# ilovepose/fast-human-pose-estimation.pytorch

Measured on AMD Instinct MI355X. Metric: images/sec FPD train step (4-stack HG student, 8-stack teacher) 256x256, higher is better.
Workload: dtype bf16; 1 GPU; configs[1]: hourglass student S=4 F=128 + teacher S=8 F=256, 256x256, batch 32/GPU, fused FPD step incl. Adam, teacher forward one batch ahead on a 2nd stream; global_batch=32, parallelism=dp1, backend=mfma, launch=one native plan call per phase, kernels launched eagerly on 3 streams, ranks=1, finite=True

## Files before the change

fast-human-pose-estimation.pytorch_amd/csrc/api.hip:

```cpp
#include <cstdarg>
#include <cstdio>
#include <cstdlib>
#include <cstring>
#include <string>
#include <vector>

#include "common.h"

int fpd_conv_mfma_launch(const fpd_conv_t& a, hipStream_t st);
int fpd_conv_tile_launch(const fpd_conv_t& a, hipStream_t st);
int fpd_conv_pp_launch(const fpd_conv_t& a, hipStream_t st);
int fpd_conv_c1_launch(const fpd_conv_t& a, hipStream_t st);
int fpd_conv_c3_launch(const fpd_conv_t& a, hipStream_t st);
int fpd_conv_c3_pair_launch(const fpd_conv_t& a, const fpd_conv_t& b, hipStream_t st);
int fpd_conv_c3_fold_ok(const fpd_conv_t& a, const fpd_conv_t* b);
int fpd_conv_c3_option(int which, int value);
int fpd_conv_c1_pair_launch(const fpd_conv_t& a, const fpd_conv_t& b, hipStream_t st);
int fpd_conv_c1_fold_ok(const fpd_conv_t& a, const fpd_conv_t* b);
int fpd_conv_c1_option(int which, int value);
int fpd_conv_c1_wgrad_partials(const fpd_conv_t& a);
int fpd_conv_c1_pair_wgrad_partials(const fpd_conv_t& a, const fpd_conv_t& b, int* na, int* nb);
int fpd_conv_pp_pair_launch(const fpd_conv_t& a, const fpd_conv_t& b, hipStream_t st);
int fpd_conv_pp_fold_ok(const fpd_conv_t& a, const fpd_conv_t* b);
int fpd_conv_tile_fold_ok(const fpd_conv_t& a);
int fpd_conv_tile_pair_fold_ok(const fpd_conv_t& a, const fpd_conv_t& b);
int fpd_conv_pp_option(int which, int value);
int fpd_conv_pp_wgrad_partials(const fpd_conv_t& a);
int fpd_conv_pp_pair_wgrad_partials(const fpd_conv_t& a, const fpd_conv_t& b, int* na, int* nb);
int fpd_conv_tile_pair_launch(const fpd_conv_t& a, const fpd_conv_t& b, hipStream_t st);
int fpd_bneck_fused_launch(const fpd_bneck_t& a, hipStream_t st);
int fpd_bneck_fold_launch(const fpd_bneck_t& a, float* out, hipStream_t st);
int fpd_pck_launch(const fpd_pck_t& a, hipStream_t st);
int fpd_conv_smallc_launch(const fpd_conv_t& a, hipStream_t st);
bool fpd_conv_f8_domain(const fpd_conv_t& a);
int fpd_conv_tile_f8_launch(const fpd_conv_t& a, const void* w8, const float* wscale, hipStream_t st);
int fpd_weight_quant_f8_launch(const fpd_wquant_entry_t* table, int n, hipStream_t st);
int fpd_flip_w_launch(const float* x, float* y, int64_t rows, int W, hipStream_t st);
int fpd_flip_merge_launch(const fpd_flipmerge_t& p, hipStream_t st);
int fpd_final_preds_launch(const fpd_finalpreds_t& p, hipStream_t st);
int fpd_render_targets_launch(const fpd_targets_t& a, hipStream_t st);
int fpd_warp_affine_launch(const fpd_warp_t& a, hipStream_t st);
int fpd_head_fused_launch(const fpd_head_t& a, hipStream_t st);
int fpd_head_fold_launch(const fpd_head_t& a, float* out, hipStream_t st);
int fpd_bneck_fused_pair_launch(const fpd_bneck_t& a, const fpd_bneck_t& b, hipStream_t st);
int fpd_wgrad_mfma_launch(const fpd_wgrad_t& a, hipStream_t st);
int fpd_wgrad_tile_launch(const fpd_wgrad_t& a, hipStream_t st);
int fpd_wgrad_tile_partials(const fpd_wgrad_t& a);
int fpd_wgrad_smallc_launch(const fpd_wgrad_t& a, hipStream_t st);
int fpd_wgrad_smallc_partials(const fpd_wgrad_t& a);
int fpd_wgrad_mfma_partials(const fpd_wgrad_t& a);
int fpd_wgrad_naive_partials(const fpd_wgrad_t& a);
int fpd_stem_wgrad_mfma_partials(const fpd_stem_t& a);
int fpd_stem_wgrad_partials(const fpd_stem_t& a);
int fpd_wreduce_launch(const fpd_wreduce_entry_t* table, int n, int64_t max_elems, hipStream_t st);
int fpd_conv_naive_launch(const fpd_conv_t& a, hipStream_t st);
int fpd_wgrad_naive_launch(const fpd_wgrad_t& a, hipStream_t st);
int fpd_stem_forward_launch(const fpd_stem_t& a, hipStream_t st);
int fpd_stem_forward_mfma_launch(const fpd_stem_t& a, hipStream_t st);
int fpd_stem_forward_s2d_launch(const fpd_stem_t& a, hipStream_t st);
int fpd_stem_wgrad_s2d_launch(const fpd_stem_t& a, hipStream_t st);
int fpd_stem_wgrad_s2d_partials(const fpd_stem_t& a);
int fpd_stem_wgrad_mfma_launch(const fpd_stem_t& a, hipStream_t st);
int fpd_stem_wgrad_launch(const fpd_stem_t& a, hipStream_t st);
int fpd_elementwise_launch(const fpd_ew_t& a, hipStream_t st);
int fpd_elementwise_pair_launch(const fpd_ew_t& a, const fpd_ew_t& b, hipStream_t st);
int fpd_affsum_launch(const fpd_affsum_t& a, hipStream_t st);
int fpd_loss_launch(const fpd_loss_t& a, hipStream_t st);
int fpd_adam_launch(const fpd_adam_t& a, hipStream_t st);
int fpd_weight_prep_launch(const fpd_wprep_entry_t* table, int n, int64_t max_elems, int dtype, hipStream_t st);
int fpd_bn_update_running_launch(const fpd_bnupd_entry_t* table, int n, hipStream_t st);
int fpd_cast_launch(const void* src, void* dst, int64_t n, int sd, int dd, hipStream_t st);
int fpd_nchw_to_nhwc_launch(const float* src, void* dst, int N, int C, int H, int W, int dtype, hipStream_t st);
int fpd_nhwc_to_nchw_launch(const void* src, float* dst, int N, int C, int H, int W, int dtype, hipStream_t st);

int g_fpd_backend = FPD_BACKEND_MFMA;
static thread_local char g_err[512] = "";

static FILE* g_launch_log_file = nullptr;
static bool launch_log_open() {
    const char* path = getenv("FPD_LAUNCH_LOG");
    if (path == nullptr || path[0] == 0) return false;
    g_launch_log_file = fopen(path, "w");
    if (g_launch_log_file == nullptr) fprintf(stderr, "[fpd_amd] FPD_LAUNCH_LOG: cannot open %s\n", path);
    return g_launch_log_file != nullptr;
}
bool g_fpd_launch_log = launch_log_open();
static thread_local char g_op_tag[256] = "-";
void fpd_log_launch(const char* kernel, const dim3& grid, const dim3& block) {
    if (g_launch_log_file == nullptr) return;
    fprintf(g_launch_log_file, "%s\t%u\t%u\t%s\n", kernel, grid.x * grid.y * grid.z, block.x * block.y * block.z, g_op_tag);
    fflush(g_launch_log_file);
}

int fpd_fail(int code, const char* fmt, ...) {
    va_list ap;
    va_start(ap, fmt);
    vsnprintf(g_err, sizeof(g_err), fmt, ap);
    va_end(ap);
    return code;
}

static int check_launch() {
    hipError_t e = hipGetLastError();
    if (e != hipSuccess) return fpd_fail(-100 - (int)e, "kernel launch failed: %s", hipGetErrorString(e));
    return 0;
}

static int validate_conv_dims(int N, int H, int W, int C, int K, int R, int S, int stride, int pad, int P, int Q) {
    FPD_REQUIRE(N > 0 && H > 0 && W > 0 && C > 0 && K > 0 && R > 0 && S > 0 && stride > 0 && pad >= 0,
                "conv: non-positive dimension");
    FPD_REQUIRE(P == (H + 2 * pad - R) / stride + 1 && Q == (W + 2 * pad - S) / stride + 1,
                "conv: output %dx%d inconsistent with input %dx%d k=%dx%d stride=%d pad=%d", P, Q, H, W, R, S, stride, pad);
    FPD_REQUIRE((int64_t)N * H * W * C < (1ll << 31) && (int64_t)N * P * Q * K < (1ll << 31), "conv: tensor too large for 32-bit indexing");
    return 0;
}

extern "C" {

const char* fpd_last_error(void) { return g_err; }
int fpd_abi_version(void) { return FPD_ABI_VERSION; }
int64_t fpd_stats_words(int32_t channels) { return FPD_STATS_WORDS(channels); }
int fpd_set_backend(int32_t backend) {
    const int prev = g_fpd_backend;
    if (backend == FPD_BACKEND_MFMA || backend == FPD_BACKEND_NAIVE || backend == FPD_BACKEND_MFMA_GENERIC) g_fpd_backend = backend;
    return prev;
}

static int g_wgrad_tile_only = 0;

int fpd_set_option(const char* name, int32_t value) {
    FPD_REQUIRE(name, "set_option: null name");
    if (!strcmp(name, "conv_pp")) return fpd_conv_pp_option(0, value);
    if (!strcmp(name, "conv_pp_blocks")) return fpd_conv_pp_option(1, value);
    if (!strcmp(name, "conv_c1")) return fpd_conv_c1_option(0, value);
    if (!strcmp(name, "conv_c1_blocks")) return fpd_conv_c1_option(1, value);
    if (!strcmp(name, "conv_c1_launches")) return fpd_conv_c1_option(2, value);
    if (!strcmp(name, "conv_c3")) return fpd_conv_c3_option(0, value);
    if (!strcmp(name, "conv_c3_blocks")) return fpd_conv_c3_option(1, value);
    if (!strcmp(name, "conv_c3_launches")) return fpd_conv_c3_option(2, value);
    if (!strcmp(name, "wgrad_tile_only")) { g_wgrad_tile_only = value; return 0; }
    return fpd_fail(-2, "set_option: unknown option '%s'", name);
}

int fpd_abi_sizeof(const char* n) {
#define SZ(T) if (!strcmp(n, #T)) return (int)sizeof(T)
    SZ(fpd_bn_t); SZ(fpd_conv_t); SZ(fpd_wgrad_t); SZ(fpd_stem_t); SZ(fpd_ew_t); SZ(fpd_loss_t); SZ(fpd_adam_t);
    SZ(fpd_wprep_entry_t); SZ(fpd_bnupd_entry_t); SZ(fpd_memset_t); SZ(fpd_table_t); SZ(fpd_wreduce_entry_t); SZ(fpd_bneck_t); SZ(fpd_conv_pair_t); SZ(fpd_bneck_pair_t); SZ(fpd_ew_pair_t); SZ(fpd_pck_t); SZ(fpd_head_t); SZ(fpd_affsum_t); SZ(fpd_layout_t);
    SZ(fpd_conv_f8_t); SZ(fpd_wquant_entry_t); SZ(fpd_flipmerge_t); SZ(fpd_finalpreds_t); SZ(fpd_targets_t); SZ(fpd_warp_src_t); SZ(fpd_warp_t);
#undef SZ
    return -1;
}

static int validate_conv(const fpd_conv_t* a) {
    FPD_REQUIRE(a && a->x && a->w && a->y, "conv: null pointer");
    int rc = validate_conv_dims(a->N, a->H, a->W, a->C, a->K, a->R, a->S, a->stride, a->pad, a->P, a->Q);
    if (rc) return rc;
    FPD_REQUIRE(a->dtype == FPD_F32 || a->dtype == FPD_BF16, "conv: bad dtype %d", a->dtype);
    FPD_REQUIRE(a->bn.mode == FPD_BN_NONE || (a->bn.gamma && a->bn.beta), "conv: BN prologue without gamma/beta");
    FPD_REQUIRE(a->bn.mode != FPD_BN_TRAIN || a->bn.stats, "conv: train-mode BN without statistics");
    FPD_REQUIRE(a->bn.mode != FPD_BN_EVAL || (a->bn.running_mean && a->bn.running_var), "conv: eval-mode BN without running stats");
    FPD_REQUIRE(a->epi == FPD_EPI_PLAIN || (a->epi_x && a->epi_stats && a->epi_bn.mode == FPD_BN_TRAIN && a->epi_bn.stats),
                "conv: BNRELU_BWD epilogue needs epi_x, epi_stats and a train-mode epi_bn");
    return 0;
}

static int dispatch_conv(const fpd_conv_t* a, hipStream_t st) {
    int rc = 1;
    if (g_fpd_backend == FPD_BACKEND_MFMA) rc = fpd_conv_c1_launch(*a, st);
    if (rc == 1 && g_fpd_backend == FPD_BACKEND_MFMA) rc = fpd_conv_c3_launch(*a, st);
    if (rc == 1 && g_fpd_backend == FPD_BACKEND_MFMA) rc = fpd_conv_pp_launch(*a, st);
    FPD_REQUIRE(rc != 1 || a->wg_partial == nullptr, "conv: a fused weight gradient (wg_partial) needs the persistent kernel; "
                "fpd_conv_fused_wgrad_partials() reports 0 for this launch");
    if (rc == 1 && g_fpd_backend == FPD_BACKEND_MFMA) rc = fpd_conv_tile_launch(*a, st);
    FPD_REQUIRE(rc != 1 || a->fold_x == nullptr, "conv: a folded BN-backward apply (fold_x) needs the persistent or the halo-tile "
                "kernel; fpd_conv_fold_supported() reports 0 for this launch");
    if (rc == 1 && g_fpd_backend != FPD_BACKEND_NAIVE) rc = fpd_conv_mfma_launch(*a, st);
    if (rc == 1 && g_fpd_backend != FPD_BACKEND_NAIVE) rc = fpd_conv_smallc_launch(*a, st);
    if (rc == 1) rc = fpd_conv_naive_launch(*a, st);
    return rc;
}

int fpd_conv_forward(const fpd_conv_t* a, fpd_stream_t stream) {
    int rc = validate_conv(a);
    if (rc) return rc;
    rc = dispatch_conv(a, (hipStream_t)stream);
    return rc ? rc : check_launch();
}

int fpd_conv_fold_supported(const fpd_conv_t* a) {
    if (!a || g_fpd_backend != FPD_BACKEND_MFMA || validate_conv(a) != 0) return 0;
    return (fpd_conv_c1_fold_ok(*a, nullptr) || fpd_conv_c3_fold_ok(*a, nullptr) || fpd_conv_pp_fold_ok(*a, nullptr) || fpd_conv_tile_fold_ok(*a)) ? 1 : 0;
}
int fpd_conv_pair_fold_supported(const fpd_conv_pair_t* p) {
    if (!p || g_fpd_backend != FPD_BACKEND_MFMA || validate_conv(&p->a) != 0 || validate_conv(&p->b) != 0) return 0;
    if (fpd_conv_c1_fold_ok(p->a, &p->b)) return 1;
    if (fpd_conv_c3_fold_ok(p->a, &p->b)) return 1;
    if (fpd_conv_pp_fold_ok(p->a, &p->b)) return 1;
    const int r = fpd_conv_tile_pair_fold_ok(p->a, p->b);
    if (r >= 0) return r;
    return (fpd_conv_fold_supported(&p->a) && fpd_conv_fold_supported(&p->b)) ? 1 : 0;
}

int fpd_conv_fused_wgrad_partials(const fpd_conv_t* a) {
    if (!a || g_fpd_backend != FPD_BACKEND_MFMA || validate_conv(a) != 0) return 0;
    const int n = fpd_conv_c1_wgrad_partials(*a);
    return n >= 0 ? n : fpd_conv_pp_wgrad_partials(*a);
}
int fpd_conv_pair_fused_wgrad_partials(const fpd_conv_pair_t* p, int32_t* n_a, int32_t* n_b) {
    FPD_REQUIRE(p && n_a && n_b, "conv_pair_fused_wgrad_partials: null pointer");
    *n_a = *n_b = 0;
    if (g_fpd_backend != FPD_BACKEND_MFMA || validate_conv(&p->a) != 0 || validate_conv(&p->b) != 0) return 0;
    int na = 0, nb = 0;
    if (fpd_conv_c1_pair_wgrad_partials(p->a, p->b, &na, &nb) < 0) fpd_conv_pp_pair_wgrad_partials(p->a, p->b, &na, &nb);
    *n_a = na; *n_b = nb;
    return 0;
}

int fpd_conv_f8_in_domain(const fpd_conv_t* c) { return (c && fpd_conv_f8_domain(*c)) ? 1 : 0; }

int fpd_conv_forward_f8(const fpd_conv_f8_t* a, fpd_stream_t stream) {
    FPD_REQUIRE(a, "conv_f8: null pointer");
    int rc = validate_conv(&a->c);
    if (rc) return rc;
    FPD_REQUIRE(a->w8 && a->w8_scale, "conv_f8: null fp8 weights / scales");
    FPD_REQUIRE(((uintptr_t)a->w8 & 15) == 0, "conv_f8: w8 must be 16-byte aligned");
    rc = 1;
    if (g_fpd_backend == FPD_BACKEND_MFMA) rc = fpd_conv_tile_f8_launch(a->c, a->w8, a->w8_scale, (hipStream_t)stream);
    if (rc == 1) rc = dispatch_conv(&a->c, (hipStream_t)stream);
    return rc ? rc : check_launch();
}

int fpd_weight_quant_f8(const fpd_wquant_entry_t* t, int32_t n, fpd_stream_t stream) {
    FPD_REQUIRE(n == 0 || t != nullptr, "weight_quant_f8: null table");
    int rc = fpd_weight_quant_f8_launch(t, n, (hipStream_t)stream);
    return rc ? rc : check_launch();
}

int fpd_conv_forward_pair(const fpd_conv_pair_t* p, fpd_stream_t stream) {
    FPD_REQUIRE(p, "conv_pair: null pointer");
    int rc = validate_conv(&p->a);
    if (rc) return rc;
    rc = validate_conv(&p->b);
    if (rc) return rc;
    hipStream_t st = (hipStream_t)stream;
    rc = 1;
    if (g_fpd_backend == FPD_BACKEND_MFMA) rc = fpd_conv_c1_pair_launch(p->a, p->b, st);
    if (rc == 1 && g_fpd_backend == FPD_BACKEND_MFMA) rc = fpd_conv_c3_pair_launch(p->a, p->b, st);
    if (rc == 1 && g_fpd_backend == FPD_BACKEND_MFMA) rc = fpd_conv_pp_pair_launch(p->a, p->b, st);
    FPD_REQUIRE(rc != 1 || (p->a.wg_partial == nullptr && p->b.wg_partial == nullptr),
                "conv_pair: fused weight gradients need the persistent kernel; fpd_conv_pair_fused_wgrad_partials() reports 0 for this launch");
    if (rc == 1 && g_fpd_backend == FPD_BACKEND_MFMA) rc = fpd_conv_tile_pair_launch(p->a, p->b, st);
    if (rc == 1) {
        rc = dispatch_conv(&p->a, st);
        if (rc == 0) rc = dispatch_conv(&p->b, st);
    }
    return rc ? rc : check_launch();
}

static int validate_bneck_bns(const fpd_bneck_t* a) {
    const fpd_bn_t* bns[3] = {&a->bn1, &a->bn2, &a->bn3};
    for (int i = 0; i < 3; ++i)
        FPD_REQUIRE(bns[i]->mode == FPD_BN_EVAL && bns[i]->relu && bns[i]->gamma && bns[i]->beta && bns[i]->running_mean &&
                    bns[i]->running_var, "bottleneck: bn%d must be an eval-mode BN+ReLU with running statistics", i + 1);
    return 0;
}

int fpd_bottleneck_fold(const fpd_bneck_t* a, fpd_stream_t stream) {
    FPD_REQUIRE(a && a->folded, "bottleneck_fold: null pointer");
    int rc = validate_bneck_bns(a);
    if (rc) return rc;
    rc = fpd_bneck_fold_launch(*a, const_cast<float*>(a->folded), (hipStream_t)stream);
    if (rc == 1) return fpd_fail(-3, "bottleneck_fold: C=%d P=%d is outside the fused kernel's domain", a->C, a->P);
    return rc ? rc : check_launch();
}

int fpd_bottleneck_forward_pair(const fpd_bneck_pair_t* p, fpd_stream_t stream) {
    FPD_REQUIRE(p, "bottleneck_pair: null pointer");
    const fpd_bneck_t* ab[2] = {&p->a, &p->b};
    for (const fpd_bneck_t* a : ab) {
        FPD_REQUIRE(a->x && a->y && a->w1 && a->w2 && a->w3 && a->x != a->y, "bottleneck_pair: null pointer or y aliases x");
        FPD_REQUIRE((int64_t)a->N * a->H * a->W * a->C < ((int64_t)1 << 31), "bottleneck_pair: tensor too large for 32-bit indexing");
        int rc = validate_bneck_bns(a);
        if (rc) return rc;
    }
    int rc = fpd_bneck_fused_pair_launch(p->a, p->b, (hipStream_t)stream);
    if (rc == 1) {
        rc = fpd_bottleneck_forward(&p->a, stream);
        return rc ? rc : fpd_bottleneck_forward(&p->b, stream);
    }
    return rc ? rc : check_launch();
}

int fpd_bottleneck_forward(const fpd_bneck_t* a, fpd_stream_t stream) {
    FPD_REQUIRE(a && a->x && a->y && a->w1 && a->w2 && a->w3, "bottleneck: null pointer");
    FPD_REQUIRE(a->x != a->y, "bottleneck: y must not alias x");
    FPD_REQUIRE(a->N > 0 && a->H > 0 && a->W > 0 && a->C > 0 && a->P > 0, "bottleneck: bad dims");
    FPD_REQUIRE((int64_t)a->N * a->H * a->W * a->C < ((int64_t)1 << 31), "bottleneck: tensor too large for 32-bit indexing");
    int rc = validate_bneck_bns(a);
    if (rc) return rc;
    rc = fpd_bneck_fused_launch(*a, (hipStream_t)stream);
    if (rc == 1)
        return fpd_fail(-3, "bottleneck: shape N=%d H=%d W=%d C=%d P=%d dtype=%d is outside the fused kernel's domain",
                        a->N, a->H, a->W, a->C, a->P, a->dtype);
    return rc ? rc : check_launch();
}

int fpd_conv_wgrad(const fpd_wgrad_t* a, fpd_stream_t stream) {
    FPD_REQUIRE(a && a->x && a->dy && a->dw, "wgrad: null pointer");
    int rc = validate_conv_dims(a->N, a->H, a->W, a->C, a->K, a->R, a->S, a->stride, a->pad, a->P, a->Q);
    if (rc) return rc;
    FPD_REQUIRE(a->dtype == FPD_F32 || a->dtype == FPD_BF16, "wgrad: bad dtype %d", a->dtype);
    hipStream_t st = (hipStream_t)stream;
    rc = 1;
    FPD_REQUIRE(a->partial == nullptr || a->partial_stride >= (int64_t)a->K * a->R * a->S * a->C + a->K,
                "wgrad: partial_stride %lld smaller than weight + bias", (long long)a->partial_stride);
    if (g_fpd_backend == FPD_BACKEND_MFMA) rc = fpd_wgrad_tile_launch(*a, st);
    FPD_REQUIRE(!(g_wgrad_tile_only && rc == 1), "wgrad: option wgrad_tile_only is set and the halo-tile kernel declines N=%d H=%d W=%d C=%d K=%d R=%d", a->N, a->H, a->W, a->C, a->K, a->R);
    if (rc == 1 && g_fpd_backend != FPD_BACKEND_NAIVE) rc = fpd_wgrad_mfma_launch(*a, st);
    if (rc == 1 && g_fpd_backend != FPD_BACKEND_NAIVE) rc = fpd_wgrad_smallc_launch(*a, st);
    if (rc == 1) rc = fpd_wgrad_naive_launch(*a, st);
    return rc ? rc : check_launch();
}

int fpd_wgrad_num_partials(const fpd_wgrad_t* a) {
    if (!a) return 0;
    int n = 0;
    if (g_fpd_backend == FPD_BACKEND_MFMA) n = fpd_wgrad_tile_partials(*a);
    if (n == 0 && g_fpd_backend != FPD_BACKEND_NAIVE) n = fpd_wgrad_mfma_partials(*a);
    if (n == 0 && g_fpd_backend != FPD_BACKEND_NAIVE) n = fpd_wgrad_smallc_partials(*a);
    if (n == 0) n = fpd_wgrad_naive_partials(*a);
    return n;
}

int fpd_stem_wgrad_num_partials(const fpd_stem_t* a) {
    if (!a) return 0;
    int n = 0;
    if (g_fpd_backend == FPD_BACKEND_MFMA) n = fpd_stem_wgrad_s2d_partials(*a);
    if (n == 0 && g_fpd_backend == FPD_BACKEND_MFMA) n = fpd_stem_wgrad_mfma_partials(*a);
    if (n == 0) n = fpd_stem_wgrad_partials(*a);
    return n;
}

int fpd_wgrad_reduce(const fpd_wreduce_entry_t* t, int32_t n, int64_t max_elems, fpd_stream_t stream) {
    int rc = fpd_wreduce_launch(t, n, max_elems, (hipStream_t)stream);
    return rc ? rc : check_launch();
}

int fpd_stem_forward(const fpd_stem_t* a, fpd_stream_t stream) {
    FPD_REQUIRE(a && a->x && a->w && a->bias && a->y, "stem: null pointer");
    FPD_REQUIRE(a->P == (a->H + 6 - 7) / 2 + 1 && a->Q == (a->W + 6 - 7) / 2 + 1, "stem: bad output size");
    int rc = 1;
    if (g_fpd_backend == FPD_BACKEND_MFMA) rc = fpd_stem_forward_s2d_launch(*a, (hipStream_t)stream);
    if (rc == 1 && g_fpd_backend == FPD_BACKEND_MFMA) rc = fpd_stem_forward_mfma_launch(*a, (hipStream_t)stream);
    if (rc == 1) rc = fpd_stem_forward_launch(*a, (hipStream_t)stream);
    return rc ? rc : check_launch();
}

int fpd_stem_wgrad(const fpd_stem_t* a, fpd_stream_t stream) {
    FPD_REQUIRE(a && a->x && a->dy && a->dw, "stem wgrad: null pointer");
    FPD_REQUIRE(a->partial == nullptr || a->partial_stride >= (int64_t)a->K * 148, "stem wgrad: partial_stride %lld smaller than weight + bias",
                (long long)a->partial_stride);
    int rc = 1;
    if (g_fpd_backend == FPD_BACKEND_MFMA) rc = fpd_stem_wgrad_s2d_launch(*a, (hipStream_t)stream);
    if (rc == 1 && g_fpd_backend == FPD_BACKEND_MFMA) rc = fpd_stem_wgrad_mfma_launch(*a, (hipStream_t)stream);
    if (rc == 1) rc = fpd_stem_wgrad_launch(*a, (hipStream_t)stream);
    return rc ? rc : check_launch();
}

int fpd_affsum(const fpd_affsum_t* a, fpd_stream_t stream) {
    FPD_REQUIRE(a && a->y, "affsum: null pointer");
    FPD_REQUIRE(a->nterms >= 1 && a->nterms <= FPD_AFFSUM_MAX, "affsum: %d terms (1..%d supported)", a->nterms, FPD_AFFSUM_MAX);
    FPD_REQUIRE(a->dtype == FPD_F32 || a->dtype == FPD_BF16, "affsum: bad dtype %d", a->dtype);
    for (int j = 0; j < a->nterms; ++j) {
        const int up = a->t[j].up;
        FPD_REQUIRE(a->t[j].x, "affsum: term %d has no input", j);
        FPD_REQUIRE((up == 1 || up == 2 || up == 4 || up == 8) && a->H % up == 0 && a->W % up == 0,
                    "affsum: term %d: up-sampling factor %d does not divide %dx%d", j, up, a->H, a->W);
        const fpd_bn_t& bn = a->t[j].bn;
        FPD_REQUIRE(bn.mode == FPD_BN_NONE || (bn.gamma && bn.beta), "affsum: term %d: BN without gamma/beta", j);
        FPD_REQUIRE(bn.mode != FPD_BN_TRAIN || bn.stats, "affsum: term %d: train-mode BN without statistics", j);
        FPD_REQUIRE(bn.mode != FPD_BN_EVAL || (bn.running_mean && bn.running_var), "affsum: term %d: eval-mode BN without running stats", j);
    }
    int rc = fpd_affsum_launch(*a, (hipStream_t)stream);
    return rc ? rc : check_launch();
}

int fpd_elementwise(const fpd_ew_t* a, fpd_stream_t stream) {
    FPD_REQUIRE(a && (a->y || a->op == FPD_EW_BNRELU_BWD_R), "elementwise: null pointer");
    int rc = fpd_elementwise_launch(*a, (hipStream_t)stream);
    return rc ? rc : check_launch();
}

static int validate_head(const fpd_head_t* a) {
    FPD_REQUIRE(a && a->y0 && a->score && a->w_fc && a->w_score, "head: null pointer");
    FPD_REQUIRE(a->next == nullptr || (a->x && a->w_fc2 && a->w_score2 && a->next != a->x && a->next != a->y0),
                "head: next needs x, w_fc2, w_score2 and must not alias an input");
    FPD_REQUIRE(a->N > 0 && a->H > 0 && a->W > 0 && (int64_t)a->N * a->H * a->W * a->C < ((int64_t)1 << 31), "head: bad dims");
    FPD_REQUIRE(a->bn.mode == FPD_BN_EVAL && a->bn.relu && a->bn.gamma && a->bn.beta && a->bn.running_mean && a->bn.running_var,
                "head: bn must be an eval-mode BN+ReLU with running statistics");
    return 0;
}
int fpd_head_forward(const fpd_head_t* a, fpd_stream_t stream) {
    int rc = validate_head(a);
    if (rc) return rc;
    rc = fpd_head_fused_launch(*a, (hipStream_t)stream);
    if (rc == 1) return fpd_fail(-3, "head: C=%d J=%d dtype=%d is outside the fused kernel's domain", a->C, a->J, a->dtype);
    return rc ? rc : check_launch();
}
int fpd_head_fold(const fpd_head_t* a, fpd_stream_t stream) {
    FPD_REQUIRE(a && a->folded, "head_fold: null pointer");
    FPD_REQUIRE(a->bn.mode == FPD_BN_EVAL && a->bn.gamma && a->bn.beta && a->bn.running_mean && a->bn.running_var, "head_fold: bn");
    int rc = fpd_head_fold_launch(*a, const_cast<float*>(a->folded), (hipStream_t)stream);
    if (rc == 1) return fpd_fail(-3, "head_fold: C=%d is outside the fused kernel's domain", a->C);
    return rc ? rc : check_launch();
}

int fpd_pck(const fpd_pck_t* a, fpd_stream_t stream) {
    FPD_REQUIRE(a && a->out && a->target && a->counts && a->log && a->cursor, "pck: null pointer");
    FPD_REQUIRE(a->B > 0 && a->J > 0 && a->H > 0 && a->W > 0 && a->log_slots > 0, "pck: bad dims");
    FPD_REQUIRE(a->dtype == FPD_F32 || a->dtype == FPD_BF16, "pck: bad dtype %d", a->dtype);
    int rc = fpd_pck_launch(*a, (hipStream_t)stream);
    return rc ? rc : check_launch();
}

int fpd_flip_w(const float* x, float* y, int64_t rows, int32_t W, fpd_stream_t stream) {
    FPD_REQUIRE(x && y && x != y, "flip_w: null or aliased pointer");
    FPD_REQUIRE(rows > 0 && W > 0, "flip_w: bad dims");
    int rc = fpd_flip_w_launch(x, y, rows, W, (hipStream_t)stream);
    return rc ? rc : check_launch();
}
int fpd_flip_merge(const fpd_flipmerge_t* a, fpd_stream_t stream) {
    FPD_REQUIRE(a && a->b && a->y && a->b != a->y, "flip_merge: null or aliased pointer");
    FPD_REQUIRE(a->N > 0 && a->H > 0 && a->W > 0 && a->J > 0 && a->J <= FPD_MAX_JOINTS, "flip_merge: bad dims (J <= %d)", FPD_MAX_JOINTS);
    for (int j = 0; j < a->J; ++j) FPD_REQUIRE(a->src[j] >= 0 && a->src[j] < a->J, "flip_merge: src[%d] = %d out of range", j, a->src[j]);
    int rc = fpd_flip_merge_launch(*a, (hipStream_t)stream);
    return rc ? rc : check_launch();
}
int fpd_final_preds(const fpd_finalpreds_t* a, fpd_stream_t stream) {
    FPD_REQUIRE(a && a->hm && a->coords && a->maxvals, "final_preds: null pointer");
    FPD_REQUIRE((a->trans == nullptr) == (a->preds == nullptr), "final_preds: trans and preds go together");
    FPD_REQUIRE(a->N > 0 && a->H > 0 && a->W > 0 && a->J > 0, "final_preds: bad dims");
    int rc = fpd_final_preds_launch(*a, (hipStream_t)stream);
    return rc ? rc : check_launch();
}
int fpd_render_targets(const fpd_targets_t* a, fpd_stream_t stream) {
    FPD_REQUIRE(a && a->joints && a->vis && a->g && a->target && a->weight, "render_targets: null pointer");
    FPD_REQUIRE(a->B > 0 && a->J > 0 && a->H > 0 && a->W > 0 && a->patch > 0 && (a->patch & 1), "render_targets: bad dims");
    FPD_REQUIRE(a->stride_x > 0 && a->stride_y > 0, "render_targets: bad stride");
    int rc = fpd_render_targets_launch(*a, (hipStream_t)stream);
    return rc ? rc : check_launch();
}
int fpd_warp_affine(const fpd_warp_t* a, fpd_stream_t stream) {
    FPD_REQUIRE(a && a->src && a->out, "warp_affine: null pointer");
    FPD_REQUIRE(a->B > 0 && a->B <= 65535 && a->H > 0 && a->W > 0, "warp_affine: bad dims");
    for (int c = 0; c < 3; ++c) FPD_REQUIRE(a->std[c] != 0.f, "warp_affine: std[%d] == 0", c);
    int rc = fpd_warp_affine_launch(*a, (hipStream_t)stream);
    return rc ? rc : check_launch();
}

int fpd_elementwise_pair(const fpd_ew_pair_t* p, fpd_stream_t stream) {
    FPD_REQUIRE(p && p->a.y && p->b.y, "elementwise_pair: null pointer");
    int rc = fpd_elementwise_pair_launch(p->a, p->b, (hipStream_t)stream);
    if (rc == 1) {
        rc = fpd_elementwise_launch(p->a, (hipStream_t)stream);
        if (rc == 0) rc = fpd_elementwise_launch(p->b, (hipStream_t)stream);
    }
    return rc ? rc : check_launch();
}

int fpd_loss(const fpd_loss_t* a, fpd_stream_t stream) {
    FPD_REQUIRE(a && a->teacher && a->target && a->weight && a->losses, "loss: null pointer");
    int rc = fpd_loss_launch(*a, (hipStream_t)stream);
    return rc ? rc : check_launch();
}

int fpd_adam(const fpd_adam_t* a, fpd_stream_t stream) {
    FPD_REQUIRE(a && a->param && a->grad && a->m && a->v && a->n >= 0, "adam: null pointer");
    int rc = fpd_adam_launch(*a, (hipStream_t)stream);
    return rc ? rc : check_launch();
}

int fpd_weight_prep(const fpd_wprep_entry_t* t, int32_t n, int64_t max_elems, int32_t dtype, fpd_stream_t stream) {
    int rc = fpd_weight_prep_launch(t, n, max_elems, dtype, (hipStream_t)stream);
    return rc ? rc : check_launch();
}
int fpd_bn_update_running(const fpd_bnupd_entry_t* t, int32_t n, fpd_stream_t stream) {
    int rc = fpd_bn_update_running_launch(t, n, (hipStream_t)stream);
    return rc ? rc : check_launch();
}
int fpd_cast(const void* src, void* dst, int64_t n, int32_t sd, int32_t dd, fpd_stream_t stream) {
    int rc = fpd_cast_launch(src, dst, n, sd, dd, (hipStream_t)stream);
    return rc ? rc : check_launch();
}
int fpd_nchw_to_nhwc(const float* src, void* dst, int32_t N, int32_t C, int32_t H, int32_t W, int32_t dtype, fpd_stream_t stream) {
    int rc = fpd_nchw_to_nhwc_launch(src, dst, N, C, H, W, dtype, (hipStream_t)stream);
    return rc ? rc : check_launch();
}
int fpd_nhwc_to_nchw(const void* src, float* dst, int32_t N, int32_t C, int32_t H, int32_t W, int32_t dtype, fpd_stream_t stream) {
    int rc = fpd_nhwc_to_nchw_launch(src, dst, N, C, H, W, dtype, (hipStream_t)stream);
    return rc ? rc : check_launch();
}

struct fpd_op {
    int32_t type;
    union {
        fpd_affsum_t affsum; fpd_layout_t layout; fpd_conv_f8_t conv8; fpd_conv_t conv; fpd_conv_pair_t pair; fpd_bneck_t bneck; fpd_bneck_pair_t bpair; fpd_ew_pair_t epair; fpd_pck_t pck; fpd_head_t head; fpd_wgrad_t wgrad; fpd_stem_t stem; fpd_ew_t ew; fpd_loss_t loss; fpd_adam_t adam;
        fpd_memset_t mset; fpd_table_t table;
    } u;
};
struct fpd_sched {
    int32_t lane = 0;
    bool record = false;
    hipEvent_t done = nullptr;
    std::vector<int32_t> waits;
};
struct fpd_plan {
    std::vector<fpd_op> ops;
    std::vector<fpd_sched> sched;
    std::vector<hipGraphExec_t> graphs;
    std::vector<hipGraph_t> graph_defs;
    hipStream_t lanes[FPD_MAX_LANES] = {};
    hipEvent_t lane_done[FPD_MAX_LANES] = {};
    hipEvent_t fork = nullptr;
};

fpd_plan* fpd_plan_create(void) { return new fpd_plan(); }
void fpd_plan_destroy(fpd_plan* p) {
    if (!p) return;
    for (auto g : p->graphs) (void)hipGraphExecDestroy(g);
    for (auto g : p->graph_defs) (void)hipGraphDestroy(g);
    for (auto& s : p->sched) if (s.done) (void)hipEventDestroy(s.done);
    for (int l = 0; l < FPD_MAX_LANES; ++l) {
        if (p->lanes[l]) (void)hipStreamDestroy(p->lanes[l]);
        if (p->lane_done[l]) (void)hipEventDestroy(p->lane_done[l]);
    }
    if (p->fork) (void)hipEventDestroy(p->fork);
    delete p;
}
int fpd_plan_size(const fpd_plan* p) { return p ? (int)p->ops.size() : -1; }

int fpd_plan_add(fpd_plan* p, int32_t op, const void* args, int64_t bytes) {
    FPD_REQUIRE(p && args, "plan_add: null");
    fpd_op o;
    memset(&o, 0, sizeof(o));
    o.type = op;
    size_t want = 0;
    switch (op) {
        case FPD_OP_CONV: want = sizeof(fpd_conv_t); break;
        case FPD_OP_CONV_F8: want = sizeof(fpd_conv_f8_t); break;
        case FPD_OP_WGRAD: want = sizeof(fpd_wgrad_t); break;
        case FPD_OP_CONV_PAIR: want = sizeof(fpd_conv_pair_t); break;
        case FPD_OP_BNECK_PAIR: want = sizeof(fpd_bneck_pair_t); break;
        case FPD_OP_EW_PAIR: want = sizeof(fpd_ew_pair_t); break;
        case FPD_OP_PCK: want = sizeof(fpd_pck_t); break;
        case FPD_OP_HEAD: case FPD_OP_HEAD_FOLD: want = sizeof(fpd_head_t); break;
        case FPD_OP_BNECK: case FPD_OP_BNECK_FOLD: want = sizeof(fpd_bneck_t); break;
        case FPD_OP_STEM_FWD: case FPD_OP_STEM_WGRAD: want = sizeof(fpd_stem_t); break;
        case FPD_OP_EW: want = sizeof(fpd_ew_t); break;
        case FPD_OP_LOSS: want = sizeof(fpd_loss_t); break;
        case FPD_OP_ADAM: want = sizeof(fpd_adam_t); break;
        case FPD_OP_MEMSET: case FPD_OP_NOP: want = sizeof(fpd_memset_t); break;
        case FPD_OP_AFFSUM: want = sizeof(fpd_affsum_t); break;
        case FPD_OP_NCHW2NHWC: want = sizeof(fpd_layout_t); break;
        case FPD_OP_WPREP: case FPD_OP_BNUPD: case FPD_OP_WREDUCE: case FPD_OP_WQUANT: want = sizeof(fpd_table_t); break;
        default: return fpd_fail(-2, "plan_add: unknown op %d", op);
    }
    FPD_REQUIRE((size_t)bytes == want, "plan_add: op %d expects %zu bytes of args, got %lld", op, want, (long long)bytes);
    memcpy(&o.u, args, want);
    p->ops.push_back(o);
    p->sched.emplace_back();
    return (int)p->ops.size() - 1;
}

int fpd_plan_set_schedule(fpd_plan* p, int32_t op, int32_t lane, const int32_t* wait_ops, int32_t n_waits) {
    FPD_REQUIRE(p && op >= 0 && op < (int)p->ops.size(), "plan_set_schedule: bad op index %d", op);
    FPD_REQUIRE(lane >= 0 && lane < FPD_MAX_LANES, "plan_set_schedule: lane %d outside [0,%d)", lane, FPD_MAX_LANES);
    FPD_REQUIRE(n_waits >= 0 && (n_waits == 0 || wait_ops != nullptr), "plan_set_schedule: bad wait list");
    for (int i = 0; i < n_waits; ++i)
        FPD_REQUIRE(wait_ops[i] >= 0 && wait_ops[i] < op, "plan_set_schedule: op %d may only wait for earlier ops (got %d)", op, wait_ops[i]);
    fpd_sched& s = p->sched[op];
    s.lane = lane;
    s.waits.assign(wait_ops, wait_ops + n_waits);
    for (int i = 0; i < n_waits; ++i) p->sched[wait_ops[i]].record = true;
    return 0;
}

int fpd_plan_mark_event(fpd_plan* p, int32_t op) {
    FPD_REQUIRE(p && op >= 0 && op < (int)p->ops.size(), "plan_mark_event: bad op index %d", op);
    p->sched[op].record = true;
    return 0;
}

int fpd_plan_wait_op(fpd_plan* p, int32_t op, fpd_stream_t stream) {
    FPD_REQUIRE(p && op >= 0 && op < (int)p->ops.size(), "plan_wait_op: bad op index %d", op);
    FPD_REQUIRE(p->sched[op].record && p->sched[op].done, "plan_wait_op: op %d has no recorded event (mark it, then run its range)", op);
    FPD_CHECK_HIP(hipStreamWaitEvent((hipStream_t)stream, p->sched[op].done, 0));
    return 0;
}

static void conv_tag(char* p, size_t n, const char* what, const fpd_conv_t& c) {
    snprintf(p, n, "%s N=%d H=%d W=%d C=%d K=%d R=%d s=%d %s%s%s%s", what, c.N, c.H, c.W, c.C, c.K, c.R, c.stride,
             c.epi == FPD_EPI_BNRELU_BWD ? "dgrad" : "fwd", c.bn.mode == FPD_BN_EVAL ? " evalbn" : "", c.wg_partial ? " +wgrad" : "", c.fold_x ? " +fold" : "");
}
static void set_op_tag(int idx, const fpd_op& o) {
    char t[200] = "";
    static const char* ew_names[] = {"bnrelu_fwd", "bnrelu_bwd_r", "bn_bwd_apply", "maxpool_fwd", "maxpool_bwd", "upadd_fwd", "sumpool", "add", "relu_mask", "dilate2"};
    auto ewn = [&](int op) { return (op >= 0 && op < 10) ? ew_names[op] : "ew"; };
    switch (o.type) {
        case FPD_OP_CONV: conv_tag(t, sizeof(t), "conv", o.u.conv); break;
        case FPD_OP_CONV_F8: conv_tag(t, sizeof(t), "conv_f8", o.u.conv8.c); break;
        case FPD_OP_CONV_PAIR: {
            char a[90], b[90];
            conv_tag(a, sizeof(a), "conv2", o.u.pair.a);
            snprintf(b, sizeof(b), " | H=%d W=%d", o.u.pair.b.H, o.u.pair.b.W);
            snprintf(t, sizeof(t), "%s%s", a, b);
            break;
        }
        case FPD_OP_WGRAD: snprintf(t, sizeof(t), "wgrad N=%d H=%d W=%d C=%d K=%d R=%d s=%d", o.u.wgrad.N, o.u.wgrad.H, o.u.wgrad.W, o.u.wgrad.C, o.u.wgrad.K, o.u.wgrad.R, o.u.wgrad.stride); break;
        case FPD_OP_BNECK: snprintf(t, sizeof(t), "bneck N=%d H=%d W=%d C=%d P=%d", o.u.bneck.N, o.u.bneck.H, o.u.bneck.W, o.u.bneck.C, o.u.bneck.P); break;
        case FPD_OP_BNECK_PAIR: snprintf(t, sizeof(t), "bneck2 N=%d H=%d W=%d C=%d P=%d | H=%d W=%d", o.u.bpair.a.N, o.u.bpair.a.H, o.u.bpair.a.W, o.u.bpair.a.C, o.u.bpair.a.P, o.u.bpair.b.H, o.u.bpair.b.W); break;
        case FPD_OP_HEAD: snprintf(t, sizeof(t), "head N=%d H=%d W=%d C=%d J=%d", o.u.head.N, o.u.head.H, o.u.head.W, o.u.head.C, o.u.head.J); break;
        case FPD_OP_EW: snprintf(t, sizeof(t), "ew %s N=%d H=%d W=%d C=%d", ewn(o.u.ew.op), o.u.ew.N, o.u.ew.H, o.u.ew.W, o.u.ew.C); break;
        case FPD_OP_EW_PAIR: snprintf(t, sizeof(t), "ew2 %s N=%d H=%d W=%d C=%d | H=%d W=%d", ewn(o.u.epair.a.op), o.u.epair.a.N, o.u.epair.a.H, o.u.epair.a.W, o.u.epair.a.C, o.u.epair.b.H, o.u.epair.b.W); break;
        case FPD_OP_STEM_FWD: case FPD_OP_STEM_WGRAD: snprintf(t, sizeof(t), "%s N=%d H=%d W=%d K=%d", o.type == FPD_OP_STEM_FWD ? "stem_fwd" : "stem_wgrad", o.u.stem.N, o.u.stem.H, o.u.stem.W, o.u.stem.K); break;
        case FPD_OP_AFFSUM: snprintf(t, sizeof(t), "affsum N=%d H=%d W=%d C=%d terms=%d", o.u.affsum.N, o.u.affsum.H, o.u.affsum.W, o.u.affsum.C, o.u.affsum.nterms); break;
        case FPD_OP_LOSS: snprintf(t, sizeof(t), "loss B=%d J=%d H=%d W=%d S=%d", o.u.loss.B, o.u.loss.J, o.u.loss.H, o.u.loss.W, o.u.loss.S); break;
        case FPD_OP_ADAM: snprintf(t, sizeof(t), "adam n=%lld", (long long)o.u.adam.n); break;
        case FPD_OP_WREDUCE: snprintf(t, sizeof(t), "wreduce entries=%d", o.u.table.n); break;
        case FPD_OP_WPREP: snprintf(t, sizeof(t), "wprep entries=%d", o.u.table.n); break;
        case FPD_OP_BNUPD: snprintf(t, sizeof(t), "bnupd entries=%d", o.u.table.n); break;
        default: snprintf(t, sizeof(t), "op%d", o.type); break;
    }
    snprintf(g_op_tag, sizeof(g_op_tag), "%d\t%s", idx, t);
}

static int run_op(const fpd_op& o, fpd_stream_t s) {
    switch (o.type) {
        case FPD_OP_CONV: return fpd_conv_forward(&o.u.conv, s);
        case FPD_OP_CONV_F8: return fpd_conv_forward_f8(&o.u.conv8, s);
        case FPD_OP_WQUANT: return fpd_weight_quant_f8((const fpd_wquant_entry_t*)o.u.table.table, o.u.table.n, s);
        case FPD_OP_WGRAD: return fpd_conv_wgrad(&o.u.wgrad, s);
        case FPD_OP_CONV_PAIR: return fpd_conv_forward_pair(&o.u.pair, s);
        case FPD_OP_BNECK_PAIR: return fpd_bottleneck_forward_pair(&o.u.bpair, s);
        case FPD_OP_EW_PAIR: return fpd_elementwise_pair(&o.u.epair, s);
        case FPD_OP_PCK: return fpd_pck(&o.u.pck, s);
        case FPD_OP_HEAD: return fpd_head_forward(&o.u.head, s);
        case FPD_OP_HEAD_FOLD: return fpd_head_fold(&o.u.head, s);
        case FPD_OP_BNECK: return fpd_bottleneck_forward(&o.u.bneck, s);
        case FPD_OP_BNECK_FOLD: return fpd_bottleneck_fold(&o.u.bneck, s);
        case FPD_OP_STEM_FWD: return fpd_stem_forward(&o.u.stem, s);
        case FPD_OP_STEM_WGRAD: return fpd_stem_wgrad(&o.u.stem, s);
        case FPD_OP_EW: return fpd_elementwise(&o.u.ew, s);
        case FPD_OP_LOSS: return fpd_loss(&o.u.loss, s);
        case FPD_OP_ADAM: return fpd_adam(&o.u.adam, s);
        case FPD_OP_MEMSET: {
            FPD_CHECK_HIP(hipMemsetAsync(o.u.mset.ptr, 0, (size_t)o.u.mset.bytes, (hipStream_t)s));
            return 0;
        }
        case FPD_OP_NOP: return 0;
        case FPD_OP_AFFSUM: return fpd_affsum(&o.u.affsum, s);
        case FPD_OP_NCHW2NHWC:
            return fpd_nchw_to_nhwc(o.u.layout.src, o.u.layout.dst, o.u.layout.N, o.u.layout.C, o.u.layout.H, o.u.layout.W, o.u.layout.dtype, s);
        case FPD_OP_WPREP:
            return fpd_weight_prep((const fpd_wprep_entry_t*)o.u.table.table, o.u.table.n, o.u.table.max_elems, o.u.table.dtype, s);
        case FPD_OP_BNUPD: return fpd_bn_update_running((const fpd_bnupd_entry_t*)o.u.table.table, o.u.table.n, s);
        case FPD_OP_WREDUCE: return fpd_wgrad_reduce((const fpd_wreduce_entry_t*)o.u.table.table, o.u.table.n, o.u.table.max_elems, s);
    }
    return fpd_fail(-2, "run_op: unknown op %d", o.type);
}

static int lane_priority() { return 0; }

static int side_streams() { return FPD_MAX_LANES; }

int fpd_plan_run(fpd_plan* p, int32_t begin, int32_t end, fpd_stream_t stream) {
    FPD_REQUIRE(p && begin >= 0 && end <= (int)p->ops.size() && begin <= end, "plan_run: bad range [%d,%d)", begin, end);
    hipStream_t main_s = (hipStream_t)stream;
    bool multi = false;
    for (int i = begin; i < end; ++i) multi |= p->sched[i].lane != 0;
    bool used[FPD_MAX_LANES] = {};
    if (multi) {
        if (!p->fork) FPD_CHECK_HIP(hipEventCreateWithFlags(&p->fork, hipEventDisableTiming));
        FPD_CHECK_HIP(hipEventRecord(p->fork, main_s));
    }
    int rc = 0;
    for (int i = begin; i < end && rc == 0; ++i) {
        fpd_sched& sc = p->sched[i];
        hipStream_t st = main_s;
        if (sc.lane != 0) {
            const int l = 1 + (sc.lane - 1) % side_streams();
            if (!p->lanes[l]) {
                FPD_CHECK_HIP(hipStreamCreateWithPriority(&p->lanes[l], hipStreamNonBlocking, lane_priority()));
                FPD_CHECK_HIP(hipEventCreateWithFlags(&p->lane_done[l], hipEventDisableTiming));
            }
            st = p->lanes[l];
            if (!used[l]) {
                FPD_CHECK_HIP(hipStreamWaitEvent(st, p->fork, 0));
                used[l] = true;
            }
        }
        for (int32_t w : sc.waits)
            if (w >= begin && w < end) FPD_CHECK_HIP(hipStreamWaitEvent(st, p->sched[w].done, 0));
        if (g_fpd_launch_log) set_op_tag(i, p->ops[i]);
        rc = run_op(p->ops[i], (fpd_stream_t)st);
        if (rc) {
            char tmp[400];
            snprintf(tmp, sizeof(tmp), "%s", g_err);
            rc = fpd_fail(rc, "plan op %d (type %d): %s", i, p->ops[i].type, tmp);
            break;
        }
        if (sc.record) {
            if (!sc.done) FPD_CHECK_HIP(hipEventCreateWithFlags(&sc.done, hipEventDisableTiming));
            FPD_CHECK_HIP(hipEventRecord(sc.done, st));
        }
    }
    for (int l = 1; l < FPD_MAX_LANES; ++l)
        if (used[l]) {
            FPD_CHECK_HIP(hipEventRecord(p->lane_done[l], p->lanes[l]));
            FPD_CHECK_HIP(hipStreamWaitEvent(main_s, p->lane_done[l], 0));
        }
    return rc;
}

int fpd_plan_run_op(fpd_plan* p, int32_t op, fpd_stream_t stream) {
    FPD_REQUIRE(p && op >= 0 && op < (int)p->ops.size(), "plan_run_op: bad op index %d", op);
    if (g_fpd_launch_log) set_op_tag(op, p->ops[op]);
    return run_op(p->ops[op], stream);
}

int fpd_plan_capture(fpd_plan* p, int32_t begin, int32_t end, fpd_stream_t stream) {
    FPD_REQUIRE(p, "plan_capture: null");
    FPD_REQUIRE(!g_fpd_launch_log, "plan_capture: FPD_LAUNCH_LOG is set -- the launch log keys a kernel trace 1:1 and cannot follow hipGraph replays; unset one of them");
    hipStream_t st = (hipStream_t)stream;
    FPD_CHECK_HIP(hipStreamBeginCapture(st, hipStreamCaptureModeThreadLocal));
    int rc = fpd_plan_run(p, begin, end, stream);
    hipGraph_t g = nullptr;
    hipError_t e = hipStreamEndCapture(st, &g);
    if (rc) { if (g) (void)hipGraphDestroy(g); return rc; }
    if (e != hipSuccess) return fpd_fail(-100 - (int)e, "hipStreamEndCapture: %s", hipGetErrorString(e));
    hipGraphExec_t ge = nullptr;
    FPD_CHECK_HIP(hipGraphInstantiate(&ge, g, nullptr, nullptr, 0));
    p->graph_defs.push_back(g);
    p->graphs.push_back(ge);
    return (int)p->graphs.size() - 1;
}

int fpd_plan_replay(fpd_plan* p, int32_t gid, fpd_stream_t stream) {
    FPD_REQUIRE(p && gid >= 0 && gid < (int)p->graphs.size(), "plan_replay: bad graph id %d", gid);
    FPD_CHECK_HIP(hipGraphLaunch(p->graphs[gid], (hipStream_t)stream));
    return 0;
}

void* fpd_event_create(void) {
    hipEvent_t e = nullptr;
    if (hipEventCreate(&e) != hipSuccess) return nullptr;
    return (void*)e;
}
int fpd_event_record(void* ev, fpd_stream_t stream) {
    FPD_CHECK_HIP(hipEventRecord((hipEvent_t)ev, (hipStream_t)stream));
    return 0;
}
float fpd_event_elapsed_ms(void* start, void* stop) {
    float ms = -1.f;
    if (hipEventSynchronize((hipEvent_t)stop) != hipSuccess) return -1.f;
    if (hipEventElapsedTime(&ms, (hipEvent_t)start, (hipEvent_t)stop) != hipSuccess) return -1.f;
    return ms;
}
void fpd_event_destroy(void* ev) { if (ev) (void)hipEventDestroy((hipEvent_t)ev); }

}
```

fast-human-pose-estimation.pytorch_amd/csrc/bneck_fused.hip:

```cpp
#include <algorithm>
#include <cstdlib>
#include <type_traits>

#include "common.h"

namespace {

typedef unsigned int u32x4 __attribute__((ext_vector_type(4)));
template <int N, typename F>
__device__ __forceinline__ void static_for(F&& f) {
    if constexpr (N > 0) {
        static_for<N - 1>(f);
        f(std::integral_constant<int, N - 1>{});
    }
}

#ifdef FPD_BNECK_TIMING
#define STAMP(i) do { if (tid == 0 && bid_in == 0) stamps[i] = clock64(); } while (0)
#else
#define STAMP(i) do { } while (0)
#endif

template <int P>
__device__ __forceinline__ void bneck_fold_tables(const fpd_bneck_t& a, float* out, int tid, int nthreads) {
    constexpr int C = 2 * P;
    for (int c = tid; c < C; c += nthreads) {
        float sc, sh;
        bn_coef_eval(a.bn1, c, sc, sh);
        out[c] = sc;
        out[C + c] = sh;
        out[2 * C + 4 * P + c] = a.b3 ? a.b3[c] : 0.f;
    }
    for (int c = tid; c < 2 * P; c += nthreads) {
        const bool second = c >= P;
        const int cc = second ? c - P : c;
        float sc, sh;
        bn_coef_eval(second ? a.bn3 : a.bn2, cc, sc, sh);
        const float* bias = second ? a.b2 : a.b1;
        out[2 * C + (second ? 2 * P : 0) + cc] = sc;
        out[2 * C + (second ? 2 * P : 0) + P + cc] = fmaf(sc, bias ? bias[cc] : 0.f, sh);
    }
}

template <int P>
__global__ void bneck_fold_kernel(const fpd_bneck_t a, float* out) { bneck_fold_tables<P>(a, out, threadIdx.x, blockDim.x); }

template <int P, bool DMA>
__device__ __forceinline__ void bneck_eval_body(const fpd_bneck_t& a, const int logW, const int swz, const int bid_in,
                                                const int nblk, const int ntiles) {
    constexpr int C = 2 * P;
    constexpr int LDW = DMA ? P : P + 8;
    constexpr int LDX = 64 + 8;
    constexpr int LD2 = P + 8;
    constexpr int TNH = P / 64;
    constexpr int CW = 32 * TNH;
    constexpr int NSTEP = 9 + 2;
    constexpr int VPR2 = P / 8;
    constexpr int WV = P * VPR2 / 512;
    constexpr int W1V = P * 8 / 512;
    constexpr int NCH = C / 64;
    constexpr int ASTG = (128 + P) * LDX;
    extern __shared__ __attribute__((aligned(16))) unsigned char smem[];

    const int tid = threadIdx.x, lane = tid & 63, wave = tid >> 6;
#ifdef FPD_BNECK_TIMING
    long long stamps[8];
    long long astamp[10];
    int acnt = 0;
#define ASTAMP() do { if (tid == 0 && bid_in == 0 && acnt < 10) astamp[acnt++] = clock64(); } while (0)
#else
#define ASTAMP() do { } while (0)
#endif
    STAMP(0);
    const int q = wave & 3, hC = wave >> 2;
    const int koff = 8 * (lane >> 5);
    const int H = a.H, W = a.W;
    const int M = a.N * H * W, GR = a.N * H;
    const int nrows = 128 >> logW, hrows = nrows + 2, WP = W + 2;
    const int rrows = 2 * nrows;
    const bool whole = (128 % (H * W)) == 0;
    const int irows = whole ? hrows : rrows;
    const int zero_px = irows * WP;
    int m0 = 0, g0 = 0;
    int vrow0 = 0;

    float* s_sc1 = reinterpret_cast<float*>(smem);
    float* s_sh1 = s_sc1 + C;
    float* s_sc2 = s_sh1 + C;
    float* s_sh2 = s_sc2 + P;
    float* s_sc3 = s_sh2 + P;
    float* s_sh3 = s_sc3 + P;
    float* s_b3 = s_sh3 + P;
    bf16_t* sA2 = reinterpret_cast<bf16_t*>(s_b3 + C);
    bf16_t* sR2 = sA2 + (zero_px + 3) * LD2;
    const bf16_t* __restrict__ x = reinterpret_cast<const bf16_t*>(a.x);
    const bf16_t* __restrict__ w1 = reinterpret_cast<const bf16_t*>(a.w1);
    const bf16_t* __restrict__ w2 = reinterpret_cast<const bf16_t*>(a.w2);
    const bf16_t* __restrict__ w3 = reinterpret_cast<const bf16_t*>(a.w3);

    int hp0 = whole ? W : 0;
    int npass = whole ? 1 : ((hrows * W + 127) >> 7);
    const int xpx = tid >> 3, xcv = (tid & 7) * 8;
    int xo[2];
    bool xok[2];
    auto pass_addr = [&](int p) __attribute__((always_inline)) {
#pragma unroll
        for (int i = 0; i < 2; ++i) {
            const int hp = hp0 + 128 * p + xpx + 64 * i;
            const int hr = hp >> logW, j = hp & (W - 1);
            const int g = g0 - 1 + hr;
            xok[i] = hr < hrows && (unsigned)g < (unsigned)GR;
            xo[i] = xok[i] ? (g * W + j) * C + xcv : 0;
        }
    };
    int w1o[W1V], w1l[W1V];
#pragma unroll
    for (int i = 0; i < W1V; ++i) {
        const int v = tid + i * 512;
        w1o[i] = (v >> 3) * C + (v & 7) * 8;
        w1l[i] = 128 * LDX + (v >> 3) * LDX + (v & 7) * 8;
    }
    const int xl = xpx * LDX + xcv;

    u32x4 rx[NCH][2], rw[NCH][W1V];
    auto a_load = [&](auto kcc) __attribute__((always_inline)) {
        constexpr int kc = decltype(kcc)::value;
        static_for<2>([&](auto ic) {
            constexpr int i = decltype(ic)::value;
            const u32x4 z = {0u, 0u, 0u, 0u};
            rx[kc][i] = z;
            if (xok[i]) rx[kc][i] = *reinterpret_cast<const u32x4*>(x + (xo[i] + kc * 64));
        });
        static_for<W1V>([&](auto ic) {
            constexpr int i = decltype(ic)::value;
            rw[kc][i] = *reinterpret_cast<const u32x4*>(w1 + (w1o[i] + kc * 64));
        });
    };
    constexpr int NSL = 2 + W1V;
    auto a_store_slice = [&](auto kcc, auto slc) __attribute__((always_inline)) {
        constexpr int kc = decltype(kcc)::value, sl = decltype(slc)::value;
        bf16_t* dst = sR2 + (kc & 1) * ASTG;
        if constexpr (sl < 2) {
            f32x4 sc[2], sh[2];
            sc[0] = *reinterpret_cast<const f32x4*>(s_sc1 + kc * 64 + xcv);
            sc[1] = *reinterpret_cast<const f32x4*>(s_sc1 + kc * 64 + xcv + 4);
            sh[0] = *reinterpret_cast<const f32x4*>(s_sh1 + kc * 64 + xcv);
            sh[1] = *reinterpret_cast<const f32x4*>(s_sh1 + kc * 64 + xcv + 4);
            float f[8];
            const u32x4 r = rx[kc][sl];
            DT<bf16_t>::unpack(make_uint4(r[0], r[1], r[2], r[3]), f);
#pragma unroll
            for (int e = 0; e < 8; ++e) f[e] = fmaxf(fmaf(f[e], sc[e >> 2][e & 3], sh[e >> 2][e & 3]), 0.f);
            *reinterpret_cast<uint4*>(dst + xl + 64 * sl * LDX) = DT<bf16_t>::pack(f);
        } else if constexpr (sl < NSL) {
            *reinterpret_cast<u32x4*>(dst + w1l[sl - 2]) = rw[kc][sl - 2];
        }
    };
    auto a_store = [&](auto kcc) __attribute__((always_inline)) {
        static_for<NSL>([&](auto slc) { a_store_slice(kcc, slc); });
    };
    int t2o[WV], t3o[WV], tlo[WV];
#pragma unroll
    for (int i = 0; i < WV; ++i) {
        const int v = tid + i * 512;
        const int row = v / VPR2, col = (v - row * VPR2) * 8;
        t2o[i] = row * 9 * P + col;
        t3o[i] = row * P + col;
        tlo[i] = row * LD2 + col;
    }
    u32x4 rb[DMA ? 1 : 2][DMA ? 1 : WV];
    auto t_load = [&](auto sc_) __attribute__((always_inline)) {
        constexpr int s = decltype(sc_)::value;
        if constexpr (!DMA) {
            static_for<WV>([&](auto ic) {
                constexpr int i = decltype(ic)::value;
                const bf16_t* src = s < 9 ? w2 + (t2o[i] + s * P) : w3 + (t3o[i] + (s - 9) * P * P);
                rb[s & 1][i] = *reinterpret_cast<const u32x4*>(src);
            });
        }
    };
    auto t_store = [&](auto sc_) __attribute__((always_inline)) {
        constexpr int s = decltype(sc_)::value;
        if constexpr (!DMA) {
            bf16_t* dst = sR2 + (s & 1) * P * LDW;
            static_for<WV>([&](auto ic) {
                constexpr int i = decltype(ic)::value;
                *reinterpret_cast<u32x4*>(dst + tlo[i]) = rb[s & 1][i];
            });
        }
    };
    constexpr int CPR = P / 8;
    constexpr int RPI = 64 / CPR;
    constexpr int DPW = P / RPI / 8;
    unsigned dma2[DMA ? DPW : 1], dma3[DMA ? DPW : 1];
    if constexpr (DMA) {
#pragma unroll
        for (int j = 0; j < DPW; ++j) {
            const int row = wave * DPW * RPI + j * RPI + lane / CPR;
            const int sw = (P == 128) ? (row & 15) : ((row >> 1) & 7);
            const int c8 = ((lane % CPR) ^ sw) * 8;
            dma2[j] = (unsigned)(row * 9 * P + c8) * 2u;
            dma3[j] = (unsigned)(row * P + c8) * 2u;
        }
    }
    auto t_dma = [&](auto sc_) __attribute__((always_inline)) {
        constexpr int s = decltype(sc_)::value;
        if constexpr (DMA) {
            unsigned char* ring = reinterpret_cast<unsigned char*>(sR2) + (s & 1) * P * P * 2 + wave * DPW * 1024;
            const char* gbase = s < 9 ? reinterpret_cast<const char*>(w2) + s * P * 2
                                      : reinterpret_cast<const char*>(w3) + (s - 9) * P * P * 2;
            static_for<DPW>([&](auto jc) {
                constexpr int j = decltype(jc)::value;
                unsigned off = s < 9 ? dma2[j] : dma3[j];
                asm volatile("" : "+v"(off));
                __builtin_amdgcn_global_load_lds((const __attribute__((address_space(1))) void*)(gbase + off),
                                                 (__attribute__((address_space(3))) void*)(ring + j * 1024), 16, 0, 0);
            });
        }
    };

    if (a.folded != nullptr) {
        for (int v = tid; v < (3 * C + 4 * P) / 4; v += 512)
            reinterpret_cast<f32x4*>(s_sc1)[v] = reinterpret_cast<const f32x4*>(a.folded)[v];
    } else {
        bneck_fold_tables<P>(a, s_sc1, tid, 512);
    }

    const int t_beg = fpd_cut(bid_in, ntiles, nblk), t_end = fpd_cut(bid_in + 1, ntiles, nblk);
    (void)swz;
    for (int tile = t_beg; tile < t_end; ++tile) {
    {
        m0 = tile * 128;
        g0 = m0 >> logW;
        vrow0 = (tile * nrows) % rrows;
        if (!whole) {
            const bool incr = tile > t_beg && (g0 % H) != 0;
            hp0 = incr ? 2 * W : 0;
            npass = incr ? 1 : ((hrows * W + 127) >> 7);
        }
    }
    pass_addr(0);
    static_for<NCH>([&](auto kcc) { a_load(kcc); });
    if (npass > 1) pass_addr(1);
    __syncthreads();
    {
        constexpr int VR = LD2 / 8;
        const uint4 z = make_uint4(0, 0, 0, 0);
        for (int v = tid; v < (2 * irows + 3) * VR; v += 512) {
            const int pz = v / VR, cv = (v - pz * VR) * 8;
            const int px = pz < 2 * irows ? ((pz >> 1) * WP + ((pz & 1) ? WP - 1 : 0)) : zero_px + (pz - 2 * irows);
            *reinterpret_cast<uint4*>(sA2 + px * LD2 + cv) = z;
        }
    }
    STAMP(1);

    auto refill = [&](auto kcc, int pp) __attribute__((always_inline)) {
        constexpr int kc = decltype(kcc)::value;
        if (pp + 1 < npass) a_load(kcc);
        else if constexpr (kc < 2) t_load(kcc);
    };
#ifdef FPD_BNECK_TIMING
    acnt = 0;
#endif
    ASTAMP();
    a_store(std::integral_constant<int, 0>{});
    refill(std::integral_constant<int, 0>{}, 0);
    __syncthreads();
    ASTAMP();
    for (int p = 0; p < npass; ++p) {
        f32x16 acc[TNH];
#pragma unroll
        for (int tn = 0; tn < TNH; ++tn)
#pragma unroll
            for (int i = 0; i < 16; ++i) acc[tn][i] = 0.f;
        static_for<NCH>([&](auto kcc) {
            constexpr int kc = decltype(kcc)::value;
            auto stage_slice = [&](auto slc) __attribute__((always_inline)) {
                constexpr int sl = decltype(slc)::value;
                if constexpr (kc + 1 < NCH) {
                    a_store_slice(std::integral_constant<int, (kc + 1) % NCH>{}, slc);
                    if constexpr (sl == NSL - 1) refill(std::integral_constant<int, (kc + 1) % NCH>{}, p);
                } else {
                    if (p + 1 < npass) {
                        a_store_slice(std::integral_constant<int, 0>{}, slc);
                        if constexpr (sl == NSL - 1) {
                            if (p + 2 < npass) pass_addr(p + 2);
                            refill(std::integral_constant<int, 0>{}, p + 1);
                        }
                    }
                }
            };
            const bf16_t* xrow = sR2 + (kc & 1) * ASTG + (q * 32 + (lane & 31)) * LDX + koff;
            const bf16_t* wrow = sR2 + (kc & 1) * ASTG + 128 * LDX + (hC * CW + (lane & 31)) * LDX + koff;
            static_for<4>([&](auto kkc) {
                constexpr int kk = decltype(kkc)::value;
                const bf16x8 px = *reinterpret_cast<const bf16x8*>(xrow + kk * 16);
#pragma unroll
                for (int tn = 0; tn < TNH; ++tn) {
                    const bf16x8 wf = *reinterpret_cast<const bf16x8*>(wrow + tn * 32 * LDX + kk * 16);
                    acc[tn] = __builtin_amdgcn_mfma_f32_32x32x16_bf16(wf, px, acc[tn], 0, 0, 0);
                }
                stage_slice(kkc);
            });
            __syncthreads();
            ASTAMP();
        });
        if (p + 1 == npass) {
            t_dma(std::integral_constant<int, 0>{});
            t_dma(std::integral_constant<int, 1>{});
        }
        const int hp = hp0 + 128 * p + q * 32 + (lane & 31);
        const int hr = hp >> logW, j = hp & (W - 1);
        if (hr < hrows) {
            const int rr = whole ? hr : ((vrow0 + hr) & (rrows - 1));
            bf16_t* dst = sA2 + (rr * WP + j + 1) * LD2;
#pragma unroll
            for (int tn = 0; tn < TNH; ++tn)
#pragma unroll
                for (int gi = 0; gi < 4; ++gi) {
                    const int c = hC * CW + tn * 32 + 8 * gi + 4 * (lane >> 5);
                    const f32x4 sc = *reinterpret_cast<const f32x4*>(s_sc2 + c);
                    const f32x4 sh = *reinterpret_cast<const f32x4*>(s_sh2 + c);
                    float v[4];
#pragma unroll
                    for (int e = 0; e < 4; ++e) v[e] = fmaxf(fmaf(acc[tn][4 * gi + e], sc[e], sh[e]), 0.f);
                    *reinterpret_cast<uint2*>(dst + c) = make_uint2(f2bf_pk(v[0], v[1]), f2bf_pk(v[2], v[3]));
                }
        }
    }

    const int ml = q * 32 + (lane & 31);
    const int a3px = whole ? 0 : vrow0 * WP;
    int ab[3];
    {
        const int ti = ml >> logW, tj = ml & (W - 1);
        const int g = g0 + ti;
        const int pr = g % H;
        const bool live = g < GR;
        const int r0 = whole ? ti : ((vrow0 + ti) & (rrows - 1)), r1 = whole ? ti + 1 : ((vrow0 + ti + 1) & (rrows - 1)),
                  r2 = whole ? ti + 2 : ((vrow0 + ti + 2) & (rrows - 1));
        ab[0] = (live && pr - 1 >= 0) ? (r0 * WP + tj) * LD2 : zero_px * LD2;
        ab[1] = live ? (r1 * WP + tj) * LD2 : zero_px * LD2;
        ab[2] = (live && pr + 1 < H) ? (r2 * WP + tj) * LD2 : zero_px * LD2;
    }
    STAMP(2);
    t_store(std::integral_constant<int, 0>{});
    t_load(std::integral_constant<int, 2>{});
    __syncthreads();
    STAMP(3);

    f32x16 accB[TNH], accC[2][TNH];
#pragma unroll
    for (int tn = 0; tn < TNH; ++tn)
#pragma unroll
        for (int i = 0; i < 16; ++i) accB[tn][i] = 0.f;

    const int wsw = (P == 128) ? (lane & 15) : ((lane >> 1) & 7);
    auto mma = [&](const bf16_t* arow, int buf, f32x16* acc) __attribute__((always_inline)) {
        const bf16_t* wbase = sR2 + buf * P * LDW + (hC * CW + (lane & 31)) * LDW;
#pragma unroll
        for (int kk = 0; kk < P / 16; ++kk) {
            const bf16x8 px = *reinterpret_cast<const bf16x8*>(arow + kk * 16);
            const int wo = DMA ? (((2 * kk + (lane >> 5)) ^ wsw) * 8) : (kk * 16 + koff);
#pragma unroll
            for (int tn = 0; tn < TNH; ++tn) {
                const bf16x8 wf = *reinterpret_cast<const bf16x8*>(wbase + tn * 32 * LDW + wo);
                acc[tn] = __builtin_amdgcn_mfma_f32_32x32x16_bf16(wf, px, acc[tn], 0, 0, 0);
            }
        }
    };

    constexpr int VW = CW / 8;
    constexpr int NIT = 32 * VW / 64;
    u32x4 rres[2][NIT];
    auto res_load = [&](auto stc) __attribute__((always_inline)) {
        constexpr int st = decltype(stc)::value;
        static_for<NIT>([&](auto itc) {
            constexpr int it = decltype(itc)::value;
            const int idx = lane + 64 * it;
            const int px = idx / VW, cv = (idx - px * VW) * 8;
            const int m = m0 + q * 32 + px;
            const u32x4 z = {0u, 0u, 0u, 0u};
            rres[st][it] = z;
            if (m < M) rres[st][it] = *reinterpret_cast<const u32x4*>(x + ((size_t)m * C + st * P + hC * CW + cv));
        });
    };

    static_for<NSTEP>([&](auto sc_) {
        constexpr int s = decltype(sc_)::value;
        if constexpr (DMA && s >= 1 && s + 1 < NSTEP) t_dma(std::integral_constant<int, (s + 1 < NSTEP ? s + 1 : 0)>{});
        if constexpr (s < 9) {
            mma(sA2 + ab[s / 3] + (s % 3) * LD2 + koff, s & 1, accB);
        } else {
#pragma unroll
            for (int tn = 0; tn < TNH; ++tn)
#pragma unroll
                for (int i = 0; i < 16; ++i) accC[s - 9][tn][i] = 0.f;
            mma(sA2 + (a3px + ml) * LD2 + koff, s & 1, accC[s - 9]);
        }
        if constexpr (s + 1 < NSTEP) {
            t_store(std::integral_constant<int, s + 1>{});
            if constexpr (s + 3 < NSTEP) t_load(std::integral_constant<int, (s + 3 < NSTEP ? s + 3 : 0)>{});
            if constexpr (s == 8) res_load(std::integral_constant<int, 0>{});
            if constexpr (s == 9) res_load(std::integral_constant<int, 1>{});
            __syncthreads();
        }
        if constexpr (s == 8) {
            STAMP(4);
            bf16_t* dst = sA2 + (a3px + ml) * LD2;
#pragma unroll
            for (int tn = 0; tn < TNH; ++tn)
#pragma unroll
                for (int gi = 0; gi < 4; ++gi) {
                    const int c = hC * CW + tn * 32 + 8 * gi + 4 * (lane >> 5);
                    const f32x4 sc = *reinterpret_cast<const f32x4*>(s_sc3 + c);
                    const f32x4 sh = *reinterpret_cast<const f32x4*>(s_sh3 + c);
                    float v[4];
#pragma unroll
                    for (int e = 0; e < 4; ++e) v[e] = fmaxf(fmaf(accB[tn][4 * gi + e], sc[e], sh[e]), 0.f);
                    *reinterpret_cast<uint2*>(dst + c) = make_uint2(f2bf_pk(v[0], v[1]), f2bf_pk(v[2], v[3]));
                }
            __syncthreads();
        }
    });

    STAMP(5);
    constexpr int LDS_ = CW + 4;
    float* stage = reinterpret_cast<float*>(sR2) + wave * 32 * LDS_;
    bf16_t* __restrict__ y = reinterpret_cast<bf16_t*>(a.y);
    static_for<2>([&](auto stc) {
        constexpr int st = decltype(stc)::value;
        __syncthreads();
#pragma unroll
        for (int tn = 0; tn < TNH; ++tn)
#pragma unroll
            for (int gi = 0; gi < 4; ++gi) {
                f32x4 v;
#pragma unroll
                for (int e = 0; e < 4; ++e) v[e] = accC[st][tn][4 * gi + e];
                *reinterpret_cast<f32x4*>(stage + (lane & 31) * LDS_ + tn * 32 + 8 * gi + 4 * (lane >> 5)) = v;
            }
        __syncthreads();
        static_for<NIT>([&](auto itc) {
            constexpr int it = decltype(itc)::value;
            const int idx = lane + 64 * it;
            const int px = idx / VW, cv = (idx - px * VW) * 8;
            const int m = m0 + q * 32 + px;
            if (m < M) {
                const int c = st * P + hC * CW + cv;
                const f32x4 v0 = *reinterpret_cast<const f32x4*>(stage + px * LDS_ + cv);
                const f32x4 v1 = *reinterpret_cast<const f32x4*>(stage + px * LDS_ + cv + 4);
                const f32x4 b0 = *reinterpret_cast<const f32x4*>(s_b3 + c);
                const f32x4 b1 = *reinterpret_cast<const f32x4*>(s_b3 + c + 4);
                float res[8], o[8];
                const u32x4 r = rres[st][it];
                DT<bf16_t>::unpack(make_uint4(r[0], r[1], r[2], r[3]), res);
#pragma unroll
                for (int e = 0; e < 4; ++e) {
                    o[e] = v0[e] + b0[e] + res[e];
                    o[4 + e] = v1[e] + b1[e] + res[4 + e];
                }
                *reinterpret_cast<uint4*>(y + ((size_t)m * C + c)) = DT<bf16_t>::pack(o);
            }
        });
    });
    }
#ifdef FPD_BNECK_TIMING
    STAMP(6);
    if (tid == 0 && bid_in == 0)
        printf("bneck W=%d: setup %lld | phaseA %lld | tile0 %lld | B(9 taps) %lld | a3+C %lld | epilogue %lld | total %lld cycles\n",
               W, stamps[1] - stamps[0], stamps[2] - stamps[1], stamps[3] - stamps[2], stamps[4] - stamps[3],
               stamps[5] - stamps[4], stamps[6] - stamps[5], stamps[6] - stamps[0]);
    if (tid == 0 && bid_in == 0 && acnt == 10)
        printf("  phase A steps: first-stage %lld | pass0 %lld %lld %lld %lld | pass1 %lld %lld %lld %lld | a2 write %lld\n",
               astamp[1] - astamp[0], astamp[2] - astamp[1], astamp[3] - astamp[2], astamp[4] - astamp[3], astamp[5] - astamp[4],
               astamp[6] - astamp[5], astamp[7] - astamp[6], astamp[8] - astamp[7], astamp[9] - astamp[8], stamps[2] - astamp[9]);
#endif
}

template <int P, bool DMA>
__global__ __launch_bounds__(512, 1) void bneck_eval_kernel(const fpd_bneck_t a, const int logW, const int ntiles) {
    bneck_eval_body<P, DMA>(a, logW, (ntiles & 7) == 0, blockIdx.x, gridDim.x, ntiles);
}

template <int P, bool DMA>
__global__ __launch_bounds__(512, 1) void bneck_eval_pair_kernel(const fpd_bneck_t a, const fpd_bneck_t b, const int logWa,
                                                                 const int logWb, const int nblk_a, const int ntiles_a,
                                                                 const int ntiles_b) {
    if ((int)blockIdx.x < nblk_a) bneck_eval_body<P, DMA>(a, logWa, (ntiles_a & 7) == 0, blockIdx.x, nblk_a, ntiles_a);
    else bneck_eval_body<P, DMA>(b, logWb, (ntiles_b & 7) == 0, (int)blockIdx.x - nblk_a, (int)gridDim.x - nblk_a, ntiles_b);
}


static int bneck_block_cap() {
    static int cap = 0;
    if (!cap) {
        const char* e = getenv("FPD_BNECK_BLOCKS");
        cap = e ? atoi(e) : 128;
        if (cap < 8) cap = 8;
    }
    return cap;
}
static int bneck_blocks(int tiles, int cap) {
    if (tiles <= cap) return tiles;
    const int rounds = cdiv(tiles, cap);
    return cdiv(tiles, rounds);
}

template <int P>
size_t bneck_lds_bytes(int H, int W) {
    constexpr int C = 2 * P, LD2 = P + 8, LDX = 72, CW = 32 * (P / 64);
    int logW = 0;
    while ((1 << logW) < W) ++logW;
    const int nrows = 128 >> logW, WP = W + 2;
    const bool whole = (128 % (H * W)) == 0;
    const int irows = whole ? nrows + 2 : 2 * nrows;
    const size_t r2 = std::max({(size_t)2 * P * LD2 * 2, (size_t)2 * (128 + P) * LDX * 2, (size_t)8 * 32 * (CW + 4) * 4});
    return (size_t)(3 * C + 4 * P) * sizeof(float) + (size_t)(irows * WP + 3) * LD2 * 2 + r2;
}

template <int P, bool DMA>
int launch_bneck_pair(const fpd_bneck_t& a, const fpd_bneck_t& b, hipStream_t st) {
    const size_t lds = std::max(bneck_lds_bytes<P>(a.H, a.W), bneck_lds_bytes<P>(b.H, b.W));
    static LdsAttr configured;
    if (int rc_ = configured.ensure(reinterpret_cast<const void*>(&bneck_eval_pair_kernel<P, DMA>), lds)) return rc_;
    int la = 0, lb = 0;
    while ((1 << la) < a.W) ++la;
    while ((1 << lb) < b.W) ++lb;
    const int ta = cdiv(a.N * a.H * a.W, 128), tb = cdiv(b.N * b.H * b.W, 128);
    int na = ta, nb = tb;
    const int cap = bneck_block_cap();
    if (ta + tb > cap) {
        const int capb = std::max(1, (int)((int64_t)cap * tb / (ta + tb)));
        nb = bneck_blocks(tb, capb);
        na = bneck_blocks(ta, std::max(1, cap - nb));
    }
    FPD_LAUNCH((bneck_eval_pair_kernel<P, DMA>), dim3(na + nb), dim3(512), lds, st, a, b, la, lb, na, ta, tb);
    return 0;
}

template <int P, bool DMA>
int launch_bneck(const fpd_bneck_t& a, int logW, hipStream_t st) {
    const size_t lds = bneck_lds_bytes<P>(a.H, a.W);
    static LdsAttr configured;
    if (int rc_ = configured.ensure(reinterpret_cast<const void*>(&bneck_eval_kernel<P, DMA>), lds)) return rc_;
    const int ntiles = cdiv(a.N * a.H * a.W, 128);
    FPD_LAUNCH((bneck_eval_kernel<P, DMA>), dim3(bneck_blocks(ntiles, bneck_block_cap())), dim3(512), lds, st, a, logW, ntiles);
    return 0;
}

}

static bool bneck_in_domain(const fpd_bneck_t& a) {
    if (a.dtype != FPD_BF16 || a.C != 2 * a.P || (a.P != 64 && a.P != 128)) return false;
    if (a.W < 4 || a.W > 64 || (a.W & (a.W - 1)) != 0) return false;
    const int hw = a.H * a.W;
    return hw % 128 == 0 || 128 % hw == 0;
}

int fpd_bneck_fused_launch(const fpd_bneck_t& a, hipStream_t st) {
    if (!bneck_in_domain(a)) return 1;
    int logW = 0;
    while ((1 << logW) < a.W) ++logW;
    return a.P == 128 ? launch_bneck<128, true>(a, logW, st) : launch_bneck<64, true>(a, logW, st);
}

int fpd_bneck_fused_pair_launch(const fpd_bneck_t& a, const fpd_bneck_t& b, hipStream_t st) {
    if (!bneck_in_domain(a) || !bneck_in_domain(b) || a.P != b.P) return 1;
    return a.P == 128 ? launch_bneck_pair<128, true>(a, b, st) : launch_bneck_pair<64, true>(a, b, st);
}

int fpd_bneck_fold_launch(const fpd_bneck_t& a, float* out, hipStream_t st) {
    if (a.C != 2 * a.P || (a.P != 64 && a.P != 128)) return 1;
    if (a.P == 128) FPD_LAUNCH((bneck_fold_kernel<128>), dim3(1), dim3(256), 0, st, a, out);
    else FPD_LAUNCH((bneck_fold_kernel<64>), dim3(1), dim3(256), 0, st, a, out);
    return 0;
}
```

fast-human-pose-estimation.pytorch_amd/executor.py:

```python
import ctypes as C
import os

import torch

from . import graph as G
from . import runtime as R
from .schedule import PhaseSchedule

_EW = {'bnrelu_fwd': R.EW_BNRELU_FWD, 'bnrelu_bwd_r': R.EW_BNRELU_BWD_R, 'bn_bwd_apply': R.EW_BN_BWD_APPLY,
       'maxpool_fwd': R.EW_MAXPOOL_FWD, 'maxpool_bwd': R.EW_MAXPOOL_BWD, 'upadd_fwd': R.EW_UPADD_FWD,
       'sumpool': R.EW_SUMPOOL, 'add': R.EW_ADD, 'relu_mask': R.EW_RELU_MASK, 'dilate2': R.EW_DILATE2}
_ARENA_DTYPE = {'param': torch.float32, 'grad': torch.float32, 'rstat': torch.float32, 'nbt': torch.int64,
                'stats': torch.int64, 'losses': torch.float64, 'image': torch.float32, 'target': torch.float32,
                'weight': torch.float32, 'adam_m': torch.float32, 'adam_v': torch.float32, 'fold': torch.float32,
                'w8': torch.uint8, 'w8s': torch.float32}


def act_torch_dtype(dtype):
    return torch.bfloat16 if dtype == R.BF16 else torch.float32


_STAT_HI, _STAT_LO = float(2 ** 20), float(2 ** 60)


class Arenas:

    def __init__(self, device, dtype, parent=None):
        self.device, self.dtype, self.parent = device, dtype, parent
        self.t = {}

    def alloc(self, name, n):
        dt = _ARENA_DTYPE.get(name, act_torch_dtype(self.dtype))
        n = max(int(n), 4) * (2 if name == 'stats' else 1)
        self.t[name] = torch.zeros(n, dtype=dt, device=self.device)
        return self.t[name]

    def stats_read(self, buf):
        raw = self.view(buf)
        return raw[:, :, 0, :].double() / _STAT_HI + raw[:, :, 1, :].double() / _STAT_LO

    def stats_write(self, buf, values):
        v = values.to(self.device, torch.float64).reshape(buf.shape)
        hi = torch.round(v * _STAT_HI)
        lo = torch.round((v - hi / _STAT_HI) * _STAT_LO)
        self.view(buf).copy_(torch.stack([hi.to(torch.int64), lo.to(torch.int64)], 2))

    def tensor(self, name):
        if name in self.t:
            return self.t[name]
        if self.parent is not None:
            return self.parent.tensor(name)
        raise KeyError(name)

    def ptr(self, buf):
        if buf is None:
            return None
        t = self.tensor(buf.arena)
        return t.data_ptr() + buf.off * t.element_size() * (2 if buf.arena == 'stats' else 1)

    def view(self, buf):
        if buf.arena == 'stats':
            r, two, c = buf.shape
            return self.tensor('stats')[2 * buf.off:2 * (buf.off + buf.numel)].view(r, two, 2, c)
        return self.tensor(buf.arena)[buf.off:buf.off + buf.numel].view(buf.shape)


def _abuf(a):
    return None if a is None else (a.buf if isinstance(a, G.Act) else a)


_WHATIF = frozenset(t for t in os.environ.get('FPD_WHATIF', '').split(',') if t)
if _WHATIF:
    import sys
    sys.stderr.write('[fpd_amd] WARNING: FPD_WHATIF=%s is set: op classes are dropped from the plans -- TIMING ONLY, every result '
                     '(maps, losses, gradients, parameters) of this process is WRONG\n' % ','.join(sorted(_WHATIF)))


def _whatif_drop(op, train):
    k = op.kind
    if k in ('conv2', 'bneck2', 'ew2'):
        sub = op.a
        k = sub.kind
    else:
        sub = op
    dims = getattr(sub, 'dims', None)
    h = dims[1] if dims else 0
    if not train:
        if k not in ('conv', 'bneck', 'head', 'ew', 'stem_fwd'):
            return False
        if h >= 64 and (('t_bneck_big' in _WHATIF and k == 'bneck') or ('t_head' in _WHATIF and k == 'head') or
                        ('t_plain_big' in _WHATIF and k in ('conv', 'ew', 'stem_fwd'))):
            return True
        return ('t_all' in _WHATIF or ('t_big' in _WHATIF and h >= 64) or ('t_mid' in _WHATIF and h == 32) or
                ('t_small' in _WHATIF and h <= 16))
    if k in ('wgrad', 'stem_wgrad', 'wreduce'):
        return ('nowgrad' in _WHATIF or ('nowgrad_small' in _WHATIF and k == 'wgrad' and h <= 16) or
                ('nowgrad_big' in _WHATIF and k == 'wgrad' and h >= 64))
    if k not in ('conv', 'ew', 'stem_fwd'):
        return False
    if k == 'ew' and ('noew' in _WHATIF or ('noapply' in _WHATIF and sub.op == 'bn_bwd_apply')):
        return True
    if k == 'conv' and 'nobigconv' in _WHATIF and h >= 64:
        return True
    if k == 'conv' and h >= 32 and (('no3x3big' in _WHATIF and dims[5] == 3) or ('no1x1big' in _WHATIF and dims[5] == 1)):
        return True
    return ('nobig' in _WHATIF and h >= 64) or ('nomid' in _WHATIF and h == 32) or ('nosmall' in _WHATIF and h <= 16)


class Lowering:

    def __init__(self, arenas, dtype):
        self.A, self.dtype = arenas, dtype
        self.keep = []
        self.use_partials = False
        self.partials, self.partial_elems = {}, 0
        self.fused = set()
        self.reduces = []

    def bn(self, bn):
        s = R.BnT()
        if bn is None:
            s.mode = R.BN_NONE
            return s
        s.mode = R.BN_TRAIN if bn.mode == 'train' else R.BN_EVAL
        s.relu = 1 if bn.relu else 0
        s.eps = G.BN_EPS
        s.stats = self.A.ptr(bn.stats) if bn.mode == 'train' else None
        s.gamma, s.beta = self.A.ptr(bn.gamma), self.A.ptr(bn.beta)
        s.running_mean, s.running_var = self.A.ptr(bn.rmean), self.A.ptr(bn.rvar)
        return s

    def conv(self, op, plain=False):
        s = R.ConvT()
        (s.N, s.H, s.W, s.C, s.K, s.R, s.S, s.stride, s.pad, s.P, s.Q) = op.dims
        s.dtype = self.dtype
        s.epi = R.EPI_BNRELU_BWD if op.epi == 'bnrelu_bwd' else R.EPI_PLAIN
        p = self.A.ptr
        s.x, s.w, s.bias, s.residual, s.y = p(_abuf(op.x)), p(op.w), p(op.bias), p(_abuf(op.residual)), p(_abuf(op.y))
        s.out_stats = p(op.out_stats)
        s.bn = self.bn(op.bn)
        s.epi_x, s.epi_bn, s.epi_stats = p(_abuf(op.epi_x)), self.bn(op.epi_bn), p(op.epi_stats)
        s.wg_partial, s.wg_stride, s.wg_bias, s.wg_count = None, 0, 0, 0
        if not plain and getattr(op, 'fused_wgrad', None) is not None and self.use_partials:
            n = R.lib().fpd_conv_fused_wgrad_partials(C.byref(s))
            if n > 0:
                self._fuse_wgrad(op, s, n)
        if not plain:
            self._fill_fold(op, s)
        if getattr(op, 'w8', None) is not None and not plain:
            f = R.ConvF8T()
            f.c, f.w8, f.w8_scale = s, p(op.w8), p(op.w8s)
            return R.OP_CONV_F8, f
        return R.OP_CONV, s

    def plan_folds(self, ops):
        if os.environ.get('FPD_FOLD_APPLY', '1') == '0':
            return
        l = R.lib()
        members_of = lambda top: [m for m in ((top.a, top.b) if top.kind in ('conv2', 'ew2', 'bneck2') else (top,)) if m is not None]
        for i, op in enumerate(ops):
            if op is None or op.kind not in ('conv', 'conv2'):
                continue
            members = members_of(op)
            cands = [m for m in members if getattr(m, 'fold_apply', None) is not None and not getattr(m.fold_apply, 'folded', False)]
            if not cands or any(getattr(m, 'w8', None) is not None for m in members):
                continue
            early = False
            for m in cands:
                y = _abuf(m.fold_apply.y)
                own = (id(m), id(m.fold_apply), id(getattr(m, 'fold_wgrad', None)))
                m.fold_other_readers = False
                for j, top in enumerate(ops):
                    if top is None:
                        continue
                    for o in members_of(top):
                        if id(o) in own or not any(_abuf(t) is y for t in o.acts_in()):
                            continue
                        if j < i:
                            early = True
                        m.fold_other_readers = True
            if early:
                continue
            if op.kind == 'conv2':
                ps = R.ConvPairT()
                ps.a, ps.b = self.conv(op.a, plain=True)[1], self.conv(op.b, plain=True)[1]
                ok = l.fpd_conv_pair_fold_supported(C.byref(ps)) == 1
            else:
                ok = l.fpd_conv_fold_supported(C.byref(self.conv(op, plain=True)[1])) == 1
            if ok:
                for m in cands:
                    m.fold_active = True
                    m.fold_apply.folded = True

    def _fill_fold(self, op, s):
        if not getattr(op, 'fold_active', False):
            return
        ap, p = op.fold_apply, self.A.ptr
        assert ap.add is None and _abuf(ap.y) is _abuf(op.x), 'fold: the apply must produce exactly this operand'
        s.x = p(_abuf(ap.dy))
        s.fold_x, s.fold_bn, s.fold_stats = p(_abuf(ap.x)), self.bn(ap.bn), p(ap.bstats)
        s.fold_dgamma, s.fold_dbeta = p(ap.dgamma), p(ap.dbeta)
        skip = getattr(op, 'fused_active', False) and not getattr(op, 'fold_other_readers', False)
        s.fold_out = None if skip else p(_abuf(ap.y))

    def _fuse_wgrad(self, op, s, n):
        fw = op.fused_wgrad
        numel = fw.dw.numel
        assert numel == s.C * s.K, (numel, s.C, s.K)
        stride = (numel + s.C + 63) // 64 * 64
        self.partials[id(fw)] = [s, fw.dw, numel, stride, n, self.partial_elems, fw.dbias, s.C]
        self.partial_elems += n * stride
        s.wg_bias = 1 if fw.dbias is not None else 0
        s.wg_count = n
        self.fused.add(id(fw))
        op.fused_active = True

    def wquant(self, entries):
        ents = []
        for w, q, sc in entries:
            e = R.WquantEntryT()
            e.w, e.w8, e.scale = self.A.ptr(w), self.A.ptr(q), self.A.ptr(sc)
            e.K, e.RSC = w.shape[0], w.numel // w.shape[0]
            ents.append(e)
        s = R.TableT()
        s.table, s.n, s.dtype, s.max_elems = self._table(ents, R.WquantEntryT), len(ents), self.dtype, 0
        return R.OP_WQUANT, s

    def bneck(self, op):
        s = R.BneckT()
        (s.N, s.H, s.W, s.C, s.P) = op.dims
        s.dtype = self.dtype
        p = self.A.ptr
        s.x, s.y = p(_abuf(op.x)), p(_abuf(op.y))
        s.w1, s.b1, s.w2, s.b2, s.w3, s.b3 = p(op.w1), p(op.b1), p(op.w2), p(op.b2), p(op.w3), p(op.b3)
        s.bn1, s.bn2, s.bn3 = self.bn(op.bn1), self.bn(op.bn2), self.bn(op.bn3)
        s.folded = p(getattr(op, 'folded', None))
        return R.OP_BNECK, s

    def head(self, op):
        s = R.HeadT()
        (s.N, s.H, s.W, s.C, s.J) = op.dims
        s.dtype = self.dtype
        p = self.A.ptr
        s.y0, s.x, s.score, s.next = p(_abuf(op.y0)), p(_abuf(op.x)), p(_abuf(op.score)), p(_abuf(op.next))
        s.w_fc, s.b_fc, s.w_score, s.b_score = p(op.w_fc), p(op.b_fc), p(op.w_score), p(op.b_score)
        s.w_fc2, s.b_fc2, s.w_score2, s.b_score2 = p(op.w_fc2), p(op.b_fc2), p(op.w_score2), p(op.b_score2)
        s.bn = self.bn(op.bn)
        s.folded = p(getattr(op, 'folded', None))
        return R.OP_HEAD, s

    def wgrad(self, op):
        if id(op) in self.fused:
            return R.OP_NOP, R.MemsetT()
        s = R.WgradT()
        (s.N, s.H, s.W, s.C, s.K, s.R, s.S, s.stride, s.pad, s.P, s.Q) = op.dims
        s.dtype = self.dtype
        p = self.A.ptr
        s.x, s.dy, s.dw, s.dbias = p(_abuf(op.x)), p(_abuf(op.dy)), p(op.dw), p(op.dbias)
        s.bn = self.bn(op.bn)
        s.partial, s.partial_stride = None, 0
        if self.use_partials:
            n = R.lib().fpd_wgrad_num_partials(C.byref(s))
            if n > 0:
                numel = op.dw.numel
                stride = (numel + s.K + 63) // 64 * 64
                self.partials[id(op)] = [s, op.dw, numel, stride, n, self.partial_elems, op.dbias, s.K]
                self.partial_elems += n * stride
        return R.OP_WGRAD, s

    def wreduce(self, op):
        if not any(id(w) in self.partials for w in op.wgrads):
            return R.OP_NOP, R.MemsetT()
        t = R.TableT()
        self.reduces.append((op, t))
        return R.OP_WREDUCE, t

    def finish_partials(self):
        if not self.partials:
            return
        ws = torch.empty(self.partial_elems, dtype=torch.float32, device=self.A.device)
        self.keep.append(ws)
        for s, dw, numel, stride, n, off, dbias, nbias in self.partials.values():
            if isinstance(s, R.ConvT):
                s.wg_partial, s.wg_stride = ws.data_ptr() + 4 * off, stride
            else:
                s.partial, s.partial_stride = ws.data_ptr() + 4 * off, stride
        for op, t in self.reduces:
            ents, mx = [], 0
            for w in op.wgrads:
                rec = self.partials.get(id(w))
                if rec is None:
                    continue
                s, dw, numel, stride, n, off, dbias, nbias = rec
                base = ws.data_ptr() + 4 * off
                e = R.WreduceEntryT()
                e.partial, e.dw, e.n, e.stride, e.count = base, self.A.ptr(dw), numel, stride, n
                ents.append(e)
                if dbias is not None:
                    e = R.WreduceEntryT()
                    e.partial, e.dw, e.n, e.stride, e.count = base + 4 * numel, self.A.ptr(dbias), nbias, stride, n
                    ents.append(e)
                mx = max(mx, numel)
            t.table, t.n, t.dtype, t.max_elems = self._table(ents, R.WreduceEntryT), len(ents), self.dtype, mx

    def stem(self, op):
        s = R.StemT()
        (s.N, s.H, s.W, s.K, s.P, s.Q) = op.dims
        s.dtype = self.dtype
        p = self.A.ptr
        s.x = p(op.image)
        if op.kind == 'stem_fwd':
            s.w, s.bias, s.y, s.out_stats = p(op.w), p(op.bias), p(_abuf(op.y)), p(op.out_stats)
            return R.OP_STEM_FWD, s
        s.dy, s.dw, s.dbias = p(_abuf(op.dy)), p(op.dw), p(op.dbias)
        s.partial, s.partial_stride = None, 0
        if self.use_partials:
            n = R.lib().fpd_stem_wgrad_num_partials(C.byref(s))
            if n > 0:
                numel = op.dw.numel
                stride = (numel + s.K + 63) // 64 * 64
                self.partials[id(op)] = [s, op.dw, numel, stride, n, self.partial_elems, op.dbias, s.K]
                self.partial_elems += n * stride
        return R.OP_STEM_WGRAD, s

    def ew(self, op):
        if getattr(op, 'folded', False):
            return R.OP_NOP, R.MemsetT()
        s = R.EwT()
        s.op, s.dtype = _EW[op.op], self.dtype
        (s.N, s.H, s.W, s.C) = op.dims
        p = self.A.ptr
        s.x, s.x2, s.dy, s.add, s.y = p(_abuf(op.x)), p(_abuf(op.x2)), p(_abuf(op.dy)), p(_abuf(op.add)), p(_abuf(op.y))
        s.out_stats, s.bstats, s.dgamma, s.dbeta = p(op.out_stats), p(op.bstats), p(op.dgamma), p(op.dbeta)
        s.bn = self.bn(op.bn)
        return R.OP_EW, s

    def _table(self, entries, cls):
        arr = (cls * len(entries))(*entries)
        raw = torch.frombuffer(bytearray(bytes(arr)), dtype=torch.uint8).to(self.A.device)
        self.keep.append(raw)
        return raw.data_ptr()

    def bnupd(self, op):
        ents = []
        for bn in op.bns:
            e = R.BnupdEntryT()
            e.stats, e.running_mean, e.running_var = self.A.ptr(bn.stats), self.A.ptr(bn.rmean), self.A.ptr(bn.rvar)
            e.num_batches_tracked = self.A.ptr(bn.nbt)
            e.count, e.momentum, e.C = float(bn.count), G.BN_MOMENTUM, bn.C
            ents.append(e)
        s = R.TableT()
        s.table, s.n, s.dtype, s.max_elems = self._table(ents, R.BnupdEntryT), len(ents), self.dtype, 0
        return R.OP_BNUPD, s

    def wprep(self, entries):
        ents, mx = [], 0
        for w, wf, wb in entries:
            e = R.WprepEntryT()
            e.w, e.w_fwd, e.w_bwd = self.A.ptr(w), self.A.ptr(wf), self.A.ptr(wb)
            (e.K, e.R, e.S, e.C) = w.shape
            mx = max(mx, w.numel)
            ents.append(e)
        s = R.TableT()
        s.table, s.n, s.dtype, s.max_elems = self._table(ents, R.WprepEntryT), len(ents), self.dtype, mx
        return R.OP_WPREP, s

    def memset(self, arena_name, off=0, n=None):
        t = self.A.tensor(arena_name)
        n = t.numel() - off if n is None else n
        s = R.MemsetT()
        s.ptr, s.bytes = t.data_ptr() + off * t.element_size(), n * t.element_size()
        return R.OP_MEMSET, s

    def op(self, op):
        if _WHATIF and _whatif_drop(op, getattr(self, 'train', True)):
            return R.OP_NOP, R.MemsetT()
        if op.kind == 'conv2':
            s = R.ConvPairT()
            s.a, s.b = self.conv(op.a, plain=True)[1], self.conv(op.b, plain=True)[1]
            if (self.use_partials and getattr(op.a, 'fused_wgrad', None) is not None and
                    getattr(op.b, 'fused_wgrad', None) is not None):
                na, nb = C.c_int32(0), C.c_int32(0)
                R.check(R.lib().fpd_conv_pair_fused_wgrad_partials(C.byref(s), C.byref(na), C.byref(nb)), 'fpd_conv_pair_fused_wgrad_partials')
                if na.value > 0 and nb.value > 0:
                    self._fuse_wgrad(op.a, s.a, na.value)
                    self._fuse_wgrad(op.b, s.b, nb.value)
            self._fill_fold(op.a, s.a)
            self._fill_fold(op.b, s.b)
            return R.OP_CONV_PAIR, s
        if op.kind == 'ew2':
            fa, fb = getattr(op.a, 'folded', False), getattr(op.b, 'folded', False)
            if fa or fb:
                return (R.OP_NOP, R.MemsetT()) if (fa and fb) else self.ew(op.b if fa else op.a)
            s = R.EwPairT()
            s.a, s.b = self.ew(op.a)[1], self.ew(op.b)[1]
            return R.OP_EW_PAIR, s
        if op.kind == 'bneck2':
            s = R.BneckPairT()
            s.a, s.b = self.bneck(op.a)[1], self.bneck(op.b)[1]
            return R.OP_BNECK_PAIR, s
        if op.kind == 'head':
            return self.head(op)
        if op.kind == 'head_fold':
            return R.OP_HEAD_FOLD, self.head(op.target)[1]
        if op.kind == 'bneck_fold':
            return R.OP_BNECK_FOLD, self.bneck(op.target)[1]
        if op.kind == 'affsum':
            s = R.AffsumT()
            (s.N, s.H, s.W, s.C) = op.dims
            s.dtype, s.relu, s.nterms = self.dtype, 1 if op.relu else 0, len(op.terms)
            assert len(op.terms) <= R.AFFSUM_MAX and op.out_stats is None
            for j, (t, bn, up) in enumerate(op.terms):
                s.t[j].x, s.t[j].bn, s.t[j].up = self.A.ptr(_abuf(t)), self.bn(bn), up
            s.y = self.A.ptr(_abuf(op.y))
            return R.OP_AFFSUM, s
        if op.kind == 'nchw2nhwc':
            s = R.LayoutT()
            (s.N, s.C, s.H, s.W) = op.dims
            s.src, s.dst, s.dtype = self.A.ptr(op.image), self.A.ptr(_abuf(op.y)), self.dtype
            return R.OP_NCHW2NHWC, s
        if op.kind == 'wreduce':
            return self.wreduce(op)
        if op.kind == 'grad_ready':
            return R.OP_NOP, R.MemsetT()
        return {'conv': self.conv, 'bneck': self.bneck, 'wgrad': self.wgrad, 'stem_fwd': self.stem, 'stem_wgrad': self.stem, 'ew': self.ew,
                'bnupd': self.bnupd}[op.kind](op)


class ModelState:

    def __init__(self, table, device, dtype):
        self.table, self.device, self.dtype = table, device, dtype
        self.A = Arenas(device, dtype)
        for name in ('param', 'rstat', 'nbt'):
            self.A.alloc(name, table.sizes[name])
        self.A.alloc('grad', table.sizes['param'])


class GraphInstance:

    def __init__(self, state, cfg, batch, height, width, train, image=None, share_weights_with=None):
        self.state, self.train = state, train
        self._wlp_owner = share_weights_with
        self.dtype = state.dtype
        env = os.environ.get
        if cfg.get('arch') == 'hrnet':
            self.g = G.HRNetGraph(state.table, cfg['extra'], cfg['J'], batch, height, width, train,
                                  wlp_is_master=(self.dtype == R.F32),
                                  wgrad_batch=int(env('FPD_WGRAD_BATCH')) if env('FPD_WGRAD_BATCH') else None,
                                  fp8=bool(cfg.get('fp8', False)))
        else:
            self.g = G.HourglassGraph(state.table, cfg['F'], cfg['S'], cfg['J'], batch, height, width, train,
                                      num_blocks=cfg.get('num_blocks', 1), wlp_is_master=(self.dtype == R.F32),
                                      fuse_bneck=(self.dtype == R.BF16 and not train and env('FPD_FUSE_BNECK', '1') != '0'),
                                      pair_branches=env('FPD_PAIR', '1') != '0', fuse_head=env('FPD_FUSE_HEAD', '1') != '0',
                                      wgrad_batch=int(env('FPD_WGRAD_BATCH')) if env('FPD_WGRAD_BATCH') else None)
        self.A = Arenas(state.device, self.dtype, parent=state.A)
        self.low = Lowering(self.A, self.dtype)
        self.low.train = train
        self.plan = R.Plan()
        self.rng = {}
        self.graphs = {}
        self._image_ext = image
        self._finalized = False
        self.mid_ops = []
        self.mid_native = []

    def _schedule(self, name, ir_ops):
        b, e = self.rng[name]
        assert e - b == len(ir_ops), (name, b, e, len(ir_ops))
        if not self.lanes_enabled or not any(o is not None and o.lane for o in ir_ops):
            return
        sch = PhaseSchedule([((o.lane or 0), o.accesses()) if o is not None else (0, None) for o in ir_ops], self.g.n_lanes)
        for k in range(len(ir_ops)):
            if sch.lanes[k] or sch.waits[k]:
                self.plan.set_schedule(b + k, sch.lanes[k], [b + w for w in sch.waits[k]])
        self.schedules[name] = sch

    def finalize(self):
        g = self.g
        ops = g.fwd + self.mid_ops + g.bwd
        self.lanes_enabled = os.environ.get('FPD_LANES', '1') != '0'
        self.schedules = {}
        delay = int(os.environ.get('FPD_REUSE_DELAY', '400')) if self.lanes_enabled else 0
        if not self.train:
            delay = 0
        act = G.plan_memory(ops, reuse_delay=delay)
        self.act_elems = act
        self.A.alloc('act', act)
        self.A.alloc('stats', g.stats_size)
        if self._wlp_owner is not None:
            o = self._wlp_owner
            assert o.g.wlp_size == g.wlp_size and o.g.fold_size == g.fold_size and not self.train
            self.A.t['wlp'] = o.A.t['wlp']
            self.A.t['fold'] = o.A.t['fold']
        else:
            self.A.alloc('wlp', g.wlp_size)
            self.A.alloc('fold', g.fold_size)
        if self._image_ext is not None:
            self.A.t['image'] = self._image_ext
        else:
            self.A.alloc('image', g.N * 3 * g.H * g.W)
        p = self.plan
        b = len(p)
        p.add(*self.low.memset('stats'))
        entries = []
        for k in self.state.table.conv_keys():
            if k in g.MASTER_ONLY:
                continue
            wf, wb = g.wfwd.get(k), g.wbwd.get(k)
            if wf is not None or wb is not None:
                entries.append((self.state.table[k], wf, wb))
        if entries:
            p.add(*self.low.wprep(entries))
        w8 = getattr(g, 'w8', None)
        if w8:
            self.A.alloc('w8', g.w8_size)
            self.A.alloc('w8s', g.w8s_size)
            p.add(*self.low.wquant([(self.state.table[k], q, sc) for k, (q, sc) in w8.items()]))
        for op in g.fwd:
            for sub in ((op.a, op.b) if op.kind == 'bneck2' else (op,)):
                if sub.kind == 'bneck' and getattr(sub, 'folded', None) is not None:
                    p.add(*self.low.op(G.Op('bneck_fold', target=sub)))
                if sub.kind == 'head' and getattr(sub, 'folded', None) is not None:
                    p.add(*self.low.op(G.Op('head_fold', target=sub)))
        self.rng['prep'] = (b, len(p))
        b = len(p)
        self.op_index = {}
        for op in g.fwd:
            self.op_index[id(op)] = p.add(*self.low.op(op))
        self.rng['fwd'] = (b, len(p))
        self._schedule('fwd', list(g.fwd))
        b = len(p)
        for fn in self.mid_native:
            fn(p)
        self.rng['mid'] = (b, len(p))
        if self.train:
            b = len(p)
            p.add(*self.low.memset('grad'))
            self.low.use_partials = True
            bwd_ir = [op for op in g.bwd if op.kind != 'seed']
            self.low.plan_folds(bwd_ir)
            lowered = [self.low.op(op) for op in bwd_ir]
            self.low.finish_partials()
            self.bucket_ops = {}
            for ir, (code, st) in zip(bwd_ir, lowered):
                k = self.op_index[id(ir)] = p.add(code, st)
                if ir.kind == 'grad_ready':
                    self.bucket_ops[ir.bucket] = k
                    p.mark_event(k)
            self.rng['bwd'] = (b, len(p))
            self._schedule('bwd', [None] + bwd_ir)
        self._finalized = True
        return self

    def run(self, name, stream=None):
        gid = self.graphs.get(name)
        if gid is not None:
            self.plan.replay(gid, stream)
            return
        b, e = self.rng[name]
        self.plan.run(b, e, stream)

    def capture(self, names, cap_stream):
        torch.cuda.synchronize()
        with torch.cuda.stream(cap_stream):
            for n in names:
                b, e = self.rng[n]
                self.graphs[n] = self.plan.capture(b, e, C.c_void_p(cap_stream.cuda_stream))
        torch.cuda.synchronize()

    def image(self):
        return self.A.tensor('image').view(self.g.N, 3, self.g.H, self.g.W)

    def calibrate_running_stats(self):
        assert self.train
        torch.cuda.synchronize()
        for bn in self.g.bns:
            st = self.A.stats_read(bn.stats).sum(0)
            mean = st[0] / bn.count
            var = (st[1] / bn.count - mean * mean).clamp_min(0) * (bn.count / max(bn.count - 1, 1))
            self.A.view(bn.rmean).copy_(mean.float())
            self.A.view(bn.rvar).copy_(var.float())

    def output_view(self, i):
        return self.A.view(self.g.outputs[i].buf)

    def out_grad_view(self, i):
        return self.A.view(self.g.out_grads[i].buf)


class FusedFPDStep:

    def __init__(self, student_state, student_cfg, teacher_state, teacher_cfg, batch, height, width, alpha,
                 lr=2.5e-4, betas=(0.9, 0.999), eps=1e-8, world_size=1, adam=None, teacher_chunks=None,
                 use_target_weight=(True, True)):
        dev = student_state.device
        self.use_w = (bool(use_target_weight[0]), bool(use_target_weight[1]))
        self.dtype = student_state.dtype
        self.alpha, self.world_size = alpha, world_size
        self.B, self.J = batch, student_cfg['J']
        self.teacher = None
        self.teachers = []
        self.tmap = [None, None]
        if teacher_state is not None:
            assert teacher_state.dtype == self.dtype
            if teacher_chunks is None:
                teacher_chunks = 1
            while batch % teacher_chunks:
                teacher_chunks -= 1
            cb = batch // teacher_chunks
            self.teacher = GraphInstance(teacher_state, teacher_cfg, cb, height, width, train=False).finalize()
            self.teachers = [self.teacher] + [
                GraphInstance(teacher_state, teacher_cfg, cb, height, width, train=False,
                              share_weights_with=self.teacher).finalize() for _ in range(1, teacher_chunks)]
            self.teacher.run('prep')
            nt = self.teacher.g.outputs[-1].numel * teacher_chunks
            self.tmap = [torch.zeros(nt, dtype=act_torch_dtype(self.dtype), device=dev) for _ in range(2)]
            self.t_streams = [torch.cuda.Stream(device=dev) for _ in range(teacher_chunks)]
            self.t_stream = self.t_streams[0]
            self.ev_t = [torch.cuda.Event(), torch.cuda.Event()]
            self.ev_chunk = [torch.cuda.Event() for _ in range(teacher_chunks)]
        self._k_t = self._k_s = 0
        self._late_teacher_wait = True
        self.student = GraphInstance(student_state, student_cfg, batch, height, width, train=True)
        g = self.student.g
        self.hh, self.hw = g.outputs[0].shape[1:3]
        A = self.student.A
        A.alloc('target', self.B * self.J * self.hh * self.hw)
        A.alloc('weight', self.B * self.J)
        if self.use_w[0] != self.use_w[1]:
            A.t['weight_kd'] = torch.ones(self.B * self.J, dtype=torch.float32, device=dev)
        if not self.use_w[0]:
            A.tensor('weight').fill_(1.0)
        A.alloc('losses', 4)
        self.student.mid_ops = [G.Op('loss', extra_in=list(g.outputs), extra_out=list(g.out_grads))]
        self.student.mid_native = [lambda plan: self._add_loss(plan, 0)]
        self.student.finalize()
        b = len(self.student.plan)
        self._add_loss(self.student.plan, 1)
        self.student.rng['mid1'] = (b, len(self.student.plan))
        n = student_state.table.sizes['param']
        self.n_param = n
        if adam is not None:
            self.m, self.v, self.lr_dev, self.step_dev = adam.m, adam.v, adam.lr_dev, adam.step_dev
            betas, eps = adam.param_groups[0]['betas'], adam.param_groups[0]['eps']
        else:
            self.m = torch.zeros(n, dtype=torch.float32, device=dev)
            self.v = torch.zeros(n, dtype=torch.float32, device=dev)
            self.lr_dev = torch.full((1,), lr, dtype=torch.float32, device=dev)
            self.step_dev = torch.zeros(1, dtype=torch.int64, device=dev)
        self.betas, self.eps = betas, eps
        a = R.AdamT()
        a.n = n
        pa = student_state.A
        a.param, a.grad = pa.tensor('param').data_ptr(), pa.tensor('grad').data_ptr()
        a.m, a.v = self.m.data_ptr(), self.v.data_ptr()
        a.param_lp = None
        a.lr, a.beta1, a.beta2, a.eps = lr, betas[0], betas[1], eps
        a.bias_corr1 = a.bias_corr2 = 1.0
        a.grad_scale = 1.0
        a.lr_dev, a.step_dev = self.lr_dev.data_ptr(), self.step_dev.data_ptr()
        self._adam_args = a
        b = len(self.student.plan)
        self.student.plan.add(R.OP_ADAM, a)
        self.student.rng['adam'] = (b, len(self.student.plan))
        self._dist_work = None

    def enable_metric(self, min_slots=0):
        m = getattr(self, 'metric', None)
        if m is None or m.slots < min_slots:
            assert m is None or m.pending() == 0, 'drain() the metric ring before enlarging it'
            from .lib.core.evaluate import DeviceAccuracy
            g, A = self.student.g, self.student.A
            self.metric = DeviceAccuracy(self.B, self.J, self.hh, self.hw, self.dtype, self.student.state.device,
                                         slots=max(4096, int(min_slots))).bind(
                A.ptr(g.outputs[-1].buf), A.tensor('target').data_ptr(), A.tensor('losses').data_ptr())
        return self.metric

    def _add_loss(self, plan, slot):
        A, g = self.student.A, self.student.g
        plan.add(*self.student.low.memset('losses'))
        s = R.LossT()
        s.B, s.J, s.H, s.W, s.S, s.dtype = self.B, self.J, self.hh, self.hw, len(g.outputs), self.dtype
        s.target_nchw, s.alpha = 1, self.alpha
        for i, (o, d) in enumerate(zip(g.outputs, g.out_grads)):
            s.out[i] = A.ptr(o.buf)
            s.dout[i] = A.ptr(d.buf)
        if self.teacher is not None:
            s.teacher = self.tmap[slot].data_ptr()
        else:
            s.teacher = A.ptr(g.outputs[-1].buf)
        s.target, s.weight = A.tensor('target').data_ptr(), A.tensor('weight').data_ptr()
        s.weight_kd = A.tensor('weight_kd').data_ptr() if 'weight_kd' in A.t else None
        s.losses = A.tensor('losses').data_ptr()
        s.grad_scale = 1.0 / self.world_size
        plan.add(R.OP_LOSS, s)

    def set_batch(self, inp, target, target_weight):
        self.student.image().copy_(inp, non_blocking=True)
        self.student.A.tensor('target').view(target.shape).copy_(target, non_blocking=True)
        if self.use_w[0]:
            self.student.A.tensor('weight').view(target_weight.shape).copy_(target_weight, non_blocking=True)
        elif self.use_w[1]:
            self.student.A.tensor('weight_kd').view(target_weight.shape).copy_(target_weight, non_blocking=True)
        self._last_inp = inp

    def teacher_async(self, inp=None):
        if self.teacher is None:
            return
        slot = self._k_t % 2
        cur = torch.cuda.current_stream()
        n = len(self.teachers)
        for k in reversed(range(n)):
            t, T = self.teachers[k], self.t_streams[k]
            T.wait_stream(cur)
            with torch.cuda.stream(T):
                cb = t.g.N
                if inp is not None:
                    t.image().copy_(inp[k * cb:(k + 1) * cb], non_blocking=True)
                t.run('fwd')
                o = t.g.outputs[-1].buf
                self.tmap[slot][k * o.numel:(k + 1) * o.numel].copy_(t.A.tensor('act')[o.off:o.off + o.numel])
                if k:
                    self.ev_chunk[k].record(T)
                else:
                    for j in range(1, n):
                        T.wait_event(self.ev_chunk[j])
                    self.ev_t[slot].record(T)
        self._k_t += 1

    def student_step(self, allreduce=None):
        s = self.student
        slot = self._k_s % 2
        late = self._late_teacher_wait
        if self.teacher is not None:
            assert self._k_t > self._k_s, 'teacher_async() must be submitted before student_step()'
            if not late:
                torch.cuda.current_stream().wait_event(self.ev_t[slot])
        if self._dist_work is not None:
            self._dist_work()
            self._dist_work = None
            s.run('adam')
        s.run('prep')
        s.run('fwd')
        if self.teacher is not None and late:
            torch.cuda.current_stream().wait_event(self.ev_t[slot])
        s.run('mid' if slot == 0 else 'mid1')
        if getattr(self, 'metric', None) is not None:
            self.metric.enqueue()
        s.run('bwd')
        if allreduce is not None:
            self._dist_work = allreduce(self.student.state.A.tensor('grad'), self.grad_buckets())
        else:
            s.run('adam')
        self._k_s += 1

    def grad_buckets(self):
        s = self.student
        n = self.n_param
        if s.graphs.get('bwd') is not None or not getattr(s, 'bucket_ops', None):
            return [(0, n, None)]
        table = s.state.table
        out = []
        for b, (lo, hi) in enumerate(table.buckets):
            op = s.bucket_ops.get(b)
            if hi <= lo:
                continue
            assert op is not None, 'gradient bucket %d [%d, %d) has no completion op: it would never be all-reduced' % (b, lo, hi)
            out.append((lo, hi, (lambda stream, op=op: s.plan.wait_op(op, C.c_void_p(stream.cuda_stream)))))
        cover = sorted((lo, hi) for lo, hi, _ in out)
        assert cover and cover[0][0] == 0 and cover[-1][1] == n and all(a[1] == b[0] for a, b in zip(cover, cover[1:])), \
            'gradient buckets %r do not tile the arena [0, %d)' % (cover, n)
        return out

    def enable_graphs(self):
        cap = torch.cuda.Stream(device=self.student.state.device)
        for t in self.teachers:
            t.capture(['fwd'], cap)
        self.student.capture(['prep', 'fwd', 'mid', 'mid1', 'bwd', 'adam'], cap)

    def step(self, allreduce=None):
        self.teacher_async(getattr(self, '_last_inp', None))
        self.student_step(allreduce)

    def run_pipelined(self, n_steps, allreduce=None):
        inp = getattr(self, '_last_inp', None)
        self.teacher_async(inp)
        for i in range(n_steps):
            if i + 1 < n_steps:
                self.teacher_async(None)
            self.student_step(allreduce)
        self.flush()

    def flush(self):
        if self._dist_work is not None:
            self._dist_work()
            self._dist_work = None
            self.student.run('adam')

    def launches_per_step(self):
        def count(inst, name):
            b, e = inst.rng[name]
            return sum(1 for k in range(b, e) if inst.plan.op_type(k) != R.OP_NOP)
        out = {'teacher_fwd': count(self.teacher, 'fwd') * len(self.teachers)} if self.teacher is not None else {}
        for ph in ('prep', 'fwd', 'mid', 'bwd', 'adam'):
            out['student_' + ph] = count(self.student, ph)
        out['total'] = sum(out.values())
        return out

    def losses(self):
        l = self.student.A.tensor('losses')[:2].cpu()
        pose, kd = float(l[0]), float(l[1])
        return pose, kd, (1 - self.alpha) * pose + self.alpha * kd

    def set_lr(self, lr):
        self.lr_dev.fill_(lr)
```

fast-human-pose-estimation.pytorch_amd/graph.py:

```python
import os
from collections import OrderedDict

BN_EPS = 1e-5
BN_MOMENTUM = 0.1
STATS_REPLICAS = int(os.environ.get('FPD_STATS_REPLICAS', '4'))
WGRAD_LANES = 1
LANE_LEVELS = 0
FOLD_APPLY = os.environ.get('FPD_FOLD_APPLY', '1') != '0'
WREDUCE_MODE = os.environ.get('FPD_WREDUCE_MODE', 'lag')
WGRAD_BATCH = 8


class Buf:
    __slots__ = ('arena', 'off', 'shape', 'name')

    def __init__(self, arena, off, shape, name=''):
        self.arena, self.off, self.shape, self.name = arena, off, tuple(shape), name

    @property
    def numel(self):
        n = 1
        for s in self.shape:
            n *= s
        return n

    def __repr__(self):
        return 'Buf(%s+%s %s %s)' % (self.arena, self.off, self.shape, self.name)


class Act:
    __slots__ = ('shape', 'buf', 'stats', 'producer', 'grad', 'name', 'persistent', 'needs_grad', 'apply_op')

    def __init__(self, shape, name=''):
        self.shape = tuple(shape)
        self.buf = None
        self.stats = None
        self.producer = None
        self.grad = None
        self.name = name
        self.persistent = False
        self.needs_grad = True
        self.apply_op = None

    @property
    def numel(self):
        n, h, w, c = self.shape
        return n * h * w * c


class BN:
    __slots__ = ('name', 'mode', 'relu', 'C', 'gamma', 'beta', 'rmean', 'rvar', 'nbt', 'stats', 'count')

    def __init__(self, name, mode, C, gamma, beta, rmean, rvar, nbt, stats=None, relu=True):
        self.name, self.mode, self.C, self.relu = name, mode, C, relu
        self.gamma, self.beta, self.rmean, self.rvar, self.nbt, self.stats = gamma, beta, rmean, rvar, nbt, stats
        self.count = 0


def f8_conv_domain(dims):
    n, h, w, C, K, R, S, stride, pad, P, Q = dims
    if stride != 1 or R != S or R not in (1, 3) or pad != (R - 1) // 2 or w > 128 or w < 2:
        return False
    if C % 32 or K % 8 or C > 512:
        return False
    bk = 64 if C % 64 == 0 else 32
    return (max(1, 128 // w) + R - 1) * w * (bk // 8) <= 2048


class Op:

    def __init__(self, kind, **kw):
        self.kind = kind
        self.lane = None
        self.__dict__.update(kw)

    def accesses(self):
        def b(a):
            return a.buf if isinstance(a, Act) else a

        def bn_bufs(bn):
            if bn is None:
                return []
            return [bn.gamma, bn.beta] + ([bn.stats] if bn.mode == 'train' else [bn.rmean, bn.rvar])
        k = self.kind
        if k in ('conv2', 'bneck2', 'ew2'):
            (ra, wa), (rb, wb) = self.a.accesses(), self.b.accesses()
            return ra + rb, wa + wb
        if k == 'conv':
            rd = [b(self.x), self.w, self.bias, b(self.residual), b(self.epi_x)] + bn_bufs(self.bn) + bn_bufs(self.epi_bn)
            rd += [getattr(self, 'w8', None), getattr(self, 'w8s', None)]
            wr = [b(self.y), self.out_stats, self.epi_stats]
            fw = getattr(self, 'fused_wgrad', None)
            if fw is not None and getattr(self, 'fused_active', False):
                wr += [fw.dw, fw.dbias]
            fa = getattr(self, 'fold_apply', None)
            if fa is not None and getattr(self, 'fold_active', False):
                rd += [b(fa.x), b(fa.dy), fa.bstats] + bn_bufs(fa.bn)
                wr += [b(fa.y), fa.dgamma, fa.dbeta]
        elif k == 'head':
            rd = [b(self.y0), b(self.x), self.w_fc, self.b_fc, self.w_score, self.b_score, self.w_fc2, self.b_fc2,
                  self.w_score2, self.b_score2] + bn_bufs(self.bn)
            wr = [b(self.score), b(self.next)]
        elif k == 'bneck':
            rd = [b(self.x), self.w1, self.b1, self.w2, self.b2, self.w3, self.b3] + bn_bufs(self.bn1) + \
                bn_bufs(self.bn2) + bn_bufs(self.bn3)
            wr = [b(self.y)]
        elif k == 'wgrad':
            rd = [b(self.x), b(self.dy)] + bn_bufs(self.bn)
            wr = [self.dw, self.dbias]
        elif k == 'affsum':
            rd = [b(t) for t, _, _ in self.terms]
            for _, bn, _ in self.terms:
                rd += bn_bufs(bn)
            wr = [b(self.y), self.out_stats]
        elif k == 'nchw2nhwc':
            rd, wr = [self.image], [b(self.y)]
        elif k == 'wreduce':
            rd, wr = list(self.bufs), list(self.bufs)
        elif k == 'grad_ready':
            rd, wr = [self.region], []
        elif k == 'stem_fwd':
            rd, wr = [self.image, self.w, self.bias], [b(self.y), self.out_stats]
        elif k == 'stem_wgrad':
            rd, wr = [self.image, b(self.dy)], [self.dw, self.dbias]
        elif k == 'ew':
            rd = [b(self.x), b(self.x2), b(self.dy), b(self.add)] + bn_bufs(self.bn)
            wr = [b(self.y), self.out_stats, self.bstats, self.dgamma, self.dbeta]
        else:
            return None
        return [x for x in rd if x is not None], [x for x in wr if x is not None]

    def acts_in(self):
        if self.kind in ('conv2', 'bneck2', 'ew2'):
            return self.a.acts_in() + self.b.acts_in()
        if self.kind == 'head':
            return [t for t in (self.y0, self.x) if t is not None]
        fa = getattr(self, 'fold_apply', None)
        folded = [t for t in (fa.x, fa.dy) if isinstance(t, Act)] if fa is not None else []
        return [getattr(self, f) for f in ('x', 'x2', 'dy', 'add', 'residual', 'epi_x') if
                isinstance(getattr(self, f, None), Act)] + [a for a in getattr(self, 'extra_in', []) if a is not None] + folded

    def acts_out(self):
        if self.kind in ('conv2', 'bneck2', 'ew2'):
            return self.a.acts_out() + self.b.acts_out()
        if self.kind == 'head':
            return [t for t in (self.score, self.next) if t is not None]
        return [getattr(self, f) for f in ('y',) if isinstance(getattr(self, f, None), Act)] + \
               [a for a in getattr(self, 'extra_out', []) if a is not None]


class ParamTable:

    def __init__(self, keys, bucket_of=None):
        self.keys = list(keys)
        self.entries = OrderedDict()
        self.logical = dict(self.keys)
        self.sizes = {'param': 0, 'rstat': 0, 'nbt': 0}
        self.bucket = {k: (bucket_of(k) if bucket_of else 0) for k, _ in self.keys}
        placed = {}
        self.buckets = []
        for k, shp in sorted(self.keys, key=lambda ks: self.bucket[ks[0]]):
            if k.endswith('num_batches_tracked'):
                arena = 'nbt'
            elif k.endswith('running_mean') or k.endswith('running_var'):
                arena = 'rstat'
            else:
                arena = 'param'
            n = 1
            for s in shp:
                n *= s
            phys = (shp[0], shp[2], shp[3], shp[1]) if len(shp) == 4 else tuple(shp)
            off = self.sizes[arena]
            placed[k] = Buf(arena, off, phys, k)
            step = 4 if arena != 'nbt' else 2
            self.sizes[arena] = off + (n + step - 1) // step * step
            if arena == 'param':
                b = self.bucket[k]
                while len(self.buckets) <= b:
                    self.buckets.append([off, off])
                self.buckets[b][1] = self.sizes[arena]
        for k, _ in self.keys:
            self.entries[k] = placed[k]
        self.buckets = [tuple(b) for b in self.buckets]

    def __getitem__(self, k):
        return self.entries[k]

    def grad(self, k):
        b = self.entries[k]
        return Buf('grad', b.off, b.shape, 'grad:' + k)

    def conv_keys(self):
        return [k for k, shp in self.keys if len(shp) == 4]

    def trainable_keys(self):
        return [k for k, b in self.entries.items() if b.arena == 'param']

    def grad_bucket(self, b):
        lo, hi = self.buckets[b]
        return Buf('grad', lo, (hi - lo,), 'grad:bucket%d' % b)


def hourglass_bucket_of(num_stacks):
    def f(key):
        p = key.split('.')
        if p[0] in ('hg', 'res', 'fc', 'score', 'fc_', 'score_'):
            return num_stacks - 1 - int(p[1])
        return num_stacks - 1
    return f


def plan_memory(ops, align=64, reuse_delay=0):
    last = {}
    for i, op in enumerate(ops):
        for a in op.acts_in() + op.acts_out():
            last[id(a)] = i
    free = []
    limbo = []
    top = 0

    def alloc(n):
        nonlocal top
        n = (n + align - 1) // align * align
        best = None
        for j, (o, s) in enumerate(free):
            if s >= n and (best is None or s < free[best][1]):
                best = j
        if best is not None:
            o, s = free.pop(best)
            if s > n:
                free.append((o + n, s - n))
            return o, n
        o = top
        top += n
        return o, n

    def release(o, n):
        free.append((o, n))
        free.sort()
        merged = []
        for o2, s2 in free:
            if merged and merged[-1][0] + merged[-1][1] == o2:
                merged[-1] = (merged[-1][0], merged[-1][1] + s2)
            else:
                merged.append((o2, s2))
        free[:] = merged

    sizes = {}
    for i, op in enumerate(ops):
        while limbo and limbo[0][0] + reuse_delay <= i:
            _, o, n = limbo.pop(0)
            release(o, n)
        for a in op.acts_in() + op.acts_out():
            if a.buf is None:
                o, n = alloc(a.numel)
                a.buf = Buf('act', o, a.shape, a.name)
                sizes[id(a)] = n
        seen = set()
        for a in op.acts_in() + op.acts_out():
            if id(a) in seen:
                continue
            seen.add(id(a))
            if last[id(a)] == i and not a.persistent and id(a) in sizes:
                limbo.append((i, a.buf.off, sizes.pop(id(a))))
    return top


class _OpList(list):

    def __init__(self, owner):
        super().__init__()
        self.owner = owner

    def append(self, op):
        if op.lane is None:
            op.lane = self.owner._lane
        super().append(op)


class HourglassGraph:

    def __init__(self, params, num_feats, num_stacks, num_joints, batch, height, width, train, num_blocks=1,
                 depth=4, wlp_is_master=True, lane_levels=None, wgrad_batch=None, fuse_bneck=False, pair_branches=True, fuse_head=True):
        self.p = params
        self.F, self.S, self.J = num_feats, num_stacks, num_joints
        self.N, self.H, self.W = batch, height, width
        self.train, self.num_blocks, self.depth = train, num_blocks, depth
        self.wlp_is_master = wlp_is_master
        self.fuse_bneck = fuse_bneck and not train
        self.fuse_head = fuse_head and self.fuse_bneck
        self.pair_branches = pair_branches
        self._pair_op = None
        self._pair_ew = None
        self.stats_size = 0
        self.fold_size = 0
        self.wlp_size = 0
        self.wfwd, self.wbwd = {}, {}
        self._lane = 0
        self.lane_levels = LANE_LEVELS if lane_levels is None else lane_levels
        self.wgrad_batch = WGRAD_BATCH if wgrad_batch is None else wgrad_batch
        self._setup()

    MASTER_ONLY = ('conv1.weight',)

    def _setup(self):
        self._wg_pending = []
        self.n_lanes = 1 + self.depth + WGRAD_LANES
        self.fwd, self.bwd = _OpList(self), _OpList(self)
        self.bns = []
        self.image = Buf('image', 0, (self.N, 3, self.H, self.W), 'image')
        self.outputs = []
        self._bn_pending = {}
        self._bn_uses = {}
        for k in self.p.conv_keys():
            if k in self.MASTER_ONLY:
                continue
            b = self.p[k]
            if not self.wlp_is_master:
                self.wfwd[k] = self._wlp(b)
            if self.train:
                K, R, S, C = b.shape
                self.wbwd[k] = self._wlp(Buf('param', 0, (C, R, S, K)))
        self.build_forward()
        if self.train:
            self.build_backward()

    def _w8(self, wkey):
        tab = self.__dict__.setdefault('w8', {})
        if wkey not in tab:
            b = self.p[wkey]
            q = Buf('w8', getattr(self, 'w8_size', 0), b.shape, 'w8:' + wkey)
            self.w8_size = q.off + (b.numel + 15) // 16 * 16
            sc = Buf('w8s', getattr(self, 'w8s_size', 0), (b.shape[0],), 'w8s:' + wkey)
            self.w8s_size = sc.off + (b.shape[0] + 3) // 4 * 4
            tab[wkey] = (q, sc)
        return tab[wkey]

    def _wlp(self, like):
        off = self.wlp_size
        self.wlp_size += (like.numel + 7) // 8 * 8
        return Buf('wlp', off, like.shape, 'wlp')

    def _stats(self, C, name=''):
        off = self.stats_size
        self.stats_size += STATS_REPLICAS * 2 * C
        return Buf('stats', off, (STATS_REPLICAS, 2, C), name)

    def _bn(self, name, C):
        g = self.p
        mode = 'train' if self.train else 'eval'
        return BN(name, mode, C, g[name + '.weight'], g[name + '.bias'], g[name + '.running_mean'],
                  g[name + '.running_var'], g[name + '.num_batches_tracked'])

    def conv(self, x, name, bn=None, residual=None, pad=0, sink=None, stride=1):
        wkey = name + '.weight'
        K, R, S, C = self.p[wkey].shape
        n, h, w, c = x.shape
        assert c == C, (name, x.shape, self.p[wkey].shape)
        y = Act((n, (h + 2 * pad - R) // stride + 1, (w + 2 * pad - S) // stride + 1, K), name)
        wbuf = self.p[wkey] if self.wlp_is_master else self.wfwd[wkey]
        bkey = name + '.bias' if (name + '.bias') in self.p.entries else None
        op = Op('conv', x=x, w=wbuf, wkey=wkey, bias=self.p[bkey] if bkey else None, bkey=bkey, residual=residual,
                y=y, out_stats=None, bn=bn, epi='plain', epi_x=None, epi_bn=None, epi_stats=None,
                dims=(n, h, w, C, K, R, S, stride, pad, y.shape[1], y.shape[2]))
        y.producer = op
        op.w8 = op.w8s = None
        if getattr(self, 'fp8', False) and sink is None and f8_conv_domain(op.dims):
            op.w8, op.w8s = self._w8(wkey)
            op.w_master = self.p[wkey]
        if bn is not None:
            self._use_bn(x, bn)
        (self.fwd if sink is None else sink).append(op)
        return y

    def _use_bn(self, x, bn):
        if bn.mode == 'train':
            if x.stats is None:
                x.stats = self._stats(x.shape[3], 'stats:' + x.name)
                prod = x.producer
                assert prod is not None and hasattr(prod, 'out_stats'), 'no stats producer for ' + x.name
                prod.out_stats = x.stats
            bn.stats = x.stats
            key = (id(x), bn.name)
            self._bn_uses[key] = self._bn_uses.get(key, 0) + 1
            if not any(b.name == bn.name for b in self.bns):
                self.bns.append(bn)
        bn.count = x.shape[0] * x.shape[1] * x.shape[2]
        return bn

    def ew(self, opname, shape_large, y_shape, name, **kw):
        y = Act(y_shape, name)
        op = Op('ew', op=opname, dims=tuple(shape_large), y=y, out_stats=None, x=kw.get('x'), x2=kw.get('x2'),
                dy=None, add=None, bstats=None, dgamma=None, dbeta=None, bn=kw.get('bn'))
        y.producer = op
        self.fwd.append(op)
        return y

    def maxpool(self, x, name):
        n, h, w, c = x.shape
        return self.ew('maxpool_fwd', x.shape, (n, h // 2, w // 2, c), name, x=x)

    def upadd(self, a, b, name):
        assert a.shape[1] == 2 * b.shape[1] and a.shape[2] == 2 * b.shape[2] and a.shape[3] == b.shape[3]
        return self.ew('upadd_fwd', a.shape, a.shape, name, x=a, x2=b)

    def bottleneck(self, x, p, sink=None):
        c_in = x.shape[3]
        planes = self.p[p + 'conv1.weight'].shape[0]
        if self._fused(x, p):
            n, h, w, _ = x.shape
            y = Act(x.shape, p + 'out')
            wb = (lambda k: self.p[k]) if self.wlp_is_master else (lambda k: self.wfwd[k])
            fold = Buf('fold', self.fold_size, (3 * c_in + 4 * planes,), 'fold:' + p)
            self.fold_size += 3 * c_in + 4 * planes
            op = Op('bneck', x=x, y=y, dims=(n, h, w, c_in, planes), folded=fold,
                    w1=wb(p + 'conv1.weight'), b1=self.p[p + 'conv1.bias'], w2=wb(p + 'conv2.weight'),
                    b2=self.p[p + 'conv2.bias'], w3=wb(p + 'conv3.weight'), b3=self.p[p + 'conv3.bias'],
                    bn1=self._bn(p + 'bn1', c_in), bn2=self._bn(p + 'bn2', planes), bn3=self._bn(p + 'bn3', planes))
            y.producer = op
            (self.fwd if sink is None else sink).append(op)
            return y
        t = self.conv(x, p + 'conv1', bn=self._bn(p + 'bn1', c_in), sink=sink)
        t = self.conv(t, p + 'conv2', bn=self._bn(p + 'bn2', planes), pad=1, sink=sink)
        skip = x
        if (p + 'downsample.0.weight') in self.p.entries:
            assert sink is None
            skip = self.conv(x, p + 'downsample.0')
        return self.conv(t, p + 'conv3', bn=self._bn(p + 'bn3', planes), residual=skip, sink=sink)

    def _fused(self, x, p):
        planes = self.p[p + 'conv1.weight'].shape[0]
        return (self.fuse_bneck and self.bneck_fusable(x.shape, planes) and
                (p + 'downsample.0.weight') not in self.p.entries)

    def bottleneck_pair(self, xa, pa, xb, pb):
        la, lb = [], []
        ya = self.bottleneck(xa, pa, sink=la)
        yb = self.bottleneck(xb, pb, sink=lb)
        assert len(la) == len(lb) and len(la) in (1, 3)
        for oa, ob in zip(la, lb):
            self.fwd.append(Op('conv2' if oa.kind == 'conv' else 'bneck2', a=oa, b=ob))
        return ya, yb

    @staticmethod
    def bneck_fusable(shape, planes):
        n, h, w, c = shape
        return (c == 2 * planes and planes in (64, 128) and 4 <= w <= 64 and w & (w - 1) == 0 and
                ((h * w) % 128 == 0 or 128 % (h * w) == 0))

    def residual_seq(self, x, p, nb):
        for b in range(nb):
            x = self.bottleneck(x, '%s%d.' % (p, b))
        return x

    def hour_glass(self, x, p, n):
        q = '%s%d.' % (p, n - 1)
        nb = self.num_blocks
        laned = n > self.depth - self.lane_levels
        pa, pb = q + '0.0.', q + '1.0.'
        n_, h_, w_, c_ = x.shape
        if (self.pair_branches and nb == 1 and not laned and
                self._fused(x, pa) == self._fused(Act((n_, h_ // 2, w_ // 2, c_)), pb) and
                (pa + 'downsample.0.weight') not in self.p.entries and (pb + 'downsample.0.weight') not in self.p.entries):
            low = self.maxpool(x, q + 'pool')
            up1, low = self.bottleneck_pair(x, pa, low, pb)
        else:
            outer = self._lane
            if laned:
                self._lane = n
            up1 = self.residual_seq(x, q + '0.', nb)
            self._lane = outer
            low = self.maxpool(x, q + 'pool')
            low = self.residual_seq(low, q + '1.', nb)
        if n > 1:
            low = self.hour_glass(low, p, n - 1)
        else:
            low = self.residual_seq(low, q + '3.', nb)
        low = self.residual_seq(low, q + '2.', nb)
        return self.upadd(up1, low, q + 'upadd')

    def build_forward(self):
        K = self.p['conv1.weight'].shape[0]
        P, Q = (self.H + 6 - 7) // 2 + 1, (self.W + 6 - 7) // 2 + 1
        x = Act((self.N, P, Q, K), 'stem')
        op = Op('stem_fwd', image=self.image, w=self.p['conv1.weight'], bias=self.p['conv1.bias'], y=x, out_stats=None,
                dims=(self.N, self.H, self.W, K, P, Q))
        x.producer = op
        self.fwd.append(op)
        bn1 = self._bn('bn1', K)
        self._use_bn(x, bn1)
        x = self.ew('bnrelu_fwd', x.shape, x.shape, 'stem_act', x=x, bn=bn1)
        x = self.residual_seq(x, 'layer1.', 1)
        x = self.maxpool(x, 'pool1')
        x = self.residual_seq(x, 'layer2.', 1)
        x = self.residual_seq(x, 'layer3.', 1)
        ch = x.shape[3]
        for i in range(self.S):
            y = self.hour_glass(x, 'hg.%d.hg.' % i, self.depth)
            y = self.residual_seq(y, 'res.%d.' % i, self.num_blocks)
            if self.fuse_head and ch == 256 and self.J == 16:
                wb = (lambda k: self.p[k]) if self.wlp_is_master else (lambda k: self.wfwd[k])
                last = i == self.S - 1
                score = Act((y.shape[0], y.shape[1], y.shape[2], self.J), 'score.%d' % i)
                score.persistent = True
                nxt = None if last else Act(x.shape, 'stack%d.out' % i)
                fold = Buf('fold', self.fold_size, (3 * ch + 32,), 'fold:head%d' % i)
                self.fold_size += 3 * ch + 32
                op = Op('head', y0=y, x=None if last else x, score=score, next=nxt, dims=(y.shape[0], y.shape[1], y.shape[2], ch, self.J),
                        w_fc=wb('fc.%d.0.weight' % i), b_fc=self.p['fc.%d.0.bias' % i],
                        w_score=wb('score.%d.weight' % i), b_score=self.p['score.%d.bias' % i],
                        w_fc2=None if last else wb('fc_.%d.weight' % i), b_fc2=None if last else self.p['fc_.%d.bias' % i],
                        w_score2=None if last else wb('score_.%d.weight' % i),
                        b_score2=None if last else self.p['score_.%d.bias' % i],
                        bn=self._bn('fc.%d.1' % i, ch), folded=fold)
                score.producer = op
                if nxt is not None:
                    nxt.producer = op
                self.fwd.append(op)
                self.outputs.append(score)
                x = nxt
                continue
            y = self.conv(y, 'fc.%d.0' % i)
            fcbn = self._bn('fc.%d.1' % i, ch)
            score = self.conv(y, 'score.%d' % i, bn=fcbn)
            score.persistent = True
            self.outputs.append(score)
            if i < self.S - 1:
                fcbn2 = self._bn('fc.%d.1' % i, ch)
                t = self.conv(y, 'fc_.%d' % i, bn=fcbn2, residual=x)
                x = self.conv(score, 'score_.%d' % i, residual=t)
        if self.train:
            self.fwd.append(Op('bnupd', bns=list(self.bns)))

    def _contribute(self, t):
        prev = t.grad
        t.grad = Act(t.shape, 'd:' + t.name)
        return prev, t.grad

    def _contribute_identity(self, t, g):
        if t.grad is None:
            t.grad = g
        else:
            prev = t.grad
            t.grad = Act(t.shape, 'd:' + t.name)
            self.bwd.append(Op('ew', op='add', dims=t.shape, x=prev, x2=g, y=t.grad, dy=None, add=None,
                               out_stats=None, bstats=None, dgamma=None, dbeta=None, bn=None, lane=self._home(t)))

    def _home(self, t):
        return t.producer.lane if t.producer is not None and t.producer.lane is not None else 0

    def _bn_backward_contribution(self, x, bn, make_dgrad):
        key = (id(x), bn.name)
        pend = self._bn_pending.get(key)
        bstats = self._stats(bn.C, 'bstats:' + bn.name)
        if pend is None:
            dz = Act(x.shape, 'dz:' + bn.name)
            make_dgrad(dz, None, bstats)
            pend = {'dz': dz, 'left': self._bn_uses[key]}
            self._bn_pending[key] = pend
        else:
            make_dgrad(pend['dz'], pend['dz'], bstats)
        pend['left'] -= 1
        if pend['left'] == 0:
            add, out = self._contribute(x)
            apply = Op('ew', op='bn_bwd_apply', dims=x.shape, x=x, x2=None, dy=pend['dz'], add=add, y=out,
                       out_stats=None, bstats=bstats, dgamma=self.p.grad(bn.name + '.weight'),
                       dbeta=self.p.grad(bn.name + '.bias'), bn=bn, lane=self._home(x))
            if add is None:
                out.apply_op = apply
            c = self._pair_ew
            if c is None or (apply.lane or 0) != 0:
                self.bwd.append(apply)
            elif c.a is None:
                c.a = apply
                self.bwd.append(c)
            else:
                assert c.b is None
                c.b = apply
            del self._bn_pending[key]

    def build_backward(self):
        self.out_grads = []
        for o in self.outputs:
            o.grad = Act(o.shape, 'd:' + o.name)
            o.grad.persistent = True
            self.out_grads.append(o.grad)
        self.bwd.append(Op('seed', extra_in=list(self.outputs), extra_out=list(self.out_grads)))
        self._cur_bucket, self._wg_bucket = None, []
        for op in reversed(self.fwd):
            self._lane = op.lane
            bk = self._op_bucket(op)
            if bk is not None and bk != self._cur_bucket:
                if self._cur_bucket is not None:
                    assert bk > self._cur_bucket, 'gradient buckets must complete in increasing order'
                    self._lane = 0
                    self._close_bucket(self._cur_bucket)
                    self._lane = op.lane
                self._cur_bucket = bk
            if len(self._wg_pending) >= self.wgrad_batch and op.lane == 0:
                self._flush_wgrads()
            if op.kind == 'conv':
                self._conv_backward(op)
            elif op.kind == 'conv2':
                c = self._pair_op = Op('conv2', a=None, b=None)
                e = self._pair_ew = Op('ew2', a=None, b=None)
                self._conv_backward(op.a)
                self._conv_backward(op.b)
                self._pair_op = self._pair_ew = None
                for cont in (c, e):
                    if cont.a is not None and cont.b is None:
                        cont.a.lane = cont.lane
                        self.bwd[self.bwd.index(cont)] = cont.a
            elif op.kind == 'stem_fwd':
                dy = op.y.grad
                sw = Op('stem_wgrad', image=self.image, dy=dy, dw=self.p.grad('conv1.weight'),
                        dbias=self.p.grad('conv1.bias'), dims=op.dims, lane=1 + self.depth)
                self._wg_pending.append(sw)
            elif op.kind == 'ew':
                self._ew_backward(op)
            elif op.kind == 'affsum':
                self._affsum_backward(op)
        self._lane = 0
        self._close_bucket(self._cur_bucket if self._cur_bucket is not None else 0)
        assert not self._bn_pending, 'unfinished BN backward: %r' % list(self._bn_pending)

    def _op_bucket(self, op):
        if op.kind in ('conv2', 'bneck2', 'ew2'):
            return self._op_bucket(op.a)
        key = getattr(op, 'wkey', None)
        if key is None and op.kind == 'stem_fwd':
            key = 'conv1.weight'
        if key is None and getattr(op, 'bn', None) is not None:
            key = op.bn.name + '.weight'
        if key is None and op.kind == 'affsum':
            names = [bn.name for _, bn, _ in op.terms if bn is not None]
            key = names[0] + '.weight' if names else None
        return None if key is None else self.p.bucket[key]

    def _close_bucket(self, b):
        self._flush_wgrads(b, reduce=True)
        self.bwd.append(Op('grad_ready', bucket=b, region=self.p.grad_bucket(b), lane=1 + self.depth))

    def _flush_wgrads(self, b=None, reduce=None):
        def emit_reduce():
            if self._wg_bucket:
                bufs = [x for w in self._wg_bucket for x in (w.dw, w.dbias) if x is not None]
                self.bwd.append(Op('wreduce', bucket=self._cur_bucket if b is None else b, wgrads=list(self._wg_bucket), bufs=bufs,
                                   lane=1 + self.depth))
                self._wg_bucket = []
        if WREDUCE_MODE == 'lag' and self._wg_pending:
            emit_reduce()
        for w in reversed(self._wg_pending):
            self.bwd.append(w)
            if w.kind in ('wgrad', 'stem_wgrad'):
                self._wg_bucket.append(w)
        self._wg_pending = []
        if (WREDUCE_MODE == 'batch') if reduce is None else reduce:
            emit_reduce()

    def _emit_dgrad(self, op):
        c = self._pair_op
        if c is None:
            self.bwd.append(op)
        elif c.a is None:
            c.a = op
            self.bwd.append(c)
        else:
            assert c.b is None
            c.b = op

    def _conv_backward(self, op):
        dy = op.y.grad
        if dy is None:
            return
        x = op.x
        self._wg_pending.append(Op('wgrad', x=x, dy=dy, dw=self.p.grad(op.wkey), dbias=self.p.grad(op.bkey) if op.bkey else None,
                                   bn=op.bn, dims=op.dims, lane=1 + self.depth))
        if op.residual is not None:
            self._contribute_identity(op.residual, dy)
        if not x.needs_grad:
            return
        n, h, w, C, K, R, S, stride, pad, P, Q = op.dims
        ddims = (n, P, Q, K, C, R, S, 1, R - 1 - pad, h, w)
        if stride == 2:
            assert h == 2 * P and w == 2 * Q, 'stride-2 data gradient needs even input dims, got %dx%d' % (h, w)
            dil = Act((n, h, w, K), 'dil:' + op.wkey)
            self.bwd.append(Op('ew', op='dilate2', dims=(n, h, w, K), x=dy, x2=None, dy=None, add=None, y=dil,
                               out_stats=None, bstats=None, dgamma=None, dbeta=None, bn=None))
            dy, ddims = dil, (n, h, w, K, C, R, S, 1, R - 1 - pad, h, w)
        else:
            assert stride == 1
        wb = self.wbwd[op.wkey]
        if op.bn is not None:
            wg = self._wg_pending[-1]

            def make(dz, add, bstats, op=op, dy=dy, x=x):
                d = Op('conv', x=dy, w=wb, wkey=op.wkey, bias=None, bkey=None, residual=add, y=dz,
                       out_stats=None, bn=None, epi='bnrelu_bwd', epi_x=x, epi_bn=op.bn, epi_stats=bstats,
                       dims=ddims)
                if R == 1 and stride == 1 and dy is op.y.grad and any(w is wg for w in self._wg_pending):
                    d.fused_wgrad = wg
                ap = getattr(op.y.grad, 'apply_op', None)
                if FOLD_APPLY and ap is not None and stride == 1 and dy is op.y.grad and (ap.lane or 0) == (self._lane or 0):
                    d.fold_apply = ap
                    d.fold_wgrad = wg
                self._emit_dgrad(d)
            self._bn_backward_contribution(x, op.bn, make)
        else:
            add, out = self._contribute(x)
            self._emit_dgrad(Op('conv', x=dy, w=wb, wkey=op.wkey, bias=None, bkey=None, residual=add, y=out,
                                out_stats=None, bn=None, epi='plain', epi_x=None, epi_bn=None, epi_stats=None, dims=ddims,
                                lane=self._home(x) if add is not None else None))

    def _affsum_backward(self, op):
        dy = op.y.grad
        if dy is None:
            return

        def ew(name, dims, **kw):
            f = dict(x=None, x2=None, dy=None, add=None, y=None, out_stats=None, bstats=None, dgamma=None, dbeta=None, bn=None)
            f.update(kw)
            o = Op('ew', op=name, dims=tuple(dims), **f)
            self.bwd.append(o)
            return o
        g = dy
        fused = None
        if op.relu:
            g = Act(op.y.shape, 'g:' + op.y.name)
            if True:
                fused = next((t for t, bn, up in op.terms if up == 1 and bn is not None and bn.mode == 'train' and t.needs_grad), None)
            if fused is None:
                ew('relu_mask', op.y.shape, x=op.y, dy=dy, y=g)
        for t, bn, up in sorted(op.terms, key=lambda tm: tm[0] is not fused):
            if not t.needs_grad:
                continue
            gj = g
            f = up
            while f > 1:
                nxt = Act((gj.shape[0], gj.shape[1] // 2, gj.shape[2] // 2, gj.shape[3]), 'gs:' + t.name)
                ew('sumpool', gj.shape, x=gj, y=nxt)
                gj, f = nxt, f // 2
            if bn is None:
                self._contribute_identity(t, gj)
                continue
            if bn.mode != 'train':
                raise AssertionError('backward through an eval-mode BN term')
            bstats = self._stats(bn.C, 'bstats:' + bn.name)
            if t is fused:
                ew('bnrelu_bwd_r', t.shape, x=t, x2=op.y, dy=dy, y=g, bstats=bstats, bn=bn)
            else:
                ew('bnrelu_bwd_r', t.shape, x=t, dy=gj, y=None, bstats=bstats, bn=bn)
            add, out = self._contribute(t)
            ew('bn_bwd_apply', t.shape, x=t, dy=gj, add=add, y=out, bstats=bstats, dgamma=self.p.grad(bn.name + '.weight'),
               dbeta=self.p.grad(bn.name + '.bias'), bn=bn)

    def _ew_backward(self, op):
        dy = op.y.grad
        if dy is None:
            return
        if op.op == 'maxpool_fwd':
            add, out = self._contribute(op.x)
            self.bwd.append(Op('ew', op='maxpool_bwd', dims=op.dims, x=op.x, x2=None, dy=dy, add=add, y=out,
                               out_stats=None, bstats=None, dgamma=None, dbeta=None, bn=None))
        elif op.op == 'upadd_fwd':
            self._contribute_identity(op.x, dy)
            add, out = self._contribute(op.x2)
            self.bwd.append(Op('ew', op='sumpool', dims=op.dims, x=dy, x2=None, dy=None, add=add, y=out,
                               out_stats=None, bstats=None, dgamma=None, dbeta=None, bn=None))
        elif op.op == 'bnrelu_fwd':
            x, bn = op.x, op.bn

            def make(dz, add, bstats, dy=dy, x=x, bn=bn):
                assert add is None
                self.bwd.append(Op('ew', op='bnrelu_bwd_r', dims=x.shape, x=x, x2=None, dy=dy, add=None, y=dz,
                                   out_stats=None, bstats=bstats, dgamma=None, dbeta=None, bn=bn))
            self._bn_backward_contribution(x, bn, make)
        else:
            raise AssertionError(op.op)


HRNET_EXPANSION = {'BASIC': 1, 'BOTTLENECK': 4}


def hrnet_bucket_of(key):
    p = key.split('.')[0]
    return {'final_layer': 0, 'stage4': 0, 'transition3': 1, 'stage3': 1, 'transition2': 2, 'stage2': 2}.get(p, 3)


class HRNetGraph(HourglassGraph):

    MASTER_ONLY = ()

    def __init__(self, params, extra, num_joints, batch, height, width, train, wlp_is_master=True, wgrad_batch=None,
                 fp8=False):
        self.p = params
        self.fp8 = bool(fp8) and not wlp_is_master
        self.extra, self.J = extra, num_joints
        self.S = 1
        self.N, self.H, self.W = batch, height, width
        self.train, self.depth = train, 4
        self.wlp_is_master = wlp_is_master
        self.fuse_bneck = self.fuse_head = False
        self.pair_branches = False
        self._pair_op = self._pair_ew = None
        self.stats_size = self.fold_size = self.wlp_size = 0
        self.wfwd, self.wbwd = {}, {}
        self._lane = 0
        self.lane_levels = 0
        self.wgrad_batch = WGRAD_BATCH if wgrad_batch is None else wgrad_batch
        self._setup()

    def _bnx(self, name, C, relu):
        bn = self._bn(name, C)
        bn.relu = relu
        return bn

    def affsum(self, terms, name, relu=True):
        t0, _, f0 = terms[0]
        n, h, w, c = t0.shape
        shape = (n, h * f0, w * f0, c)
        for t, bn, f in terms:
            assert (t.shape[0], t.shape[1] * f, t.shape[2] * f, t.shape[3]) == shape, (name, t.shape, f, shape)
            if bn is not None:
                self._use_bn(t, bn)
        y = Act(shape, name)
        op = Op('affsum', terms=list(terms), y=y, relu=relu, out_stats=None, dims=shape, extra_in=[t for t, _, _ in terms])
        y.producer = op
        self.fwd.append(op)
        return y

    def block(self, x, p, kind, stride=1):
        planes = self.p[p + 'conv1.weight'].shape[0]
        if kind == 'BASIC':
            t = self.conv(x, p + 'conv1', pad=1, stride=stride)
            t = self.conv(t, p + 'conv2', bn=self._bnx(p + 'bn1', planes, True), pad=1)
            tail = (t, self._bnx(p + 'bn2', planes, False), 1)
        else:
            t = self.conv(x, p + 'conv1')
            t = self.conv(t, p + 'conv2', bn=self._bnx(p + 'bn1', planes, True), pad=1, stride=stride)
            t = self.conv(t, p + 'conv3', bn=self._bnx(p + 'bn2', planes, True))
            tail = (t, self._bnx(p + 'bn3', 4 * planes, False), 1)
        if (p + 'downsample.0.weight') in self.p.entries:
            d = self.conv(x, p + 'downsample.0', stride=stride)
            skip = (d, self._bnx(p + 'downsample.1', d.shape[3], False), 1)
        else:
            skip = (x, None, 1)
        return self.affsum([tail, skip], p + 'out')

    def hr_module(self, xs, p, sc, multi_scale_output):
        nb = len(xs)
        ys = []
        for i in range(nb):
            y = xs[i]
            for b in range(sc['NUM_BLOCKS'][i]):
                y = self.block(y, '%sbranches.%d.%d.' % (p, i, b), sc['BLOCK'])
            ys.append(y)
        if nb == 1:
            return ys
        outs = []
        for i in range(nb if multi_scale_output else 1):
            terms = []
            for j in range(nb):
                q = '%sfuse_layers.%d.%d.' % (p, i, j)
                if j == i:
                    terms.append((ys[j], None, 1))
                elif j > i:
                    t = self.conv(ys[j], q + '0')
                    terms.append((t, self._bnx(q + '1', t.shape[3], False), 2 ** (j - i)))
                else:
                    t, bn = ys[j], None
                    for k in range(i - j):
                        t = self.conv(t, '%s%d.0' % (q, k), bn=bn, pad=1, stride=2)
                        bn = self._bnx('%s%d.1' % (q, k), t.shape[3], k != i - j - 1)
                    terms.append((t, bn, 1))
            terms.sort(key=lambda tm: tm[2])
            outs.append(self.affsum(terms, '%sfuse%d' % (p, i)))
        return outs

    def transition(self, ys, p, pre, cur):
        xs = []
        for i, c in enumerate(cur):
            q = '%s%d.' % (p, i)
            if i < len(pre):
                if c != pre[i]:
                    t = self.conv(ys[-1], q + '0', pad=1)
                    xs.append(self.affsum([(t, self._bnx(q + '1', c, False), 1)], q + 'out'))
                else:
                    xs.append(ys[i])
            else:
                t, bn = ys[-1], None
                nlay = i + 1 - len(pre)
                for j in range(nlay):
                    t = self.conv(t, '%s%d.0' % (q, j), bn=bn, pad=1, stride=2)
                    bn = self._bnx('%s%d.1' % (q, j), t.shape[3], True)
                bn.relu = False
                xs.append(self.affsum([(t, bn, 1)], q + 'out'))
        return xs

    def build_forward(self):
        x0 = Act((self.N, self.H, self.W, 3), 'image_nhwc')
        x0.needs_grad = False
        op = Op('nchw2nhwc', image=self.image, y=x0, dims=(self.N, 3, self.H, self.W), extra_out=[])
        x0.producer = op
        self.fwd.append(op)
        t = self.conv(x0, 'conv1', pad=1, stride=2)
        t = self.conv(t, 'conv2', bn=self._bnx('bn1', 64, True), pad=1, stride=2)
        x = self.affsum([(t, self._bnx('bn2', 64, False), 1)], 'stem')
        for b in range(4):
            x = self.block(x, 'layer1.%d.' % b, 'BOTTLENECK')
        chans = [[c * HRNET_EXPANSION[self.extra[s]['BLOCK']] for c in self.extra[s]['NUM_CHANNELS']]
                 for s in ('STAGE2', 'STAGE3', 'STAGE4')]
        ys, pre = [x], [256]
        for si, sname in enumerate(('STAGE2', 'STAGE3', 'STAGE4')):
            sc = self.extra[sname]
            xs = self.transition(ys, 'transition%d.' % (si + 1), pre, chans[si])
            for m in range(sc['NUM_MODULES']):
                last = sname == 'STAGE4' and m == sc['NUM_MODULES'] - 1
                xs = self.hr_module(xs, 'stage%d.%d.' % (si + 2, m), sc, not last)
            ys, pre = xs, chans[si]
        k = self.extra.get('FINAL_CONV_KERNEL', 1)
        out = self.conv(ys[0], 'final_layer', pad=1 if k == 3 else 0)
        out.persistent = True
        self.outputs.append(out)
        if self.train:
            self.fwd.append(Op('bnupd', bns=list(self.bns)))
```

fast-human-pose-estimation.pytorch_amd/runtime.py:

```python
import ctypes as C
import os

_HERE = os.path.dirname(os.path.abspath(__file__))
LIB_PATH = os.environ.get('FPD_AMD_LIB') or os.path.join(_HERE, 'csrc', 'libfpd_amd.so')

F32, BF16 = 0, 1
BN_NONE, BN_TRAIN, BN_EVAL = 0, 1, 2
EPI_PLAIN, EPI_BNRELU_BWD = 0, 1
BACKEND_MFMA, BACKEND_NAIVE, BACKEND_MFMA_GENERIC = 0, 1, 2
(EW_BNRELU_FWD, EW_BNRELU_BWD_R, EW_BN_BWD_APPLY, EW_MAXPOOL_FWD, EW_MAXPOOL_BWD, EW_UPADD_FWD, EW_SUMPOOL,
 EW_ADD, EW_RELU_MASK, EW_DILATE2) = range(10)
(OP_CONV, OP_WGRAD, OP_STEM_FWD, OP_STEM_WGRAD, OP_EW, OP_LOSS, OP_ADAM, OP_MEMSET, OP_WPREP, OP_BNUPD,
 OP_WREDUCE, OP_BNECK, OP_BNECK_FOLD, OP_CONV_PAIR, OP_BNECK_PAIR, OP_EW_PAIR, OP_PCK, OP_HEAD, OP_HEAD_FOLD,
 OP_NOP, OP_AFFSUM, OP_NCHW2NHWC, OP_CONV_F8, OP_WQUANT) = range(24)
AFFSUM_MAX = 4
MAX_STACKS = 8
MAXC = 512

_i32, _i64, _f32, _f64, _vp = C.c_int32, C.c_int64, C.c_float, C.c_double, C.c_void_p


class BnT(C.Structure):
    _fields_ = [('mode', _i32), ('relu', _i32), ('eps', _f32), ('_pad', _i32), ('stats', _vp), ('gamma', _vp),
                ('beta', _vp), ('running_mean', _vp), ('running_var', _vp)]


class ConvT(C.Structure):
    _fields_ = [('N', _i32), ('H', _i32), ('W', _i32), ('C', _i32), ('K', _i32), ('R', _i32), ('S', _i32),
                ('stride', _i32), ('pad', _i32), ('P', _i32), ('Q', _i32), ('dtype', _i32), ('epi', _i32),
                ('_pad', _i32), ('x', _vp), ('w', _vp), ('bias', _vp), ('residual', _vp), ('y', _vp),
                ('out_stats', _vp), ('bn', BnT), ('epi_x', _vp), ('epi_bn', BnT), ('epi_stats', _vp),
                ('wg_partial', _vp), ('wg_stride', _i64), ('wg_bias', _i32), ('wg_count', _i32),
                ('fold_x', _vp), ('fold_bn', BnT), ('fold_stats', _vp), ('fold_out', _vp), ('fold_dgamma', _vp), ('fold_dbeta', _vp)]


class ConvF8T(C.Structure):
    _fields_ = [('c', ConvT), ('w8', _vp), ('w8_scale', _vp)]


class WquantEntryT(C.Structure):
    _fields_ = [('w', _vp), ('w8', _vp), ('scale', _vp), ('K', _i32), ('RSC', _i32)]


class ConvPairT(C.Structure):
    _fields_ = [('a', ConvT), ('b', ConvT)]


class BneckT(C.Structure):
    _fields_ = [('N', _i32), ('H', _i32), ('W', _i32), ('C', _i32), ('P', _i32), ('dtype', _i32), ('_pad', _i32 * 2),
                ('x', _vp), ('y', _vp), ('w1', _vp), ('b1', _vp), ('w2', _vp), ('b2', _vp), ('w3', _vp), ('b3', _vp),
                ('bn1', BnT), ('bn2', BnT), ('bn3', BnT), ('folded', _vp)]


class BneckPairT(C.Structure):
    _fields_ = [('a', BneckT), ('b', BneckT)]


class WgradT(C.Structure):
    _fields_ = [('N', _i32), ('H', _i32), ('W', _i32), ('C', _i32), ('K', _i32), ('R', _i32), ('S', _i32),
                ('stride', _i32), ('pad', _i32), ('P', _i32), ('Q', _i32), ('dtype', _i32), ('x', _vp), ('dy', _vp),
                ('dw', _vp), ('dbias', _vp), ('bn', BnT), ('partial', _vp), ('partial_stride', _i64)]


class StemT(C.Structure):
    _fields_ = [('N', _i32), ('H', _i32), ('W', _i32), ('K', _i32), ('P', _i32), ('Q', _i32), ('dtype', _i32),
                ('_pad', _i32), ('x', _vp), ('w', _vp), ('bias', _vp), ('y', _vp), ('out_stats', _vp), ('dy', _vp),
                ('dw', _vp), ('dbias', _vp), ('partial', _vp), ('partial_stride', _i64)]


class EwT(C.Structure):
    _fields_ = [('op', _i32), ('dtype', _i32), ('N', _i32), ('H', _i32), ('W', _i32), ('C', _i32), ('x', _vp),
                ('x2', _vp), ('dy', _vp), ('add', _vp), ('y', _vp), ('out_stats', _vp), ('bstats', _vp),
                ('dgamma', _vp), ('dbeta', _vp), ('bn', BnT)]


class EwPairT(C.Structure):
    _fields_ = [('a', EwT), ('b', EwT)]


class HeadT(C.Structure):
    _fields_ = [('N', _i32), ('H', _i32), ('W', _i32), ('C', _i32), ('J', _i32), ('dtype', _i32), ('_pad', _i32 * 2),
                ('y0', _vp), ('x', _vp), ('score', _vp), ('next', _vp), ('w_fc', _vp), ('b_fc', _vp), ('w_score', _vp),
                ('b_score', _vp), ('w_fc2', _vp), ('b_fc2', _vp), ('w_score2', _vp), ('b_score2', _vp), ('bn', BnT),
                ('folded', _vp)]


class AffTermT(C.Structure):
    _fields_ = [('x', _vp), ('bn', BnT), ('up', _i32), ('_pad', _i32)]


class AffsumT(C.Structure):
    _fields_ = [('N', _i32), ('H', _i32), ('W', _i32), ('C', _i32), ('dtype', _i32), ('relu', _i32), ('nterms', _i32),
                ('_pad', _i32), ('t', AffTermT * 4), ('y', _vp)]


class LayoutT(C.Structure):
    _fields_ = [('src', _vp), ('dst', _vp), ('N', _i32), ('C', _i32), ('H', _i32), ('W', _i32), ('dtype', _i32), ('_pad', _i32)]


class PckT(C.Structure):
    _fields_ = [('B', _i32), ('J', _i32), ('H', _i32), ('W', _i32), ('dtype', _i32), ('log_slots', _i32), ('thr', C.c_float),
                ('_pad', _i32), ('out', _vp), ('target', _vp), ('counts', _vp), ('log', _vp), ('cursor', _vp), ('losses', _vp)]


class FlipMergeT(C.Structure):
    _fields_ = [('N', _i32), ('J', _i32), ('H', _i32), ('W', _i32), ('shift', _i32), ('_pad', _i32), ('a', _vp), ('b', _vp),
                ('y', _vp), ('src', _i32 * 32)]


class FinalPredsT(C.Structure):
    _fields_ = [('N', _i32), ('J', _i32), ('H', _i32), ('W', _i32), ('post_process', _i32), ('_pad', _i32), ('hm', _vp),
                ('trans', _vp), ('coords', _vp), ('preds', _vp), ('maxvals', _vp)]


class TargetsT(C.Structure):
    _fields_ = [('B', _i32), ('J', _i32), ('H', _i32), ('W', _i32), ('patch', _i32), ('_pad', _i32), ('stride_x', _f64),
                ('stride_y', _f64), ('joints', _vp), ('vis', _vp), ('g', _vp), ('target', _vp), ('weight', _vp)]


class WarpSrcT(C.Structure):
    _fields_ = [('img', _vp), ('h', _i32), ('w', _i32), ('row_bytes', _i64), ('minv', _f64 * 6)]


class WarpT(C.Structure):
    _fields_ = [('B', _i32), ('H', _i32), ('W', _i32), ('_pad', _i32), ('src', _vp), ('mean', _f32 * 3), ('std', _f32 * 3),
                ('out', _vp)]


class LossT(C.Structure):
    _fields_ = [('B', _i32), ('J', _i32), ('H', _i32), ('W', _i32), ('S', _i32), ('dtype', _i32),
                ('target_nchw', _i32), ('alpha', _f32), ('out', _vp * MAX_STACKS), ('dout', _vp * MAX_STACKS),
                ('teacher', _vp), ('target', _vp), ('weight', _vp), ('losses', _vp), ('grad_scale', _f32),
                ('_pad', _i32), ('weight_kd', _vp)]


class AdamT(C.Structure):
    _fields_ = [('n', _i64), ('param', _vp), ('grad', _vp), ('m', _vp), ('v', _vp), ('param_lp', _vp),
                ('lr', _f32), ('beta1', _f32), ('beta2', _f32), ('eps', _f32), ('bias_corr1', _f32),
                ('bias_corr2', _f32), ('grad_scale', _f32), ('_pad', _i32), ('lr_dev', _vp), ('step_dev', _vp)]


class WprepEntryT(C.Structure):
    _fields_ = [('w', _vp), ('w_fwd', _vp), ('w_bwd', _vp), ('K', _i32), ('R', _i32), ('S', _i32), ('C', _i32)]


class BnupdEntryT(C.Structure):
    _fields_ = [('stats', _vp), ('running_mean', _vp), ('running_var', _vp), ('num_batches_tracked', _vp),
                ('count', _f64), ('momentum', _f32), ('C', _i32)]


class WreduceEntryT(C.Structure):
    _fields_ = [('partial', _vp), ('dw', _vp), ('n', _i64), ('stride', _i64), ('count', _i32), ('_pad', _i32)]


class MemsetT(C.Structure):
    _fields_ = [('ptr', _vp), ('bytes', _i64)]


class TableT(C.Structure):
    _fields_ = [('table', _vp), ('n', _i32), ('dtype', _i32), ('max_elems', _i64)]


_STRUCTS = {'fpd_bn_t': BnT, 'fpd_conv_t': ConvT, 'fpd_wgrad_t': WgradT, 'fpd_stem_t': StemT, 'fpd_ew_t': EwT,
            'fpd_loss_t': LossT, 'fpd_adam_t': AdamT, 'fpd_wprep_entry_t': WprepEntryT,
            'fpd_bnupd_entry_t': BnupdEntryT, 'fpd_memset_t': MemsetT, 'fpd_table_t': TableT,
            'fpd_wreduce_entry_t': WreduceEntryT, 'fpd_bneck_t': BneckT, 'fpd_conv_pair_t': ConvPairT, 'fpd_bneck_pair_t': BneckPairT, 'fpd_ew_pair_t': EwPairT, 'fpd_pck_t': PckT, 'fpd_head_t': HeadT, 'fpd_affsum_t': AffsumT, 'fpd_layout_t': LayoutT,
            'fpd_conv_f8_t': ConvF8T, 'fpd_wquant_entry_t': WquantEntryT, 'fpd_flipmerge_t': FlipMergeT, 'fpd_finalpreds_t': FinalPredsT, 'fpd_targets_t': TargetsT,
            'fpd_warp_src_t': WarpSrcT, 'fpd_warp_t': WarpT}

ABI_VERSION = 2

SYMBOLS = {
    'fpd_conv_forward': (C.c_int, [C.POINTER(ConvT), _vp]),
    'fpd_conv_forward_pair': (C.c_int, [C.POINTER(ConvPairT), _vp]),
    'fpd_conv_forward_f8': (C.c_int, [C.POINTER(ConvF8T), _vp]),
    'fpd_conv_f8_in_domain': (C.c_int, [C.POINTER(ConvT)]),
    'fpd_weight_quant_f8': (C.c_int, [_vp, _i32, _vp]),
    'fpd_bottleneck_forward': (C.c_int, [C.POINTER(BneckT), _vp]),
    'fpd_bottleneck_fold': (C.c_int, [C.POINTER(BneckT), _vp]),
    'fpd_bottleneck_forward_pair': (C.c_int, [C.POINTER(BneckPairT), _vp]),
    'fpd_conv_fused_wgrad_partials': (C.c_int, [C.POINTER(ConvT)]),
    'fpd_conv_fold_supported': (C.c_int, [_vp]),
    'fpd_conv_pair_fold_supported': (C.c_int, [_vp]),
    'fpd_conv_pair_fused_wgrad_partials': (C.c_int, [C.POINTER(ConvPairT), C.POINTER(C.c_int32), C.POINTER(C.c_int32)]),
    'fpd_conv_wgrad': (C.c_int, [C.POINTER(WgradT), _vp]),
    'fpd_wgrad_num_partials': (C.c_int, [C.POINTER(WgradT)]),
    'fpd_wgrad_reduce': (C.c_int, [_vp, _i32, _i64, _vp]),
    'fpd_stem_forward': (C.c_int, [C.POINTER(StemT), _vp]),
    'fpd_stem_wgrad': (C.c_int, [C.POINTER(StemT), _vp]),
    'fpd_stem_wgrad_num_partials': (C.c_int, [C.POINTER(StemT)]),
    'fpd_elementwise': (C.c_int, [C.POINTER(EwT), _vp]),
    'fpd_elementwise_pair': (C.c_int, [C.POINTER(EwPairT), _vp]),
    'fpd_pck': (C.c_int, [C.POINTER(PckT), _vp]),
    'fpd_affsum': (C.c_int, [C.POINTER(AffsumT), _vp]),
    'fpd_flip_w': (C.c_int, [_vp, _vp, _i64, _i32, _vp]),
    'fpd_flip_merge': (C.c_int, [C.POINTER(FlipMergeT), _vp]),
    'fpd_final_preds': (C.c_int, [C.POINTER(FinalPredsT), _vp]),
    'fpd_render_targets': (C.c_int, [C.POINTER(TargetsT), _vp]),
    'fpd_warp_affine': (C.c_int, [C.POINTER(WarpT), _vp]),
    'fpd_head_forward': (C.c_int, [C.POINTER(HeadT), _vp]),
    'fpd_head_fold': (C.c_int, [C.POINTER(HeadT), _vp]),
    'fpd_loss': (C.c_int, [C.POINTER(LossT), _vp]),
    'fpd_adam': (C.c_int, [C.POINTER(AdamT), _vp]),
    'fpd_weight_prep': (C.c_int, [_vp, _i32, _i64, _i32, _vp]),
    'fpd_bn_update_running': (C.c_int, [_vp, _i32, _vp]),
    'fpd_cast': (C.c_int, [_vp, _vp, _i64, _i32, _i32, _vp]),
    'fpd_nchw_to_nhwc': (C.c_int, [_vp, _vp, _i32, _i32, _i32, _i32, _i32, _vp]),
    'fpd_nhwc_to_nchw': (C.c_int, [_vp, _vp, _i32, _i32, _i32, _i32, _i32, _vp]),
    'fpd_plan_create': (_vp, []),
    'fpd_plan_destroy': (None, [_vp]),
    'fpd_plan_add': (C.c_int, [_vp, _i32, _vp, _i64]),
    'fpd_plan_size': (C.c_int, [_vp]),
    'fpd_plan_set_schedule': (C.c_int, [_vp, _i32, _i32, C.POINTER(C.c_int32), _i32]),
    'fpd_plan_mark_event': (C.c_int, [_vp, _i32]),
    'fpd_plan_wait_op': (C.c_int, [_vp, _i32, _vp]),
    'fpd_plan_run': (C.c_int, [_vp, _i32, _i32, _vp]),
    'fpd_plan_run_op': (C.c_int, [_vp, _i32, _vp]),
    'fpd_plan_capture': (C.c_int, [_vp, _i32, _i32, _vp]),
    'fpd_plan_replay': (C.c_int, [_vp, _i32, _vp]),
    'fpd_last_error': (C.c_char_p, []),
    'fpd_set_backend': (C.c_int, [_i32]),
    'fpd_set_option': (C.c_int, [C.c_char_p, _i32]),
    'fpd_abi_sizeof': (C.c_int, [C.c_char_p]),
    'fpd_abi_version': (C.c_int, []),
    'fpd_stats_words': (C.c_int64, [C.c_int32]),
    'fpd_event_create': (_vp, []),
    'fpd_event_record': (C.c_int, [_vp, _vp]),
    'fpd_event_elapsed_ms': (C.c_float, [_vp, _vp]),
    'fpd_event_destroy': (None, [_vp]),
}

_lib = None


class FpdError(RuntimeError):
    pass


def lib_sha16():
    import hashlib
    with open(LIB_PATH, 'rb') as f:
        return hashlib.sha256(f.read()).hexdigest()[:16]


def lib():
    global _lib
    if _lib is not None:
        return _lib
    if not os.path.exists(LIB_PATH):
        raise FpdError('HIP extension %s is missing: run `python __graft_entry__.py` (build()) first; '
                       'there is no CPU fallback for the FPD path' % LIB_PATH)
    import torch
    try:
        torch.cuda.is_available()
    except Exception:
        pass
    l = C.CDLL(LIB_PATH)
    for name, (res, args) in SYMBOLS.items():
        fn = getattr(l, name)
        fn.restype = res
        fn.argtypes = args
    if l.fpd_abi_version() != ABI_VERSION:
        raise FpdError('ABI version mismatch: library %d, python host %d' % (l.fpd_abi_version(), ABI_VERSION))
    for name, st in _STRUCTS.items():
        got = l.fpd_abi_sizeof(name.encode())
        if got != C.sizeof(st):
            raise FpdError('ABI mismatch for %s: library %d bytes, python %d bytes' % (name, got, C.sizeof(st)))
    _lib = l
    return l


def check(rc, what=''):
    if rc != 0:
        raise FpdError('%s failed (rc=%d): %s' % (what or 'fpd call', rc, lib().fpd_last_error().decode()))


def set_backend(backend):
    return lib().fpd_set_backend(backend)


def set_option(name, value):
    prev = lib().fpd_set_option(name.encode(), int(value))
    if prev < 0:
        check(prev, 'fpd_set_option(%s)' % name)
    return prev


def current_stream():
    import torch
    return C.c_void_p(torch.cuda.current_stream().cuda_stream)


class Plan:

    def __init__(self):
        self._l = lib()
        self._p = C.c_void_p(self._l.fpd_plan_create())
        self._graphs = {}
        self._types = []

    def add(self, op, args):
        rc = self._l.fpd_plan_add(self._p, op, C.byref(args), C.sizeof(args))
        if rc < 0:
            check(rc, 'fpd_plan_add')
        self._types.append(op)
        return rc

    def op_type(self, k):
        return self._types[k]

    def __len__(self):
        return self._l.fpd_plan_size(self._p)

    def set_schedule(self, op, lane, waits=()):
        arr = (C.c_int32 * max(len(waits), 1))(*waits)
        check(self._l.fpd_plan_set_schedule(self._p, op, lane, arr, len(waits)), 'fpd_plan_set_schedule')

    def mark_event(self, op):
        check(self._l.fpd_plan_mark_event(self._p, op), 'fpd_plan_mark_event')

    def wait_op(self, op, stream):
        check(self._l.fpd_plan_wait_op(self._p, op, stream), 'fpd_plan_wait_op')

    def run(self, begin, end, stream=None):
        check(self._l.fpd_plan_run(self._p, begin, end, stream if stream is not None else current_stream()),
              'fpd_plan_run')

    def run_op(self, op, stream=None):
        check(self._l.fpd_plan_run_op(self._p, op, stream if stream is not None else current_stream()), 'fpd_plan_run_op')

    def capture(self, begin, end, stream):
        gid = self._l.fpd_plan_capture(self._p, begin, end, stream)
        if gid < 0:
            check(gid, 'fpd_plan_capture')
        return gid

    def replay(self, gid, stream=None):
        check(self._l.fpd_plan_replay(self._p, gid, stream if stream is not None else current_stream()),
              'fpd_plan_replay')

    def __del__(self):
        try:
            if self._p:
                self._l.fpd_plan_destroy(self._p)
                self._p = None
        except Exception:
            pass
```

include/fpd_amd.h:

```cpp
#ifndef FPD_AMD_H
#define FPD_AMD_H

#include <stddef.h>
#include <stdint.h>

#ifdef __cplusplus
extern "C" {
#endif

typedef void* fpd_stream_t;

enum { FPD_F32 = 0, FPD_BF16 = 1 };
#ifndef FPD_STATS_REPLICAS
#define FPD_STATS_REPLICAS 4
#endif
typedef int64_t fpd_stat_t;
#define FPD_STATS_WORDS(C) ((int64_t)FPD_STATS_REPLICAS * 4 * (C))
enum { FPD_BN_NONE = 0, FPD_BN_TRAIN = 1, FPD_BN_EVAL = 2 };
enum { FPD_EPI_PLAIN = 0, FPD_EPI_BNRELU_BWD = 1 };
enum { FPD_BACKEND_MFMA = 0, FPD_BACKEND_NAIVE = 1, FPD_BACKEND_MFMA_GENERIC = 2 };

typedef struct {
    int32_t mode;
    int32_t relu;
    float eps;
    int32_t _pad;
    const fpd_stat_t* stats;
    const float* gamma;
    const float* beta;
    const float* running_mean;
    const float* running_var;
} fpd_bn_t;

typedef struct {
    int32_t N, H, W, C;
    int32_t K, R, S;
    int32_t stride, pad;
    int32_t P, Q;
    int32_t dtype;
    int32_t epi;
    int32_t _pad;
    const void* x;
    const void* w;
    const float* bias;
    const void* residual;
    void* y;
    fpd_stat_t* out_stats;
    fpd_bn_t bn;
    const void* epi_x;
    fpd_bn_t epi_bn;
    fpd_stat_t* epi_stats;
    float* wg_partial;
    int64_t wg_stride;
    int32_t wg_bias;
    int32_t wg_count;
    const void* fold_x;
    fpd_bn_t fold_bn;
    const fpd_stat_t* fold_stats;
    void* fold_out;
    float* fold_dgamma;
    float* fold_dbeta;
} fpd_conv_t;

typedef struct {
    int32_t N, H, W, C, P, dtype;
    int32_t _pad[2];
    const void* x;
    void* y;
    const void* w1;
    const float* b1;
    const void* w2;
    const float* b2;
    const void* w3;
    const float* b3;
    fpd_bn_t bn1, bn2, bn3;
    const float* folded;
} fpd_bneck_t;

typedef struct {
    int32_t N, H, W, C, J, dtype;
    int32_t _pad[2];
    const void* y0;
    const void* x;
    void* score;
    void* next;
    const void* w_fc;
    const float* b_fc;
    const void* w_score;
    const float* b_score;
    const void* w_fc2;
    const float* b_fc2;
    const void* w_score2;
    const float* b_score2;
    fpd_bn_t bn;
    const float* folded;
} fpd_head_t;
int fpd_head_forward(const fpd_head_t* a, fpd_stream_t stream);
int fpd_head_fold(const fpd_head_t* a, fpd_stream_t stream);

typedef struct { fpd_conv_t a, b; } fpd_conv_pair_t;

typedef struct { fpd_bneck_t a, b; } fpd_bneck_pair_t;

typedef struct {
    int32_t N, H, W, C, K, R, S, stride, pad, P, Q, dtype;
    const void* x;
    const void* dy;
    float* dw;
    float* dbias;
    fpd_bn_t bn;
    float* partial;
    int64_t partial_stride;
} fpd_wgrad_t;

typedef struct {
    int32_t N, H, W, K, P, Q, dtype, _pad;
    const float* x;
    const float* w;
    const float* bias;
    void* y;
    fpd_stat_t* out_stats;
    const void* dy;
    float* dw;
    float* dbias;
    float* partial;
    int64_t partial_stride;
} fpd_stem_t;

enum {
    FPD_EW_BNRELU_FWD = 0, FPD_EW_BNRELU_BWD_R = 1, FPD_EW_BN_BWD_APPLY = 2, FPD_EW_MAXPOOL_FWD = 3,
    FPD_EW_MAXPOOL_BWD = 4, FPD_EW_UPADD_FWD = 5, FPD_EW_SUMPOOL = 6, FPD_EW_ADD = 7, FPD_EW_RELU_MASK = 8,
    FPD_EW_DILATE2 = 9
};
typedef struct {
    int32_t op, dtype;
    int32_t N, H, W, C;
    const void* x;
    const void* x2;
    const void* dy;
    const void* add;
    void* y;
    fpd_stat_t* out_stats;
    fpd_stat_t* bstats;
    float* dgamma;
    float* dbeta;
    fpd_bn_t bn;
} fpd_ew_t;

#define FPD_AFFSUM_MAX 4
typedef struct { const void* x; fpd_bn_t bn; int32_t up; int32_t _pad; } fpd_affterm_t;
typedef struct {
    int32_t N, H, W, C;
    int32_t dtype, relu, nterms, _pad;
    fpd_affterm_t t[FPD_AFFSUM_MAX];
    void* y;
} fpd_affsum_t;
int fpd_affsum(const fpd_affsum_t* a, fpd_stream_t stream);

typedef struct { const float* src; void* dst; int32_t N, C, H, W, dtype, _pad; } fpd_layout_t;

#define FPD_MAX_STACKS 8
typedef struct {
    int32_t B, J, H, W, S, dtype;
    int32_t target_nchw;
    float alpha;
    const void* out[FPD_MAX_STACKS];
    void* dout[FPD_MAX_STACKS];
    const void* teacher;
    const float* target;
    const float* weight;
    double* losses;
    float grad_scale;
    int32_t _pad;
    const float* weight_kd;
} fpd_loss_t;

typedef struct {
    int64_t n;
    float* param; const float* grad; float* m; float* v;
    void* param_lp;
    float lr, beta1, beta2, eps;
    float bias_corr1, bias_corr2;
    float grad_scale;
    int32_t _pad;
    const float* lr_dev;
    int64_t* step_dev;
} fpd_adam_t;

typedef struct {
    const float* w;
    void* w_fwd;
    void* w_bwd;
    int32_t K, R, S, C;
} fpd_wprep_entry_t;

typedef struct {
    const fpd_stat_t* stats;
    float* running_mean; float* running_var; int64_t* num_batches_tracked;
    double count; float momentum; int32_t C;
} fpd_bnupd_entry_t;

typedef struct {
    const float* partial; float* dw; int64_t n; int64_t stride; int32_t count; int32_t _pad;
} fpd_wreduce_entry_t;

int fpd_conv_forward(const fpd_conv_t* a, fpd_stream_t stream);
int fpd_conv_forward_pair(const fpd_conv_pair_t* p, fpd_stream_t stream);
int fpd_bottleneck_forward(const fpd_bneck_t* a, fpd_stream_t stream);
int fpd_bottleneck_fold(const fpd_bneck_t* a, fpd_stream_t stream);
int fpd_bottleneck_forward_pair(const fpd_bneck_pair_t* p, fpd_stream_t stream);
int fpd_conv_fused_wgrad_partials(const fpd_conv_t* a);
int fpd_conv_fold_supported(const fpd_conv_t* a);
int fpd_conv_pair_fold_supported(const fpd_conv_pair_t* p);
int fpd_conv_pair_fused_wgrad_partials(const fpd_conv_pair_t* p, int32_t* n_a, int32_t* n_b);
int fpd_conv_wgrad(const fpd_wgrad_t* a, fpd_stream_t stream);
int fpd_wgrad_num_partials(const fpd_wgrad_t* a);
int fpd_wgrad_reduce(const fpd_wreduce_entry_t* table_dev, int32_t n_entries, int64_t max_elems, fpd_stream_t stream);
int fpd_stem_forward(const fpd_stem_t* a, fpd_stream_t stream);
int fpd_stem_wgrad(const fpd_stem_t* a, fpd_stream_t stream);
int fpd_stem_wgrad_num_partials(const fpd_stem_t* a);
int fpd_elementwise(const fpd_ew_t* a, fpd_stream_t stream);
typedef struct { fpd_ew_t a, b; } fpd_ew_pair_t;
int fpd_elementwise_pair(const fpd_ew_pair_t* p, fpd_stream_t stream);
int fpd_loss(const fpd_loss_t* a, fpd_stream_t stream);
int fpd_adam(const fpd_adam_t* a, fpd_stream_t stream);
int fpd_weight_prep(const fpd_wprep_entry_t* table_dev, int32_t n_entries, int64_t max_elems, int32_t dtype,
                    fpd_stream_t stream);
int fpd_bn_update_running(const fpd_bnupd_entry_t* table_dev, int32_t n_entries, fpd_stream_t stream);
int fpd_cast(const void* src, void* dst, int64_t n, int32_t src_dtype, int32_t dst_dtype, fpd_stream_t stream);
int fpd_nchw_to_nhwc(const float* src, void* dst, int32_t N, int32_t C, int32_t H, int32_t W, int32_t dtype,
                     fpd_stream_t stream);
int fpd_nhwc_to_nchw(const void* src, float* dst, int32_t N, int32_t C, int32_t H, int32_t W, int32_t dtype,
                     fpd_stream_t stream);

typedef struct {
    int32_t B, J, H, W, dtype, log_slots;
    float thr;
    int32_t _pad;
    const void* out;
    const float* target;
    float* counts;
    double* log;
    long long* cursor;
    const double* losses;
} fpd_pck_t;
int fpd_pck(const fpd_pck_t* a, fpd_stream_t stream);

typedef struct {
    fpd_conv_t c;
    const void* w8;
    const float* w8_scale;
} fpd_conv_f8_t;
int fpd_conv_forward_f8(const fpd_conv_f8_t* a, fpd_stream_t stream);
int fpd_conv_f8_in_domain(const fpd_conv_t* c);

typedef struct {
    const float* w;
    void* w8;
    float* scale;
    int32_t K, RSC;
} fpd_wquant_entry_t;
int fpd_weight_quant_f8(const fpd_wquant_entry_t* table_dev, int32_t n_entries, fpd_stream_t stream);

int fpd_flip_w(const float* x, float* y, int64_t rows, int32_t W, fpd_stream_t stream);

#define FPD_MAX_JOINTS 32
typedef struct {
    int32_t N, J, H, W;
    int32_t shift, _pad;
    const float* a;
    const float* b;
    float* y;
    int32_t src[FPD_MAX_JOINTS];
} fpd_flipmerge_t;
int fpd_flip_merge(const fpd_flipmerge_t* a, fpd_stream_t stream);

typedef struct {
    int32_t N, J, H, W;
    int32_t post_process, _pad;
    const float* hm;
    const double* trans;
    float* coords;
    float* preds;
    float* maxvals;
} fpd_finalpreds_t;
int fpd_final_preds(const fpd_finalpreds_t* a, fpd_stream_t stream);

typedef struct {
    int32_t B, J, H, W;
    int32_t patch, _pad;
    double stride_x, stride_y;
    const double* joints;
    const float* vis;
    const float* g;
    float* target;
    float* weight;
} fpd_targets_t;
int fpd_render_targets(const fpd_targets_t* a, fpd_stream_t stream);

typedef struct {
    const uint8_t* img;
    int32_t h, w;
    int64_t row_bytes;
    double minv[6];
} fpd_warp_src_t;
typedef struct {
    int32_t B, H, W, _pad;
    const fpd_warp_src_t* src;
    float mean[3], std[3];
    float* out;
} fpd_warp_t;
int fpd_warp_affine(const fpd_warp_t* a, fpd_stream_t stream);

enum {
    FPD_OP_CONV = 0, FPD_OP_WGRAD = 1, FPD_OP_STEM_FWD = 2, FPD_OP_STEM_WGRAD = 3, FPD_OP_EW = 4,
    FPD_OP_LOSS = 5, FPD_OP_ADAM = 6, FPD_OP_MEMSET = 7, FPD_OP_WPREP = 8, FPD_OP_BNUPD = 9, FPD_OP_WREDUCE = 10,
    FPD_OP_BNECK = 11, FPD_OP_BNECK_FOLD = 12, FPD_OP_CONV_PAIR = 13, FPD_OP_BNECK_PAIR = 14, FPD_OP_EW_PAIR = 15, FPD_OP_PCK = 16, FPD_OP_HEAD = 17,
    FPD_OP_HEAD_FOLD = 18, FPD_OP_NOP = 19, FPD_OP_AFFSUM = 20, FPD_OP_NCHW2NHWC = 21, FPD_OP_CONV_F8 = 22,
    FPD_OP_WQUANT = 23
};
typedef struct { void* ptr; int64_t bytes; } fpd_memset_t;
typedef struct { const void* table; int32_t n; int32_t dtype; int64_t max_elems; } fpd_table_t;

typedef struct fpd_plan fpd_plan;
fpd_plan* fpd_plan_create(void);
void fpd_plan_destroy(fpd_plan* p);
int fpd_plan_add(fpd_plan* p, int32_t op, const void* args, int64_t args_bytes);
int fpd_plan_size(const fpd_plan* p);
#define FPD_MAX_LANES 16
int fpd_plan_set_schedule(fpd_plan* p, int32_t op, int32_t lane, const int32_t* wait_ops, int32_t n_waits);
int fpd_plan_mark_event(fpd_plan* p, int32_t op);
int fpd_plan_wait_op(fpd_plan* p, int32_t op, fpd_stream_t stream);
int fpd_plan_run(fpd_plan* p, int32_t begin, int32_t end, fpd_stream_t stream);
int fpd_plan_run_op(fpd_plan* p, int32_t op, fpd_stream_t stream);
int fpd_plan_capture(fpd_plan* p, int32_t begin, int32_t end, fpd_stream_t stream);
int fpd_plan_replay(fpd_plan* p, int32_t graph_id, fpd_stream_t stream);

const char* fpd_last_error(void);
int fpd_set_backend(int32_t backend);
int fpd_set_option(const char* name, int32_t value);
int fpd_abi_sizeof(const char* struct_name);
#define FPD_ABI_VERSION 2
int fpd_abi_version(void);
int64_t fpd_stats_words(int32_t channels);
void* fpd_event_create(void);
int fpd_event_record(void* ev, fpd_stream_t stream);
float fpd_event_elapsed_ms(void* start, void* stop);
void fpd_event_destroy(void* ev);

#ifdef __cplusplus
}
#endif
#endif
```

Baseline: 3709 images/s.

## Fuse maxpool and upsample-add producers into eval bottleneck input loads

Adds x-source modes to the fused eval bottleneck kernel so it can read its input as a 2x2 max-pool of a larger tensor or as an upsample-add of two tensors, computed on the fly in both the A-operand loads and the residual path. A planning pass folds single-reader maxpool/upadd elementwise ops into the following bottleneck in non-train (teacher) forward, removing a separate kernel launch and an intermediate activation write and read. The cost is four loads per pooled input vector and extra unpack/pack work in the kernel, plus a changed struct layout.

```diff
diff --git a/fast-human-pose-estimation.pytorch_amd/csrc/api.hip b/fast-human-pose-estimation.pytorch_amd/csrc/api.hip
--- a/fast-human-pose-estimation.pytorch_amd/csrc/api.hip
+++ b/fast-human-pose-estimation.pytorch_amd/csrc/api.hip
@@ -29,6 +29,7 @@
 int fpd_conv_pp_pair_wgrad_partials(const fpd_conv_t& a, const fpd_conv_t& b, int* na, int* nb);
 int fpd_conv_tile_pair_launch(const fpd_conv_t& a, const fpd_conv_t& b, hipStream_t st);
 int fpd_bneck_fused_launch(const fpd_bneck_t& a, hipStream_t st);
+int fpd_bneck_xsrc_ok(const fpd_bneck_t& a);
 int fpd_bneck_fold_launch(const fpd_bneck_t& a, float* out, hipStream_t st);
 int fpd_pck_launch(const fpd_pck_t& a, hipStream_t st);
 int fpd_conv_smallc_launch(const fpd_conv_t& a, hipStream_t st);
@@ -265,6 +266,21 @@
     return 0;
 }
 
+static int validate_bneck_xsrc(const fpd_bneck_t* a) {
+    FPD_REQUIRE(a->xsrc == FPD_BNECK_X_PLAIN || a->xsrc == FPD_BNECK_X_POOL || a->xsrc == FPD_BNECK_X_UPADD,
+                "bottleneck: unknown x-source mode %d", a->xsrc);
+    FPD_REQUIRE(a->xsrc != FPD_BNECK_X_UPADD || a->x2, "bottleneck: x-source mode UPADD needs x2");
+    FPD_REQUIRE(a->xsrc != FPD_BNECK_X_UPADD || a->x2 != a->y, "bottleneck: y must not alias x2");
+    FPD_REQUIRE(a->xsrc != FPD_BNECK_X_POOL || (int64_t)a->N * a->H * a->W * a->C * 4 < ((int64_t)1 << 31),
+                "bottleneck: pooled source too large for 32-bit indexing");
+    return 0;
+}
+
+int fpd_bottleneck_xsrc_supported(const fpd_bneck_t* a) {
+    if (!a || g_fpd_backend != FPD_BACKEND_MFMA || a->N <= 0 || a->H <= 0 || a->W <= 0) return 0;
+    return fpd_bneck_xsrc_ok(*a);
+}
+
 int fpd_bottleneck_fold(const fpd_bneck_t* a, fpd_stream_t stream) {
     FPD_REQUIRE(a && a->folded, "bottleneck_fold: null pointer");
     int rc = validate_bneck_bns(a);
@@ -282,6 +298,8 @@
         FPD_REQUIRE((int64_t)a->N * a->H * a->W * a->C < ((int64_t)1 << 31), "bottleneck_pair: tensor too large for 32-bit indexing");
         int rc = validate_bneck_bns(a);
         if (rc) return rc;
+        rc = validate_bneck_xsrc(a);
+        if (rc) return rc;
     }
     int rc = fpd_bneck_fused_pair_launch(p->a, p->b, (hipStream_t)stream);
     if (rc == 1) {
@@ -298,10 +316,12 @@
     FPD_REQUIRE((int64_t)a->N * a->H * a->W * a->C < ((int64_t)1 << 31), "bottleneck: tensor too large for 32-bit indexing");
     int rc = validate_bneck_bns(a);
     if (rc) return rc;
+    rc = validate_bneck_xsrc(a);
+    if (rc) return rc;
     rc = fpd_bneck_fused_launch(*a, (hipStream_t)stream);
     if (rc == 1)
-        return fpd_fail(-3, "bottleneck: shape N=%d H=%d W=%d C=%d P=%d dtype=%d is outside the fused kernel's domain",
-                        a->N, a->H, a->W, a->C, a->P, a->dtype);
+        return fpd_fail(-3, "bottleneck: shape N=%d H=%d W=%d C=%d P=%d dtype=%d xsrc=%d is outside the fused kernel's domain",
+                        a->N, a->H, a->W, a->C, a->P, a->dtype, a->xsrc);
     return rc ? rc : check_launch();
 }
 
@@ -606,6 +626,7 @@
     char t[200] = "";
     static const char* ew_names[] = {"bnrelu_fwd", "bnrelu_bwd_r", "bn_bwd_apply", "maxpool_fwd", "maxpool_bwd", "upadd_fwd", "sumpool", "add", "relu_mask", "dilate2"};
     auto ewn = [&](int op) { return (op >= 0 && op < 10) ? ew_names[op] : "ew"; };
+    auto xsrc_tag = [](int m) { return m == FPD_BNECK_X_POOL ? " x=pool" : m == FPD_BNECK_X_UPADD ? " x=upadd" : ""; };
     switch (o.type) {
         case FPD_OP_CONV: conv_tag(t, sizeof(t), "conv", o.u.conv); break;
         case FPD_OP_CONV_F8: conv_tag(t, sizeof(t), "conv_f8", o.u.conv8.c); break;
@@ -617,8 +638,8 @@
             break;
         }
         case FPD_OP_WGRAD: snprintf(t, sizeof(t), "wgrad N=%d H=%d W=%d C=%d K=%d R=%d s=%d", o.u.wgrad.N, o.u.wgrad.H, o.u.wgrad.W, o.u.wgrad.C, o.u.wgrad.K, o.u.wgrad.R, o.u.wgrad.stride); break;
-        case FPD_OP_BNECK: snprintf(t, sizeof(t), "bneck N=%d H=%d W=%d C=%d P=%d", o.u.bneck.N, o.u.bneck.H, o.u.bneck.W, o.u.bneck.C, o.u.bneck.P); break;
-        case FPD_OP_BNECK_PAIR: snprintf(t, sizeof(t), "bneck2 N=%d H=%d W=%d C=%d P=%d | H=%d W=%d", o.u.bpair.a.N, o.u.bpair.a.H, o.u.bpair.a.W, o.u.bpair.a.C, o.u.bpair.a.P, o.u.bpair.b.H, o.u.bpair.b.W); break;
+        case FPD_OP_BNECK: snprintf(t, sizeof(t), "bneck N=%d H=%d W=%d C=%d P=%d%s", o.u.bneck.N, o.u.bneck.H, o.u.bneck.W, o.u.bneck.C, o.u.bneck.P, xsrc_tag(o.u.bneck.xsrc)); break;
+        case FPD_OP_BNECK_PAIR: snprintf(t, sizeof(t), "bneck2 N=%d H=%d W=%d C=%d P=%d%s | H=%d W=%d%s", o.u.bpair.a.N, o.u.bpair.a.H, o.u.bpair.a.W, o.u.bpair.a.C, o.u.bpair.a.P, xsrc_tag(o.u.bpair.a.xsrc), o.u.bpair.b.H, o.u.bpair.b.W, xsrc_tag(o.u.bpair.b.xsrc)); break;
         case FPD_OP_HEAD: snprintf(t, sizeof(t), "head N=%d H=%d W=%d C=%d J=%d", o.u.head.N, o.u.head.H, o.u.head.W, o.u.head.C, o.u.head.J); break;
         case FPD_OP_EW: snprintf(t, sizeof(t), "ew %s N=%d H=%d W=%d C=%d", ewn(o.u.ew.op), o.u.ew.N, o.u.ew.H, o.u.ew.W, o.u.ew.C); break;
         case FPD_OP_EW_PAIR: snprintf(t, sizeof(t), "ew2 %s N=%d H=%d W=%d C=%d | H=%d W=%d", ewn(o.u.epair.a.op), o.u.epair.a.N, o.u.epair.a.H, o.u.epair.a.W, o.u.epair.a.C, o.u.epair.b.H, o.u.epair.b.W); break;
diff --git a/fast-human-pose-estimation.pytorch_amd/csrc/bneck_fused.hip b/fast-human-pose-estimation.pytorch_amd/csrc/bneck_fused.hip
--- a/fast-human-pose-estimation.pytorch_amd/csrc/bneck_fused.hip
+++ b/fast-human-pose-estimation.pytorch_amd/csrc/bneck_fused.hip
@@ -45,7 +45,32 @@
 template <int P>
 __global__ void bneck_fold_kernel(const fpd_bneck_t a, float* out) { bneck_fold_tables<P>(a, out, threadIdx.x, blockDim.x); }
 
-template <int P, bool DMA>
+__device__ __forceinline__ u32x4 bneck_pack8(const float* f) {
+    const uint4 pk = DT<bf16_t>::pack(f);
+    const u32x4 r = {pk.x, pk.y, pk.z, pk.w};
+    return r;
+}
+__device__ __forceinline__ u32x4 bneck_pool4(const bf16_t* __restrict__ s, const int col, const int row) {
+    const u32x4 r0 = *reinterpret_cast<const u32x4*>(s), r1 = *reinterpret_cast<const u32x4*>(s + col),
+                r2 = *reinterpret_cast<const u32x4*>(s + row), r3 = *reinterpret_cast<const u32x4*>(s + row + col);
+    float v0[8], v1[8], v2[8], v3[8], o[8];
+    DT<bf16_t>::unpack(make_uint4(r0[0], r0[1], r0[2], r0[3]), v0);
+    DT<bf16_t>::unpack(make_uint4(r1[0], r1[1], r1[2], r1[3]), v1);
+    DT<bf16_t>::unpack(make_uint4(r2[0], r2[1], r2[2], r2[3]), v2);
+    DT<bf16_t>::unpack(make_uint4(r3[0], r3[1], r3[2], r3[3]), v3);
+#pragma unroll
+    for (int e = 0; e < 8; ++e) o[e] = fmaxf(fmaxf(v0[e], v1[e]), fmaxf(v2[e], v3[e]));
+    return bneck_pack8(o);
+}
+__device__ __forceinline__ void bneck_upadd8(float* f, const u32x4 r2) {
+    float u[8];
+    DT<bf16_t>::unpack(make_uint4(r2[0], r2[1], r2[2], r2[3]), u);
+#pragma unroll
+    for (int e = 0; e < 8; ++e) f[e] = f[e] + u[e];
+    DT<bf16_t>::unpack(DT<bf16_t>::pack(f), f);
+}
+
+template <int P, bool DMA, int XS = FPD_BNECK_X_PLAIN>
 __device__ __forceinline__ void bneck_eval_body(const fpd_bneck_t& a, const int logW, const int swz, const int bid_in,
                                                 const int nblk, const int ntiles) {
     constexpr int C = 2 * P;
@@ -94,6 +119,8 @@
     bf16_t* sA2 = reinterpret_cast<bf16_t*>(s_b3 + C);
     bf16_t* sR2 = sA2 + (zero_px + 3) * LD2;
     const bf16_t* __restrict__ x = reinterpret_cast<const bf16_t*>(a.x);
+    const bf16_t* __restrict__ x2 = reinterpret_cast<const bf16_t*>(a.x2);
+    const int pcol = C, prow = 2 * W * C;
     const bf16_t* __restrict__ w1 = reinterpret_cast<const bf16_t*>(a.w1);
     const bf16_t* __restrict__ w2 = reinterpret_cast<const bf16_t*>(a.w2);
     const bf16_t* __restrict__ w3 = reinterpret_cast<const bf16_t*>(a.w3);
@@ -102,6 +129,7 @@
     int npass = whole ? 1 : ((hrows * W + 127) >> 7);
     const int xpx = tid >> 3, xcv = (tid & 7) * 8;
     int xo[2];
+    int xo2[2];
     bool xok[2];
     auto pass_addr = [&](int p) __attribute__((always_inline)) {
 #pragma unroll
@@ -110,7 +138,9 @@
             const int hr = hp >> logW, j = hp & (W - 1);
             const int g = g0 - 1 + hr;
             xok[i] = hr < hrows && (unsigned)g < (unsigned)GR;
-            xo[i] = xok[i] ? (g * W + j) * C + xcv : 0;
+            if constexpr (XS == FPD_BNECK_X_POOL) xo[i] = xok[i] ? (4 * g * W + 2 * j) * C + xcv : 0;
+            else xo[i] = xok[i] ? (g * W + j) * C + xcv : 0;
+            if constexpr (XS == FPD_BNECK_X_UPADD) xo2[i] = xok[i] ? ((g >> 1) * (W >> 1) + (j >> 1)) * C + xcv : 0;
         }
     };
     int w1o[W1V], w1l[W1V];
@@ -123,18 +153,40 @@
     const int xl = xpx * LDX + xcv;
 
     u32x4 rx[NCH][2], rw[NCH][W1V];
+    u32x4 rx2[XS == FPD_BNECK_X_UPADD ? NCH : 1][2];
     auto a_load = [&](auto kcc) __attribute__((always_inline)) {
         constexpr int kc = decltype(kcc)::value;
         static_for<2>([&](auto ic) {
             constexpr int i = decltype(ic)::value;
             const u32x4 z = {0u, 0u, 0u, 0u};
             rx[kc][i] = z;
-            if (xok[i]) rx[kc][i] = *reinterpret_cast<const u32x4*>(x + (xo[i] + kc * 64));
+            if constexpr (XS == FPD_BNECK_X_POOL) {
+                if (xok[i]) rx[kc][i] = bneck_pool4(x + (xo[i] + kc * 64), pcol, prow);
+            } else {
+                if (xok[i]) rx[kc][i] = *reinterpret_cast<const u32x4*>(x + (xo[i] + kc * 64));
+            }
+            if constexpr (XS == FPD_BNECK_X_UPADD) {
+                rx2[kc][i] = z;
+                if (xok[i]) rx2[kc][i] = *reinterpret_cast<const u32x4*>(x2 + (xo2[i] + kc * 64));
+            }
         });
         static_for<W1V>([&](auto ic) {
             constexpr int i = decltype(ic)::value;
             rw[kc][i] = *reinterpret_cast<const u32x4*>(w1 + (w1o[i] + kc * 64));
         });
+    };
+    auto a_sum = [&](auto kcc) __attribute__((always_inline)) {
+        constexpr int kc = decltype(kcc)::value;
+        if constexpr (XS == FPD_BNECK_X_UPADD) {
+            static_for<2>([&](auto ic) {
+                constexpr int i = decltype(ic)::value;
+                float f[8];
+                const u32x4 r = rx[kc][i];
+                DT<bf16_t>::unpack(make_uint4(r[0], r[1], r[2], r[3]), f);
+                bneck_upadd8(f, rx2[kc][i]);
+                rx[kc][i] = bneck_pack8(f);
+            });
+        }
     };
     constexpr int NSL = 2 + W1V;
     auto a_store_slice = [&](auto kcc, auto slc) __attribute__((always_inline)) {
@@ -252,11 +304,12 @@
             *reinterpret_cast<uint4*>(sA2 + px * LD2 + cv) = z;
         }
     }
+    static_for<NCH>([&](auto kcc) { a_sum(kcc); });
     STAMP(1);
 
     auto refill = [&](auto kcc, int pp) __attribute__((always_inline)) {
         constexpr int kc = decltype(kcc)::value;
-        if (pp + 1 < npass) a_load(kcc);
+        if (pp + 1 < npass) { a_load(kcc); a_sum(kcc); }
         else if constexpr (kc < 2) t_load(kcc);
     };
 #ifdef FPD_BNECK_TIMING
@@ -382,7 +435,24 @@
             const int m = m0 + q * 32 + px;
             const u32x4 z = {0u, 0u, 0u, 0u};
             rres[st][it] = z;
-            if (m < M) rres[st][it] = *reinterpret_cast<const u32x4*>(x + ((size_t)m * C + st * P + hC * CW + cv));
+            if constexpr (XS == FPD_BNECK_X_PLAIN) {
+                if (m < M) rres[st][it] = *reinterpret_cast<const u32x4*>(x + ((size_t)m * C + st * P + hC * CW + cv));
+            } else {
+                const int g = m >> logW, j = m & (W - 1);
+                const int c = st * P + hC * CW + cv;
+                if constexpr (XS == FPD_BNECK_X_POOL) {
+                    if (m < M) rres[st][it] = bneck_pool4(x + ((size_t)(4 * g * W + 2 * j) * C + c), pcol, prow);
+                } else {
+                    if (m < M) {
+                        const u32x4 r1 = *reinterpret_cast<const u32x4*>(x + ((size_t)m * C + c));
+                        const u32x4 r2 = *reinterpret_cast<const u32x4*>(x2 + ((size_t)((g >> 1) * (W >> 1) + (j >> 1)) * C + c));
+                        float f[8];
+                        DT<bf16_t>::unpack(make_uint4(r1[0], r1[1], r1[2], r1[3]), f);
+                        bneck_upadd8(f, r2);
+                        rres[st][it] = bneck_pack8(f);
+                    }
+                }
+            }
         });
     };
 
@@ -478,17 +548,17 @@
 #endif
 }
 
-template <int P, bool DMA>
+template <int P, bool DMA, int XS>
 __global__ __launch_bounds__(512, 1) void bneck_eval_kernel(const fpd_bneck_t a, const int logW, const int ntiles) {
-    bneck_eval_body<P, DMA>(a, logW, (ntiles & 7) == 0, blockIdx.x, gridDim.x, ntiles);
-}
-
-template <int P, bool DMA>
+    bneck_eval_body<P, DMA, XS>(a, logW, (ntiles & 7) == 0, blockIdx.x, gridDim.x, ntiles);
+}
+
+template <int P, bool DMA, int XB>
 __global__ __launch_bounds__(512, 1) void bneck_eval_pair_kernel(const fpd_bneck_t a, const fpd_bneck_t b, const int logWa,
                                                                  const int logWb, const int nblk_a, const int ntiles_a,
                                                                  const int ntiles_b) {
     if ((int)blockIdx.x < nblk_a) bneck_eval_body<P, DMA>(a, logWa, (ntiles_a & 7) == 0, blockIdx.x, nblk_a, ntiles_a);
-    else bneck_eval_body<P, DMA>(b, logWb, (ntiles_b & 7) == 0, (int)blockIdx.x - nblk_a, (int)gridDim.x - nblk_a, ntiles_b);
+    else bneck_eval_body<P, DMA, XB>(b, logWb, (ntiles_b & 7) == 0, (int)blockIdx.x - nblk_a, (int)gridDim.x - nblk_a, ntiles_b);
 }
 
 
@@ -519,11 +589,11 @@
     return (size_t)(3 * C + 4 * P) * sizeof(float) + (size_t)(irows * WP + 3) * LD2 * 2 + r2;
 }
 
-template <int P, bool DMA>
+template <int P, bool DMA, int XB>
 int launch_bneck_pair(const fpd_bneck_t& a, const fpd_bneck_t& b, hipStream_t st) {
     const size_t lds = std::max(bneck_lds_bytes<P>(a.H, a.W), bneck_lds_bytes<P>(b.H, b.W));
     static LdsAttr configured;
-    if (int rc_ = configured.ensure(reinterpret_cast<const void*>(&bneck_eval_pair_kernel<P, DMA>), lds)) return rc_;
+    if (int rc_ = configured.ensure(reinterpret_cast<const void*>(&bneck_eval_pair_kernel<P, DMA, XB>), lds)) return rc_;
     int la = 0, lb = 0;
     while ((1 << la) < a.W) ++la;
     while ((1 << lb) < b.W) ++lb;
@@ -535,17 +605,17 @@
         nb = bneck_blocks(tb, capb);
         na = bneck_blocks(ta, std::max(1, cap - nb));
     }
-    FPD_LAUNCH((bneck_eval_pair_kernel<P, DMA>), dim3(na + nb), dim3(512), lds, st, a, b, la, lb, na, ta, tb);
+    FPD_LAUNCH((bneck_eval_pair_kernel<P, DMA, XB>), dim3(na + nb), dim3(512), lds, st, a, b, la, lb, na, ta, tb);
     return 0;
 }
 
-template <int P, bool DMA>
+template <int P, bool DMA, int XS>
 int launch_bneck(const fpd_bneck_t& a, int logW, hipStream_t st) {
     const size_t lds = bneck_lds_bytes<P>(a.H, a.W);
     static LdsAttr configured;
-    if (int rc_ = configured.ensure(reinterpret_cast<const void*>(&bneck_eval_kernel<P, DMA>), lds)) return rc_;
+    if (int rc_ = configured.ensure(reinterpret_cast<const void*>(&bneck_eval_kernel<P, DMA, XS>), lds)) return rc_;
     const int ntiles = cdiv(a.N * a.H * a.W, 128);
-    FPD_LAUNCH((bneck_eval_kernel<P, DMA>), dim3(bneck_blocks(ntiles, bneck_block_cap())), dim3(512), lds, st, a, logW, ntiles);
+    FPD_LAUNCH((bneck_eval_kernel<P, DMA, XS>), dim3(bneck_blocks(ntiles, bneck_block_cap())), dim3(512), lds, st, a, logW, ntiles);
     return 0;
 }
 
@@ -555,19 +625,35 @@
     if (a.dtype != FPD_BF16 || a.C != 2 * a.P || (a.P != 64 && a.P != 128)) return false;
     if (a.W < 4 || a.W > 64 || (a.W & (a.W - 1)) != 0) return false;
     const int hw = a.H * a.W;
-    return hw % 128 == 0 || 128 % hw == 0;
-}
+    if (!(hw % 128 == 0 || 128 % hw == 0)) return false;
+    if (a.xsrc == FPD_BNECK_X_PLAIN) return true;
+    if (a.xsrc != FPD_BNECK_X_POOL && a.xsrc != FPD_BNECK_X_UPADD) return false;
+    if ((a.H & 1) || (a.W & 1)) return false;
+    if (a.xsrc == FPD_BNECK_X_UPADD && a.x2 == nullptr) return false;
+    if (a.x == nullptr || a.y == a.x || (a.x2 != nullptr && a.y == a.x2)) return false;
+    const int64_t src = (int64_t)a.N * a.H * a.W * a.C * (a.xsrc == FPD_BNECK_X_POOL ? 4 : 1);
+    return src < ((int64_t)1 << 31);
+}
+
+int fpd_bneck_xsrc_ok(const fpd_bneck_t& a) { return bneck_in_domain(a) ? 1 : 0; }
 
 int fpd_bneck_fused_launch(const fpd_bneck_t& a, hipStream_t st) {
     if (!bneck_in_domain(a)) return 1;
     int logW = 0;
     while ((1 << logW) < a.W) ++logW;
-    return a.P == 128 ? launch_bneck<128, true>(a, logW, st) : launch_bneck<64, true>(a, logW, st);
+    if (a.xsrc == FPD_BNECK_X_POOL)
+        return a.P == 128 ? launch_bneck<128, true, FPD_BNECK_X_POOL>(a, logW, st) : launch_bneck<64, true, FPD_BNECK_X_POOL>(a, logW, st);
+    if (a.xsrc == FPD_BNECK_X_UPADD)
+        return a.P == 128 ? launch_bneck<128, true, FPD_BNECK_X_UPADD>(a, logW, st) : launch_bneck<64, true, FPD_BNECK_X_UPADD>(a, logW, st);
+    return a.P == 128 ? launch_bneck<128, true, FPD_BNECK_X_PLAIN>(a, logW, st) : launch_bneck<64, true, FPD_BNECK_X_PLAIN>(a, logW, st);
 }
 
 int fpd_bneck_fused_pair_launch(const fpd_bneck_t& a, const fpd_bneck_t& b, hipStream_t st) {
     if (!bneck_in_domain(a) || !bneck_in_domain(b) || a.P != b.P) return 1;
-    return a.P == 128 ? launch_bneck_pair<128, true>(a, b, st) : launch_bneck_pair<64, true>(a, b, st);
+    if (a.xsrc != FPD_BNECK_X_PLAIN || b.xsrc == FPD_BNECK_X_UPADD) return 1;
+    if (b.xsrc == FPD_BNECK_X_POOL)
+        return a.P == 128 ? launch_bneck_pair<128, true, FPD_BNECK_X_POOL>(a, b, st) : launch_bneck_pair<64, true, FPD_BNECK_X_POOL>(a, b, st);
+    return a.P == 128 ? launch_bneck_pair<128, true, FPD_BNECK_X_PLAIN>(a, b, st) : launch_bneck_pair<64, true, FPD_BNECK_X_PLAIN>(a, b, st);
 }
 
 int fpd_bneck_fold_launch(const fpd_bneck_t& a, float* out, hipStream_t st) {
diff --git a/fast-human-pose-estimation.pytorch_amd/executor.py b/fast-human-pose-estimation.pytorch_amd/executor.py
--- a/fast-human-pose-estimation.pytorch_amd/executor.py
+++ b/fast-human-pose-estimation.pytorch_amd/executor.py
@@ -105,6 +105,37 @@
     if k == 'conv' and h >= 32 and (('no3x3big' in _WHATIF and dims[5] == 3) or ('no1x1big' in _WHATIF and dims[5] == 1)):
         return True
     return ('nobig' in _WHATIF and h >= 64) or ('nomid' in _WHATIF and h == 32) or ('nosmall' in _WHATIF and h <= 16)
+
+
+_XSRC = {'pool': R.BNECK_X_POOL, 'upadd': R.BNECK_X_UPADD}
+
+
+def plan_bneck_xsrc(ops, supported):
+    members_of = lambda top: [m for m in ((top.a, top.b) if top.kind in ('conv2', 'ew2', 'bneck2') else (top,)) if m is not None]
+    out, taken = [], set()
+    for i, op in enumerate(ops):
+        if op.kind != 'ew' or op.op not in ('maxpool_fwd', 'upadd_fwd') or getattr(op, 'folded', False):
+            continue
+        if op.out_stats is not None or op.add is not None or op.y.persistent:
+            continue
+        readers = [(j, m) for j, top in enumerate(ops) for m in members_of(top) if any(t is op.y for t in m.acts_in())]
+        if len(readers) != 1:
+            continue
+        j, m = readers[0]
+        if j <= i or m.kind != 'bneck' or m.x is not op.y or id(m) in taken:
+            continue
+        mode = 'pool' if op.op == 'maxpool_fwd' else 'upadd'
+        if supported(m, mode):
+            taken.add(id(m))
+            out.append((op, m, mode))
+    return out
+
+
+def apply_bneck_xsrc(decisions):
+    for ew, m, mode in decisions:
+        ew.folded = True
+        m.xsrc, m.xsrc_op = mode, ew
+        m.extra_in = list(getattr(m, 'extra_in', [])) + [t for t in (ew.x, ew.x2) if t is not None]
 
 
 class Lowering:
@@ -226,12 +257,22 @@
         s.table, s.n, s.dtype, s.max_elems = self._table(ents, R.WquantEntryT), len(ents), self.dtype, 0
         return R.OP_WQUANT, s
 
+    def bneck_xsrc_supported(self, op, mode):
+        s = R.BneckT()
+        (s.N, s.H, s.W, s.C, s.P) = op.dims
+        s.dtype, s.xsrc = self.dtype, _XSRC[mode]
+        s.x, s.x2, s.y = 1 << 20, (2 << 20) if mode == 'upadd' else None, 3 << 20
+        return R.lib().fpd_bottleneck_xsrc_supported(C.byref(s)) == 1
+
     def bneck(self, op):
         s = R.BneckT()
         (s.N, s.H, s.W, s.C, s.P) = op.dims
         s.dtype = self.dtype
         p = self.A.ptr
         s.x, s.y = p(_abuf(op.x)), p(_abuf(op.y))
+        if getattr(op, 'xsrc', None):
+            ew = op.xsrc_op
+            s.xsrc, s.x, s.x2 = _XSRC[op.xsrc], p(_abuf(ew.x)), p(_abuf(ew.x2))
         s.w1, s.b1, s.w2, s.b2, s.w3, s.b3 = p(op.w1), p(op.b1), p(op.w2), p(op.b2), p(op.w3), p(op.b3)
         s.bn1, s.bn2, s.bn3 = self.bn(op.bn1), self.bn(op.bn2), self.bn(op.bn3)
         s.folded = p(getattr(op, 'folded', None))
@@ -485,6 +526,8 @@
         delay = int(os.environ.get('FPD_REUSE_DELAY', '400')) if self.lanes_enabled else 0
         if not self.train:
             delay = 0
+            if os.environ.get('FPD_BNECK_XSRC', '1') != '0':
+                apply_bneck_xsrc(plan_bneck_xsrc(g.fwd, self.low.bneck_xsrc_supported))
         act = G.plan_memory(ops, reuse_delay=delay)
         self.act_elems = act
         self.A.alloc('act', act)
diff --git a/fast-human-pose-estimation.pytorch_amd/graph.py b/fast-human-pose-estimation.pytorch_amd/graph.py
--- a/fast-human-pose-estimation.pytorch_amd/graph.py
+++ b/fast-human-pose-estimation.pytorch_amd/graph.py
@@ -104,6 +104,7 @@
         elif k == 'bneck':
             rd = [b(self.x), self.w1, self.b1, self.w2, self.b2, self.w3, self.b3] + bn_bufs(self.bn1) + \
                 bn_bufs(self.bn2) + bn_bufs(self.bn3)
+            rd += [b(t) for t in getattr(self, 'extra_in', [])]
             wr = [b(self.y)]
         elif k == 'wgrad':
             rd = [b(self.x), b(self.dy)] + bn_bufs(self.bn)
diff --git a/fast-human-pose-estimation.pytorch_amd/runtime.py b/fast-human-pose-estimation.pytorch_amd/runtime.py
--- a/fast-human-pose-estimation.pytorch_amd/runtime.py
+++ b/fast-human-pose-estimation.pytorch_amd/runtime.py
@@ -7,6 +7,7 @@
 F32, BF16 = 0, 1
 BN_NONE, BN_TRAIN, BN_EVAL = 0, 1, 2
 EPI_PLAIN, EPI_BNRELU_BWD = 0, 1
+BNECK_X_PLAIN, BNECK_X_POOL, BNECK_X_UPADD = 0, 1, 2
 BACKEND_MFMA, BACKEND_NAIVE, BACKEND_MFMA_GENERIC = 0, 1, 2
 (EW_BNRELU_FWD, EW_BNRELU_BWD_R, EW_BN_BWD_APPLY, EW_MAXPOOL_FWD, EW_MAXPOOL_BWD, EW_UPADD_FWD, EW_SUMPOOL,
  EW_ADD, EW_RELU_MASK, EW_DILATE2) = range(10)
@@ -47,8 +48,8 @@
 
 
 class BneckT(C.Structure):
-    _fields_ = [('N', _i32), ('H', _i32), ('W', _i32), ('C', _i32), ('P', _i32), ('dtype', _i32), ('_pad', _i32 * 2),
-                ('x', _vp), ('y', _vp), ('w1', _vp), ('b1', _vp), ('w2', _vp), ('b2', _vp), ('w3', _vp), ('b3', _vp),
+    _fields_ = [('N', _i32), ('H', _i32), ('W', _i32), ('C', _i32), ('P', _i32), ('dtype', _i32), ('xsrc', _i32), ('_pad', _i32),
+                ('x', _vp), ('x2', _vp), ('y', _vp), ('w1', _vp), ('b1', _vp), ('w2', _vp), ('b2', _vp), ('w3', _vp), ('b3', _vp),
                 ('bn1', BnT), ('bn2', BnT), ('bn3', BnT), ('folded', _vp)]
 
 
@@ -177,6 +178,7 @@
     'fpd_conv_f8_in_domain': (C.c_int, [C.POINTER(ConvT)]),
     'fpd_weight_quant_f8': (C.c_int, [_vp, _i32, _vp]),
     'fpd_bottleneck_forward': (C.c_int, [C.POINTER(BneckT), _vp]),
+    'fpd_bottleneck_xsrc_supported': (C.c_int, [C.POINTER(BneckT)]),
     'fpd_bottleneck_fold': (C.c_int, [C.POINTER(BneckT), _vp]),
     'fpd_bottleneck_forward_pair': (C.c_int, [C.POINTER(BneckPairT), _vp]),
     'fpd_conv_fused_wgrad_partials': (C.c_int, [C.POINTER(ConvT)]),
diff --git a/include/fpd_amd.h b/include/fpd_amd.h
--- a/include/fpd_amd.h
+++ b/include/fpd_amd.h
@@ -62,10 +62,13 @@
     float* fold_dbeta;
 } fpd_conv_t;
 
+enum { FPD_BNECK_X_PLAIN = 0, FPD_BNECK_X_POOL = 1, FPD_BNECK_X_UPADD = 2 };
 typedef struct {
     int32_t N, H, W, C, P, dtype;
-    int32_t _pad[2];
-    const void* x;
+    int32_t xsrc;
+    int32_t _pad;
+    const void* x;
+    const void* x2;
     void* y;
     const void* w1;
     const float* b1;
@@ -207,6 +210,7 @@
 int fpd_conv_forward(const fpd_conv_t* a, fpd_stream_t stream);
 int fpd_conv_forward_pair(const fpd_conv_pair_t* p, fpd_stream_t stream);
 int fpd_bottleneck_forward(const fpd_bneck_t* a, fpd_stream_t stream);
+int fpd_bottleneck_xsrc_supported(const fpd_bneck_t* a);
 int fpd_bottleneck_fold(const fpd_bneck_t* a, fpd_stream_t stream);
 int fpd_bottleneck_forward_pair(const fpd_bneck_pair_t* p, fpd_stream_t stream);
 int fpd_conv_fused_wgrad_partials(const fpd_conv_t* a);
```

New measurement: 3634 images/s. 2.0% lower.
